# rickenator/steganosaurus

Measured on AMD Instinct MI355X. Metric: MPixels/s embed+extract round-trip (RGB 2D-FFT fwd+inv), higher is better.
Workload: dtype f32

## Files before the change

steganosaurus_amd/csrc/tfft_capi.hip:

```cpp
#include <hip/hip_runtime.h>
#include <math.h>
#include <stdio.h>
#include <stdlib.h>
#include <string.h>

#include <algorithm>
#include <complex>
#include <map>
#include <tuple>
#include <new>
#include <vector>

#include "tfft_kernels.h"

extern "C" void tfft_internal_radius_bounds(double lo, double hi, uint64_t* s_lo, uint64_t* s_hi, int* empty);
extern "C" float tfft_internal_mag2_threshold(double thr) { return tfft::mag2_threshold(thr); }

namespace {

using namespace tfft;

int next_pow2(int v) { int p = 1; while (p < v) p <<= 1; return p; }
int ilog2i(int n) { int l = 0; while ((1 << l) < n) l++; return l; }

struct Slot {
    int W = 0, H = 0, PW = 0, PH = 0, PWi = 0, center = 0;
    bool has_spec = false;
    const uint8_t* rgb_src = nullptr;
};

struct ColPlan { bool direct; int log_n1, log_n2; bool fused_fwd; };

}

struct tfft_ctx {
    int device = 0;
    int max_w = 0, max_h = 0, n_slots = 0;
    hipStream_t stream = nullptr;
    bool own_stream = false;
    hipEvent_t ev_t0 = nullptr, ev_t1 = nullptr;
    int last_hip = 0;
    size_t dev_bytes = 0;
    std::vector<Slot> slots;
    size_t img_stride_b = 0;
    size_t slot_stride = 0;
    size_t cand_stride = 0;
    uint8_t* img_pool = nullptr;
    float2* spec_pool = nullptr;
    float2* tmp_pool = nullptr;
    unsigned* cand_pool = nullptr;
    int stats_prio = 1;
    int stats_tile = 1;
    int stats_tile_step_forced = 0;
    int stats_tile_step = 8;
    float2* col0_pool = nullptr;
    int stats_skew = 0;
    SelectState* sel = nullptr;
    float* med = nullptr;
    unsigned* partial = nullptr;
    float* amb = nullptr;
    unsigned long long* usable = nullptr;
    int exact_stats = 1;
    ExactCand* ex_cand = nullptr; double2* ex_val = nullptr; unsigned long long* ex_below = nullptr; unsigned* ex_n = nullptr;
    std::map<int, double2*> ex_table;
    int ex_last[3] = {0, 0, 0};
    int* err = nullptr;
    uint8_t* trash = nullptr;
    int* last_row = nullptr;
    struct TileBuckets { float2* fl = nullptr; uint8_t* pb = nullptr; uint64_t fl_cap = 0;
                         unsigned* cnt = nullptr; unsigned* off = nullptr; TileBin* ent = nullptr; uint64_t cap = 0; int nb_cap = 0;
                         const void* built_for = nullptr; uint64_t built_n = 0; int built_ph = 0, built_pw = 0, built_g = 0; const void* built_index = nullptr; bool built_bad = false;
                         const void* row_for = nullptr; uint64_t row_n = 0; int row_ph = 0, row_pw = 0;
                         float2* jp = nullptr; uint64_t jp_cap = 0; uint64_t jp_for = 0;
                       } tb[2];
    const void* reg_bins = nullptr; uint64_t reg_n = 0;
    int embed_delta = 1;
    int tile_read = 1;
    hipStream_t stream2 = nullptr;
    hipEvent_t ev_fork = nullptr, ev_join = nullptr;
    hipStream_t stream_stats[2] = {nullptr, nullptr};
    hipEvent_t ev_stats_fork[2] = {nullptr, nullptr}, ev_stats_join[2] = {nullptr, nullptr};
    int stats_async = 1;
    int stats_m2 = 1;
    int n_streams = 1;
    int n_cus = 0, collect_resident = 0;
    uint32_t* bit_index = nullptr;
    uint64_t bit_index_n = 0;
    float* ph_jit = nullptr;
    uint64_t ph_n = 0;
    int ph_adaptive = 0;
    uint64_t ph_version = 0;
    std::map<int, float2*> tw;
    std::map<std::tuple<int, int, int, int>, float2*> dc;
    float dc_bias = 128.0f;
    uint8_t* sio_hdr = nullptr; uint8_t* sio_pay = nullptr; int* sio_status = nullptr; uint64_t sio_plen = 0;
    uint8_t* stream_bits = nullptr; unsigned* stream_plen = nullptr; size_t stream_cap = 0;
    void* stage_bins = nullptr; void* stage_bits = nullptr; void* stage_jit = nullptr; void* stage_out = nullptr;
    size_t stage_cap = 0;
    hipStream_t s_in = nullptr, s_out = nullptr;
    hipEvent_t ev_in[4] = {}, ev_comp[4] = {}, ev_out[4] = {};
    uint8_t* out_pool = nullptr;
    int cols_direct_max_log = 8;
    int cols_force_log_n1 = -1;
    int cols_tiles_per_block = 8;
    int cols_tiles_forced = 0;
    int cols_tiles_embed = 0;
    int cols_tiles_stat = 16;
    int cols_tiles_read = 16;
    int median_force_fallback = 0;
#ifndef TFFT_NO_GRAPHS
    struct GraphEntry { hipGraphExec_t exec = nullptr; int state = 0; };
    std::map<std::vector<uint64_t>, GraphEntry> graphs;
#endif
    int stats_fail_once = 0;
    bool stats_dirty = false;
    bool graphs_stale = false;
    int graph_max_images = 0;
    int stats_fused = 1;
    int stats_compact = 1;
    int fuse = 1;
    int fuse_wide = 1;
// ... 66 lines not shown
    if (w > c->max_w || h > c->max_h) return TFFT_E_TOO_LARGE;
    s.W = w; s.H = h; s.PW = next_pow2(w); s.PH = next_pow2(h);
    s.PWi = s.PW < 2 ? 2 : s.PW;
    s.center = center ? 1 : 0;
    if (s.PWi > TFFT_MAX_DIM || s.PH > TFFT_MAX_DIM) return TFFT_E_TOO_LARGE;
    return TFFT_OK;
}

enum Stage { ROWS_FWD = 0, COLS_FWD_A = 1, COLS_FWD_B = 2, EMBED = 3, COLS_INV_A = 4, COLS_INV_B = 5, ROWS_INV = 6,
             READ = 7, MEDIANS = 8, CAPACITY = 9,
             COLS_FWD_READ = 10,
             N_STAGES = 11 };

int get_dc_table(tfft_ctx* c, int valid, int N, int center, int kind, double scale, const float2** out);
void invalidate_graphs(tfft_ctx* c);

static void copy_embed_fields(ColParams& cp, const ColParams& e, bool inverse) {
    cp.rd_bins = e.rd_bins; cp.rd_off = e.rd_off; cp.trash = e.trash; cp.rd_walks = e.rd_walks;
    cp.em_n = e.em_n; cp.em_cos = e.em_cos; cp.em_sin = e.em_sin; cp.em_fl = e.em_fl; cp.em_pb = e.em_pb; cp.em_on = 1; cp.em_m2 = e.em_m2;
    if (inverse) { cp.em_jp = e.em_jp; cp.em_med = e.em_med; cp.em_alpha = e.em_alpha; cp.em_dsrc = e.em_dsrc; }
    cp.st_sel = e.st_sel; cp.st_cand = e.st_cand; cp.st_cand_stride = e.st_cand_stride; cp.st_partial = e.st_partial; cp.st_amb = e.st_amb;
    cp.st_col0 = e.st_col0; cp.st_slo = e.st_slo; cp.st_shi = e.st_shi; cp.st_cap = e.st_cap; cp.st_PW = e.st_PW;
}

static void copy_plain_extra(ColParams& cp, const ColParams& e) {
    if (e.tile_step > 1) cp.tiles_per_block = e.hist_sel ? 2 : 1;
    cp.tile_step = e.tile_step; cp.tile_off = e.tile_off; cp.out_M = e.out_M; cp.out_plane_stride = e.out_plane_stride; cp.out_img_stride = e.out_img_stride; cp.gate = e.gate;
    cp.hist_sel = e.hist_sel; cp.g_step = e.g_step; cp.g_off = e.g_off;
}

struct StageMode {
    const ColParams* fwd_emit = nullptr;
    const ColParams* fwd_read = nullptr;
    const int* fwd_last_row = nullptr;
    const ColParams* inv_embed = nullptr;
    const uint8_t* inv_cover = nullptr;
    const ColParams* fwd_plain_extra = nullptr;
    float2* fwd_out_override = nullptr;
    bool inv_via_spec = false;
};

int enqueue_fft_stage(tfft_ctx* c, int s0, int n, int stage, const uint8_t* rgb_in, uint8_t* rgb_out, hipStream_t st, const StageMode& md = StageMode()) {
    const Slot& s = c->slots[s0];
    const int M = s.PWi / 2;
    const float2 *tw_w, *tw_h;
    int rc = get_twiddles(c, s.PWi, &tw_w); if (rc) return rc;
    rc = get_twiddles(c, s.PH, &tw_h); if (rc) return rc;
    const ColPlan pl = plan_cols(c, s.PH, s.PWi, n);
    const int N1 = 1 << pl.log_n1, N2 = 1 << pl.log_n2;
    float2 *spec = c->spec(s0), *tmp = c->tmp(s0);
    ColParams cp{};
    cp.M = M; cp.PH = s.PH; cp.plane_stride = (size_t)s.PH * M; cp.img_stride = c->slot_stride;
    cp.tiles_per_block = c->cols_tiles_per_block;
    switch (stage) {
        case ROWS_FWD: {
            RowParams rp{s.W, s.H, s.PWi, s.PH, s.center, 0.f, c->slot_stride, c->dc_bias, nullptr};
            if (pl.fused_fwd && c->fuse_live && s.H < s.PH) HIPCHK(c, launch_rowcol_fwd_live(rgb_in, tmp, tw_w, tw_h, rp, n, st));
            else if (pl.fused_fwd) HIPCHK(c, launch_rowcol_fwd(rgb_in, tmp, tw_w, tw_h, rp, n, st));
            else HIPCHK(c, launch_rows_fwd(rgb_in, tmp, tw_w, rp, n, st));
            return TFFT_OK;
        }
        case COLS_FWD_A:
            if (pl.fused_fwd) return TFFT_OK;
            if (pl.direct) {
                cp.G = 1; cp.in_a = 1; cp.in_b = 0; cp.out_a = 1; cp.out_b = 0; cp.in_rows = s.H; cp.out_rows = s.PH; cp.tw_out = 0;
                cp.last_row_dev = md.fwd_last_row;
            if (c->dc_bias != 0.0f) {
                rc = get_dc_table(c, s.H, s.PH, s.center, 0, (double)c->dc_bias, &cp.dc_ah); if (rc) return rc;
                rc = get_dc_table(c, s.W, s.PWi, s.center, 1, 1.0, &cp.dc_aw); if (rc) return rc;
            }
                if (md.fwd_read) { const ColParams& r = *md.fwd_read; cp.rd_bins = r.rd_bins; cp.rd_off = r.rd_off; cp.rd_bits = r.rd_bits; cp.rd_n = r.rd_n; cp.em_jp = r.em_jp; cp.rd_walks = r.rd_walks; cp.trash = c->trash; cp.tiles_per_block = c->cols_tiles_read; }
                else if (md.fwd_emit) { copy_embed_fields(cp, *md.fwd_emit, false); if (!c->cols_tiles_forced && pl.log_n2 <= 8) cp.tiles_per_block = 2; if (cp.st_sel && c->cols_tiles_stat) cp.tiles_per_block = c->cols_tiles_stat; }
                else if (md.fwd_plain_extra) copy_plain_extra(cp, *md.fwd_plain_extra);
                HIPCHK(c, launch_cols(tmp, md.fwd_out_override ? md.fwd_out_override : spec, tw_h, cp, pl.log_n2, +1, 3 * n, st));
            } else {
                cp.G = N2; cp.in_a = N2; cp.in_b = 1; cp.out_a = N2; cp.out_b = 1; cp.in_rows = s.H; cp.out_rows = s.PH; cp.tw_out = 1;
                HIPCHK(c, launch_cols(tmp, tmp, tw_h, cp, pl.log_n1, +1, 3 * n, st));
            }
            return TFFT_OK;
        case COLS_FWD_B:
            if (pl.direct) return TFFT_OK;
            cp.G = N1; cp.in_a = 1; cp.in_b = N2; cp.out_a = N1; cp.out_b = 1; cp.in_rows = s.PH; cp.out_rows = s.PH; cp.tw_out = 0;
            cp.last_row_dev = md.fwd_last_row;
            if (c->dc_bias != 0.0f) {
                rc = get_dc_table(c, s.H, s.PH, s.center, 0, (double)c->dc_bias, &cp.dc_ah); if (rc) return rc;
                rc = get_dc_table(c, s.W, s.PWi, s.center, 1, 1.0, &cp.dc_aw); if (rc) return rc;
            }
            if (md.fwd_read) { const ColParams& r = *md.fwd_read; cp.rd_bins = r.rd_bins; cp.rd_off = r.rd_off; cp.rd_bits = r.rd_bits; cp.rd_n = r.rd_n; cp.em_jp = r.em_jp; cp.rd_walks = r.rd_walks; cp.trash = c->trash; cp.tiles_per_block = c->cols_tiles_read; }
            else if (md.fwd_emit) { copy_embed_fields(cp, *md.fwd_emit, false); if (!c->cols_tiles_forced && pl.log_n2 <= 8) cp.tiles_per_block = 2; if (cp.st_sel && c->cols_tiles_stat) cp.tiles_per_block = c->cols_tiles_stat; }
                else if (md.fwd_plain_extra) copy_plain_extra(cp, *md.fwd_plain_extra);
            HIPCHK(c, launch_cols(tmp, md.fwd_out_override ? md.fwd_out_override : spec, tw_h, cp, pl.log_n2, +1, 3 * n, st));
            return TFFT_OK;
        case COLS_INV_A:
            if (pl.direct) {
                cp.G = 1; cp.in_a = 1; cp.in_b = 0; cp.out_a = 1; cp.out_b = 0; cp.in_rows = s.PH; cp.out_rows = s.H; cp.tw_out = 0;
                if (md.inv_embed) { copy_embed_fields(cp, *md.inv_embed, true); cp.tiles_per_block = c->cols_tiles_embed ? c->cols_tiles_embed : (pl.log_n2 >= 9 ? 2 : 16); }
                else if (c->dc_bias != 0.0f) {
                    rc = get_dc_table(c, s.H, s.PH, s.center, 0, (double)c->dc_bias, &cp.dc_ah); if (rc) return rc;
                    rc = get_dc_table(c, s.W, s.PWi, s.center, 1, 1.0, &cp.dc_aw); if (rc) return rc;
                }
                HIPCHK(c, launch_cols(spec, md.inv_via_spec ? spec : tmp, tw_h, cp, pl.log_n2, -1, 3 * n, st));
            } else {
                cp.G = N1; cp.in_a = N1; cp.in_b = 1; cp.out_a = 1; cp.out_b = N2; cp.in_rows = s.PH; cp.out_rows = s.PH; cp.tw_out = 1;
                if (md.inv_embed) { copy_embed_fields(cp, *md.inv_embed, true); cp.tiles_per_block = c->cols_tiles_embed ? c->cols_tiles_embed : (pl.log_n2 >= 9 ? 2 : 16); }
                else if (c->dc_bias != 0.0f) {
                    rc = get_dc_table(c, s.H, s.PH, s.center, 0, (double)c->dc_bias, &cp.dc_ah); if (rc) return rc;
                    rc = get_dc_table(c, s.W, s.PWi, s.center, 1, 1.0, &cp.dc_aw); if (rc) return rc;
                }
                HIPCHK(c, launch_cols(spec, md.inv_via_spec ? spec : tmp, tw_h, cp, pl.log_n2, -1, 3 * n, st));
            }
            return TFFT_OK;
        case COLS_INV_B:
            if (pl.direct || pl.fused_fwd) return TFFT_OK;
            cp.G = N2; cp.in_a = N2; cp.in_b = 1; cp.out_a = N2; cp.out_b = 1; cp.in_rows = s.PH; cp.out_rows = s.H; cp.tw_out = 0;
            HIPCHK(c, launch_cols(md.inv_via_spec ? spec : tmp, md.inv_via_spec ? spec : tmp, tw_h, cp, pl.log_n1, -1, 3 * n, st));
            return TFFT_OK;
        case ROWS_INV: {
            RowParams rp{s.W, s.H, s.PWi, s.PH, s.center, (float)(1.0 / ((double)M * (double)s.PH)), c->slot_stride, c->dc_bias, nullptr};
            if (md.inv_cover) { rp.cover = md.inv_cover; rp.bias = 0.f; }
            if (md.inv_via_spec && !md.inv_embed) return TFFT_E_INVALID;
            if (pl.fused_fwd) HIPCHK(c, launch_colrow_inv(md.inv_via_spec ? spec : tmp, rgb_out, tw_w, rp, n, st));
            else HIPCHK(c, launch_rows_inv(md.inv_via_spec ? spec : tmp, rgb_out, tw_w, rp, n, st));
            return TFFT_OK;
        }
        default: return TFFT_E_INVALID;
    }
}

int enqueue_forward(tfft_ctx* c, int s0, int n, const uint8_t* rgb_dev, hipStream_t st, const StageMode& md = StageMode()) {
    for (int stage : {ROWS_FWD, COLS_FWD_A, COLS_FWD_B}) {
        int rc = enqueue_fft_stage(c, s0, n, stage, rgb_dev, nullptr, st, md);
        if (rc) return rc;
    }
    for (int i = 0; i < n; i++) { c->slots[s0 + i].has_spec = true; c->slots[s0 + i].rgb_src = nullptr; }
    return TFFT_OK;
}

int enqueue_inverse(tfft_ctx* c, int s0, int n, uint8_t* rgb_out_dev, hipStream_t st, const StageMode& md = StageMode()) {
    for (int stage : {COLS_INV_A, COLS_INV_B, ROWS_INV}) {
        int rc = enqueue_fft_stage(c, s0, n, stage, nullptr, rgb_out_dev, st, md);
        if (rc) return rc;
    }
    for (int i = 0; i < n; i++) c->slots[s0 + i].has_spec = false;
    return TFFT_OK;
}

static std::complex<double> dc_series(int k, int valid, int N, int center) {
    double th = 2.0 * M_PI * (double)k / (double)N + (center ? M_PI : 0.0);
    th = fmod(th, 2.0 * M_PI);
    const double sh = sin(0.5 * th);
    if (fabs(sh) < 1e-14) return std::complex<double>((double)valid, 0.0);
    const double mag = sin(0.5 * th * valid) / sh, ph = 0.5 * th * (valid - 1);
    return std::complex<double>(mag * cos(ph), mag * sin(ph));
}
int get_dc_table(tfft_ctx* c, int valid, int N, int center, int kind, double scale, const float2** out) {
    const auto key = std::make_tuple(valid, N, center ? 1 : 0, kind);
    auto it = c->dc.find(key);
    if (it != c->dc.end()) { *out = it->second; return TFFT_OK; }
    const int n = (kind == 0) ? N : (N / 2 > 0 ? N / 2 : 1);
    std::vector<float2> h((size_t)n);
    for (int k = 0; k < n; k++) {
        std::complex<double> a = dc_series(k, valid, N, center);
        if (kind == 1 && k == 0) a += std::complex<double>(0.0, 1.0) * dc_series(N / 2, valid, N, center);
        a *= scale;
        h[k] = make_float2((float)a.real(), (float)a.imag());
    }
    float2* d = nullptr;
    int rc = dev_alloc(c, (void**)&d, sizeof(float2) * (size_t)n);
    if (rc) return rc;
    HIPCHK(c, hipMemcpy(d, h.data(), sizeof(float2) * (size_t)n, hipMemcpyHostToDevice));
    c->dc[key] = d;
    *out = d;
// ... 135 lines not shown
}

bool slot_ok(const tfft_ctx* c, int slot) { return c && slot >= 0 && slot < c->n_slots; }

}

extern "C" {

int tfft_abi_version(void) { return TFFT_ABI_VERSION; }

const char* tfft_strerror(int status) {
    switch (status) {
        case TFFT_OK: return "ok";
        case TFFT_E_INVALID: return "invalid argument";
        case TFFT_E_NO_DEVICE: return "no usable gfx950 HIP device (this library has no CPU fallback)";
        case TFFT_E_TOO_LARGE: return "image larger than the context allows";
        case TFFT_E_NOMEM: return "out of memory";
        case TFFT_E_HIP: return "HIP runtime error";
        case TFFT_E_STATE: return "slot holds no forward spectrum";
        case TFFT_E_EXHAUSTED: return "annulus exhausted";
        case TFFT_E_BIN_RANGE: return "bin outside the grid or on an excluded axis";
        default: return "unknown status";
    }
}

int tfft_create(int device, int max_w, int max_h, int n_slots, tfft_ctx** out) {
    if (!out || max_w < 1 || max_h < 1 || n_slots < 1 || n_slots > 1024) return TFFT_E_INVALID;
    *out = nullptr;
    int pw = next_pow2(max_w), ph = next_pow2(max_h);
    if (pw < 2) pw = 2;
    if (pw > TFFT_MAX_DIM || ph > TFFT_MAX_DIM) return TFFT_E_TOO_LARGE;
    int ndev = 0;
    if (hipGetDeviceCount(&ndev) != hipSuccess || device < 0 || device >= ndev) return TFFT_E_NO_DEVICE;
    hipDeviceProp_t prop;
    if (hipGetDeviceProperties(&prop, device) != hipSuccess) return TFFT_E_NO_DEVICE;
    if (strncmp(prop.gcnArchName, "gfx950", 6) != 0 && !getenv("TFFT_ALLOW_OTHER_ARCH")) return TFFT_E_NO_DEVICE;
    if (hipSetDevice(device) != hipSuccess) return TFFT_E_NO_DEVICE;
    tfft_ctx* c = new (std::nothrow) tfft_ctx();
    if (!c) return TFFT_E_NOMEM;
    c->device = device; c->max_w = max_w; c->max_h = max_h; c->n_slots = n_slots;
    if (const char* e = getenv("TFFT_COLS_DIRECT_MAX_LOG")) c->cols_direct_max_log = atoi(e);
    if (const char* e = getenv("TFFT_COLS_LOG_N1")) c->cols_force_log_n1 = atoi(e);
    c->n_cus = prop.multiProcessorCount;
    c->collect_resident = collect_bracket_resident_blocks();
    if (const char* e = getenv("TFFT_FUSE")) c->fuse = atoi(e);
    if (const char* e = getenv("TFFT_FUSE_WIDE")) c->fuse_wide = atoi(e);
    if (const char* e = getenv("TFFT_FUSE_LIVE")) c->fuse_live = atoi(e);
    if (const char* e = getenv("TFFT_EMBED_DELTA")) c->embed_delta = atoi(e);
    if (const char* e = getenv("TFFT_STATS_ASYNC")) c->stats_async = atoi(e);
    if (const char* e = getenv("TFFT_STATS_M2")) c->stats_m2 = atoi(e);
    if (const char* e = getenv("TFFT_STATS_SKEW")) c->stats_skew = atoi(e);
    if (const char* e = getenv("TFFT_STREAMS")) c->n_streams = atoi(e);
    if (const char* e = getenv("TFFT_TILE_READ")) c->tile_read = atoi(e);
    if (const char* e = getenv("TFFT_DC_BIAS")) c->dc_bias = (float)atof(e);
    if (const char* e = getenv("TFFT_MEDIAN_FALLBACK")) c->median_force_fallback = atoi(e);
    if (const char* e = getenv("TFFT_STATS_FUSED")) c->stats_fused = atoi(e);
    if (const char* e = getenv("TFFT_STATS_COMPACT")) c->stats_compact = atoi(e);
    if (const char* e = getenv("TFFT_GRAPHS")) c->graph_max_images = atoi(e);
    if (const char* e = getenv("TFFT_EXACT_STATS")) c->exact_stats = atoi(e);
    if (const char* e = getenv("TFFT_BATCH_EXACT_TRACE")) c->bx_trace = atoi(e);
    if (const char* e = getenv("TFFT_STATS_TILE")) c->stats_tile = atoi(e);
    if (const char* e = getenv("TFFT_STATS_PRIO")) c->stats_prio = atoi(e);
    if (const char* e = getenv("TFFT_STATS_FAIL_ONCE")) c->stats_fail_once = atoi(e);
    if (const char* e = getenv("TFFT_STATS_TILE_STEP")) { c->stats_tile_step = atoi(e); if (c->stats_tile_step < 8) c->stats_tile_step = 8; c->stats_tile_step_forced = 1; }
    if (const char* e = getenv("TFFT_COLS_TILES")) { c->cols_tiles_per_block = atoi(e) > 0 ? atoi(e) : 1; c->cols_tiles_forced = 1; }
    if (const char* e = getenv("TFFT_COLS_TILES_EMBED")) c->cols_tiles_embed = atoi(e) > 0 ? atoi(e) : 0;
    if (const char* e = getenv("TFFT_COLS_TILES_STAT")) c->cols_tiles_stat = atoi(e) > 0 ? atoi(e) : 0;
    if (const char* e = getenv("TFFT_COLS_TILES_READ")) c->cols_tiles_read = atoi(e) > 0 ? atoi(e) : 1;
    if (c->cols_direct_max_log > 10) c->cols_direct_max_log = 10;
    if (hipStreamCreateWithFlags(&c->stream, hipStreamNonBlocking) != hipSuccess) { delete c; return TFFT_E_HIP; }
    c->own_stream = true;
    (void)hipEventCreate(&c->ev_t0); (void)hipEventCreate(&c->ev_t1);
    c->slots.resize(n_slots);
    const size_t M = (size_t)pw / 2;
    c->slot_stride = 3 * (size_t)ph * M;
    c->cand_stride = (size_t)ph * (M + 1) + (size_t)ph * M / 4 + 256;
    c->img_stride_b = (((size_t)max_w * max_h * 3 + 255) / 256) * 256;
    const size_t ns = (size_t)n_slots;
    int rc = dev_alloc(c, (void**)&c->img_pool, ns * c->img_stride_b + 256);
    if (!rc) rc = dev_alloc(c, (void**)&c->spec_pool, ns * c->slot_stride * sizeof(float2));
    if (!rc) rc = dev_alloc(c, (void**)&c->tmp_pool, ns * c->slot_stride * sizeof(float2));
    if (!rc) rc = dev_alloc(c, (void**)&c->cand_pool, ns * 3 * c->cand_stride * sizeof(unsigned));
    if (!rc) rc = dev_alloc(c, (void**)&c->col0_pool, ns * 3 * (size_t)ph * sizeof(float2));
    if (!rc) rc = dev_alloc(c, (void**)&c->sel, ns * 3 * sizeof(SelectState));
    if (!rc) rc = dev_alloc(c, (void**)&c->med, ns * 3 * sizeof(float));
    if (!rc) rc = dev_alloc(c, (void**)&c->partial, (ns * 3 * TFFT_STAT_MAX_BLOCKS + ns) * sizeof(unsigned));
    if (!rc) rc = dev_alloc(c, (void**)&c->amb, ns * 3 * TFFT_AMB_CAP * sizeof(float));
    if (!rc) rc = dev_alloc(c, (void**)&c->usable, ns * sizeof(unsigned long long));
    if (!rc) rc = dev_alloc(c, (void**)&c->err, sizeof(int));
    if (!rc) rc = dev_alloc(c, (void**)&c->trash, 8192);
    if (!rc) rc = dev_alloc(c, (void**)&c->last_row, 2 * sizeof(int));
    if (!rc && hipMemset(c->err, 0, sizeof(int)) != hipSuccess) rc = TFFT_E_HIP;
    if (!rc && hipMemset(c->sel, 0, ns * 3 * sizeof(SelectState)) != hipSuccess) rc = TFFT_E_HIP;
    if (!rc && hipDeviceSynchronize() != hipSuccess) rc = TFFT_E_HIP;
    if (rc != TFFT_OK) { tfft_destroy(c); return rc; }
    *out = c;
    return TFFT_OK;
}

int tfft_destroy(tfft_ctx* c) {
    if (!c) return TFFT_OK;
    (void)hipSetDevice(c->device);
    (void)hipDeviceSynchronize();
    invalidate_graphs(c);
    (void)hipFree(c->img_pool); (void)hipFree(c->spec_pool); (void)hipFree(c->tmp_pool); (void)hipFree(c->cand_pool);
    (void)hipFree(c->col0_pool);
    (void)hipFree(c->sel); (void)hipFree(c->med); (void)hipFree(c->partial); (void)hipFree(c->amb); (void)hipFree(c->usable); (void)hipFree(c->err); (void)hipFree(c->ex_cand); (void)hipFree(c->ex_val); (void)hipFree(c->ex_below); (void)hipFree(c->ex_n); for (auto& kv : c->ex_table) (void)hipFree(kv.second); (void)hipFree(c->trash); (void)hipFree(c->bit_index); (void)hipFree(c->last_row); (void)hipFree(c->ph_jit);
    (void)hipFree(c->fit_d); (void)hipFree(c->fit_mu); (void)hipFree(c->fit_part); (void)hipFree(c->fit_cnt); (void)hipFree(c->fit_iters); (void)hipFree(c->fit_wrong);
    (void)hipFree(c->bx_win); (void)hipFree(c->bx_cand); (void)hipFree(c->bx_below); (void)hipFree(c->bx_n); (void)hipFree(c->bx_idx); (void)hipFree(c->bx_grp);
    (void)hipFree(c->bx_part); (void)hipFree(c->bx_val); (void)hipFree(c->an_buf);
    for (auto& b : c->tb) { (void)hipFree(b.cnt); (void)hipFree(b.off); (void)hipFree(b.ent); (void)hipFree(b.fl); (void)hipFree(b.pb); (void)hipFree(b.jp); }
    for (auto& kv : c->tw) (void)hipFree(kv.second);
    for (auto& kv : c->dc) (void)hipFree(kv.second);
    (void)hipFree(c->stage_bins); (void)hipFree(c->stage_bits); (void)hipFree(c->stage_jit); (void)hipFree(c->stage_out);
    (void)hipFree(c->out_pool); (void)hipFree(c->stream_bits); (void)hipFree(c->stream_plen);
    (void)hipFree(c->sio_hdr); (void)hipFree(c->sio_pay); (void)hipFree(c->sio_status);
    for (int i = 0; i < 4; i++) { if (c->ev_in[i]) (void)hipEventDestroy(c->ev_in[i]); if (c->ev_comp[i]) (void)hipEventDestroy(c->ev_comp[i]); if (c->ev_out[i]) (void)hipEventDestroy(c->ev_out[i]); }
    if (c->s_in) (void)hipStreamDestroy(c->s_in);
    if (c->stream2) (void)hipStreamDestroy(c->stream2);
    for (int i = 0; i < 2; i++) {
        if (c->stream_stats[i]) (void)hipStreamDestroy(c->stream_stats[i]);
        if (c->ev_stats_fork[i]) (void)hipEventDestroy(c->ev_stats_fork[i]);
        if (c->ev_stats_join[i]) (void)hipEventDestroy(c->ev_stats_join[i]);
    }
    if (c->ev_fork) (void)hipEventDestroy(c->ev_fork);
    if (c->ev_join) (void)hipEventDestroy(c->ev_join);
    if (c->s_out) (void)hipStreamDestroy(c->s_out);
    if (c->ev_t0) (void)hipEventDestroy(c->ev_t0);
    if (c->ev_t1) (void)hipEventDestroy(c->ev_t1);
    if (c->own_stream && c->stream) (void)hipStreamDestroy(c->stream);
    delete c;
    return TFFT_OK;
}

int tfft_set_stream(tfft_ctx* c, void* hip_stream) {
    if (!c) return TFFT_E_INVALID;
    invalidate_graphs(c);
    HIPCHK(c, hipStreamSynchronize(c->stream));
    if (c->own_stream && c->stream) (void)hipStreamDestroy(c->stream);
    c->stream = (hipStream_t)hip_stream;
    c->own_stream = false;
    return TFFT_OK;
}

int tfft_sync(tfft_ctx* c) {
    if (!c) return TFFT_E_INVALID;
    return check_err_flag(c);
}

int tfft_last_hip_error(const tfft_ctx* c) { return c ? c->last_hip : 0; }

int tfft_plan_info(const tfft_ctx* c, int w, int h, int n_images, int info[4]) {
    if (!c || !info || w < 1 || h < 1 || n_images < 1) return TFFT_E_INVALID;
    int pw = next_pow2(w), ph = next_pow2(h);
    if (pw < 2) pw = 2;
    if (pw > TFFT_MAX_DIM || ph > TFFT_MAX_DIM) return TFFT_E_TOO_LARGE;
    const ColPlan p = plan_cols(c, ph, pw, n_images);
    info[0] = p.direct ? 1 : 0; info[1] = p.log_n1; info[2] = p.log_n2; info[3] = p.fused_fwd ? 1 : 0;
    return TFFT_OK;
}
// ... 597 lines not shown
    if (!slot_ok(c, slot) || !out) return TFFT_E_INVALID;
    Slot& s = c->slots[slot];
    if (!s.has_spec) return TFFT_E_STATE;
    const size_t n = (size_t)3 * s.PH * s.PW;
    float2* d = nullptr;
    if (hipMalloc((void**)&d, n * sizeof(float2)) != hipSuccess) return TFFT_E_NOMEM;
    hipError_t e = launch_export_full(c->spec(slot), s.PH, s.PWi, s.PW, d, c->stream);
    if (e == hipSuccess) e = hipMemcpyAsync(out, d, n * sizeof(float2), hipMemcpyDeviceToHost, c->stream);
    if (e == hipSuccess) e = hipStreamSynchronize(c->stream);
    (void)hipFree(d);
    if (e != hipSuccess) { c->last_hip = (int)e; return TFFT_E_HIP; }
    return TFFT_OK;
}

static int batch_geometry(tfft_ctx* c, int g, int w, int h, int center) {
    for (int i = 0; i < g; i++) { int rc = set_geometry(c, c->slots[i], w, h, center); if (rc) return rc; }
    return TFFT_OK;
}

static int ensure_buckets(tfft_ctx* c, int which, uint64_t n, int nb, bool with_values = false) {
    auto& b = c->tb[which];
    if (n > b.cap || !b.ent) {
        (void)hipStreamSynchronize(c->stream);
        if (c->stream2) (void)hipStreamSynchronize(c->stream2);
        invalidate_graphs(c);
        b.built_for = nullptr;
        (void)hipFree(b.ent); b.ent = nullptr; b.cap = 0;
        const uint64_t cap = n + n / 4 + 1024;
        if (dev_alloc(c, (void**)&b.ent, cap * sizeof(TileBin))) return TFFT_E_NOMEM;
        b.cap = cap;
    }
    if (nb + 1 > b.nb_cap || !b.cnt) {
        (void)hipStreamSynchronize(c->stream);
        if (c->stream2) (void)hipStreamSynchronize(c->stream2);
        invalidate_graphs(c);
        b.built_for = nullptr;
        (void)hipFree(b.cnt); (void)hipFree(b.off); b.cnt = b.off = nullptr; b.nb_cap = 0;
        if (dev_alloc(c, (void**)&b.cnt, (size_t)(nb + 1) * sizeof(unsigned)) || dev_alloc(c, (void**)&b.off, (size_t)(nb + 1 + (nb + 1023) / 1024) * sizeof(unsigned)))
            return TFFT_E_NOMEM;
        b.nb_cap = nb + 1;
    }
    if (with_values && (n * (uint64_t)c->n_slots > b.fl_cap || !b.fl)) {
        (void)hipStreamSynchronize(c->stream);
        if (c->stream2) (void)hipStreamSynchronize(c->stream2);
        invalidate_graphs(c);
        (void)hipFree(b.fl); (void)hipFree(b.pb); b.fl = nullptr; b.pb = nullptr; b.fl_cap = 0;
        const uint64_t cap = (n + n / 4 + 1024) * (uint64_t)c->n_slots;
        if (dev_alloc(c, (void**)&b.fl, cap * sizeof(float2)) || dev_alloc(c, (void**)&b.pb, cap)) return TFFT_E_NOMEM;
        b.fl_cap = cap;
    }
    return TFFT_OK;
}

static int build_buckets(tfft_ctx* c, int which, const tfft_bin* bins, uint64_t n_bits, const Slot& s, int G, hipStream_t st) {
    auto& tb = c->tb[which];
    const bool registered = bins == c->reg_bins && n_bits == c->reg_n;
    if (!(registered && tb.built_for == bins && tb.built_n == n_bits && tb.built_ph == s.PH && tb.built_pw == s.PWi && tb.built_g == G &&
          tb.built_index == c->bit_index)) {
        if (tb.built_for) c->graphs_stale = true;
        HIPCHK(c, launch_bucket_bins(bins, c->bit_index, n_bits, s.PH, s.PWi, G, tb.cnt, tb.off, tb.ent, c->err, c->tile_read == 2, st));
        tb.built_for = registered ? bins : nullptr; tb.built_n = n_bits; tb.built_ph = s.PH; tb.built_pw = s.PWi; tb.built_g = G; tb.built_index = c->bit_index;
        tb.built_bad = false;
        tb.jp_for = 0;
        if (registered && st == c->stream) {
            const int rc = check_err_flag(c);
            if (rc == TFFT_E_BIN_RANGE) tb.built_bad = true;
            else if (rc) return rc;
        }
    }
    if (tb.built_bad) HIPCHK(c, hipMemsetAsync(c->err, 0x01, sizeof(int), st));
    return TFFT_OK;
}

static int gather_jitter(tfft_ctx* c, int which, uint64_t n_bits, int nb, hipStream_t st) {
    auto& tb = c->tb[which];
    if (!c->ph_jit) return TFFT_OK;
    if (n_bits > tb.jp_cap || !tb.jp) {
        (void)hipStreamSynchronize(c->stream);
        if (c->stream2) (void)hipStreamSynchronize(c->stream2);
        invalidate_graphs(c);
        (void)hipFree(tb.jp); tb.jp = nullptr; tb.jp_cap = 0; tb.jp_for = 0;
        const uint64_t cap = n_bits + n_bits / 4 + 1024;
        if (dev_alloc(c, (void**)&tb.jp, cap * sizeof(float2))) return TFFT_E_NOMEM;
        tb.jp_cap = cap;
    }
    if (tb.jp_for != c->ph_version) {
        if (tb.jp_for) c->graphs_stale = true;
        HIPCHK(c, launch_gather_jitter(tb.ent, tb.off + nb, c->ph_jit, n_bits, tb.jp, st));
        tb.jp_for = c->ph_version;
    }
    return TFFT_OK;
}

static hipError_t create_stats_stream(tfft_ctx* c, hipStream_t* out) {
    int lo = 0, hi = 0;
    if (c->stats_prio && hipDeviceGetStreamPriorityRange(&lo, &hi) == hipSuccess && lo != hi)
        return hipStreamCreateWithPriority(out, hipStreamNonBlocking, lo);
    return hipStreamCreateWithFlags(out, hipStreamNonBlocking);
}

static bool tilestats_applies(const tfft_ctx* c, const Slot& s, const ColPlan& pl, const CapParams& p, int n) {
    if (!(c->stats_tile && c->stats_fused && c->stats_compact && !c->median_force_fallback)) return false;
    if (c->stats_tile < 2 && (unsigned long long)n * s.PH * s.PWi < (1ull << 24)) return false;
    const unsigned long long mirror_d = (unsigned long long)(p.PW - s.PWi / 2) * (unsigned long long)(p.PW - s.PWi / 2);
    return p.bw > 0 && p.s_lo <= p.s_hi && p.s_hi < 0xFFFFFFFFull && mirror_d > p.s_hi && !pl.direct && pl.log_n2 >= 4 && pl.log_n2 <= 9 &&
           (unsigned long long)s.PH * s.PWi <= (1ull << 24) && (s.PWi / 2) % 16 == 0;
}

static int enqueue_tilestats_select(tfft_ctx* c, int s0, int g, hipStream_t st) {
    const Slot& s = c->slots[s0];
    HIPCHK(c, launch_stat_select(s.PH, g, c->sel + 3 * s0, c->cand_pool + (size_t)3 * s0 * c->cand_stride, c->cand_stride, c->med + 3 * s0,
                                 c->col0_pool + (size_t)s0 * 3 * s.PH, st));
    return TFFT_OK;
// ... 25 lines not shown
    if (!c->stats_tile_step_forced && G >= 8 && step >= 2 && ntiles / step >= 2) { g_step = 4; step /= 2; }
    const int off = ntiles > step / 2 ? step / 2 : 0;
    const int Ms = 16 * ((ntiles - off + step - 1) / step);
    int rc;
    for (int stage : {ROWS_FWD, COLS_FWD_A}) {
        if (stage == final_fwd || !(phases & 1)) break;
        rc = enqueue_fft_stage(c, s0, g, stage, rgb_in, nullptr, st);
        if (rc) return rc;
    }
    float2* col0 = c->col0_pool + (size_t)s0 * 3 * s.PH;
    SelectState* sel = c->sel + 3 * s0;
    unsigned* partial = c->partial + (size_t)s0 * (3 * TFFT_STAT_MAX_BLOCKS + 1);
    float* amb = c->amb + (size_t)3 * s0 * TFFT_AMB_CAP;
    unsigned* cand = c->cand_pool + (size_t)3 * s0 * c->cand_stride;
    ColParams ex{};
    ex.tile_step = step; ex.tile_off = off; ex.out_M = Ms; ex.out_plane_stride = (size_t)s.PH * Ms; ex.out_img_stride = (size_t)3 * s.PH * Ms;
    ex.hist_sel = sel; ex.g_step = g_step; ex.g_off = g_step / 2;
    if (phases & 2) {
        StageMode ms;
        ms.fwd_plain_extra = &ex;
        rc = enqueue_fft_stage(c, s0, g, final_fwd, rgb_in, nullptr, st, ms);
        if (rc) return rc;
        HIPCHK(c, launch_stat_guess(nullptr, s.PH, s.PWi, Ms, ex.out_img_stride, g, sel, &cap, partial, 0, st));
        if (c->stats_skew) HIPCHK(c, launch_skew_bracket(sel, g, c->stats_skew, st));
    }
    if (phases & 4) {
    em.st_sel = sel; em.st_cand = cand; em.st_cand_stride = c->cand_stride; em.st_partial = partial; em.st_amb = amb; em.st_col0 = col0;
    em.st_slo = cap.s_lo > 0xFFFFFFFFull ? 0xFFFFFFFFu : (unsigned)cap.s_lo; em.st_shi = cap.s_hi > 0xFFFFFFFFull ? 0xFFFFFFFFu : (unsigned)cap.s_hi;
    em.st_cap = 1; em.st_PW = cap.PW;
    { StageMode me; me.fwd_emit = &em;
      rc = enqueue_fft_stage(c, s0, g, final_fwd, rgb_in, nullptr, st, me); }
    em.st_sel = nullptr;
    if (rc) return rc;
    }
    if (phases & 8) {
        rc = enqueue_tilestats_select(c, s0, g, st);
        if (rc) return rc;
    }
    if (phases & 16) return enqueue_tilestats_tail(c, s0, g, rgb_in, st, cap, usable);
    return TFFT_OK;
}

struct FrameSrc { const uint8_t* hdr; const uint8_t* pay; uint64_t plen; };
struct WalkSrc { const float* jit; int adaptive; };
static int build_buckets_walks(tfft_ctx* c, int which, const tfft_bin* bins, uint64_t n_bits, int g, const Slot& s, int G, const float* jit,
                               hipStream_t st) {
    const int ntiles = (s.PWi / 2 + 15) / 16, nbt = 3 * ntiles * G * g + 1;
    if ((uint64_t)g * n_bits > 0xFFFFFFFFull || (uint64_t)3 * ntiles * G * g + 1 > 1024ull * 1024ull) return TFFT_E_TOO_LARGE;
    int rc = ensure_buckets(c, which, (uint64_t)g * n_bits, nbt);
    if (rc) return rc;
    auto& tb = c->tb[which];
    if (tb.built_for) c->graphs_stale = true;
    tb.built_for = nullptr; tb.jp_for = 0; tb.row_for = nullptr;
    HIPCHK(c, launch_bucket_walks(bins, n_bits, g, s.PH, s.PWi, G, tb.cnt, tb.off, tb.ent, c->err, st));
    if (!jit) return TFFT_OK;
    const uint64_t need = (uint64_t)g * n_bits;
    if (need > tb.jp_cap || !tb.jp) {
        (void)hipStreamSynchronize(c->stream);
        if (c->stream2) (void)hipStreamSynchronize(c->stream2);
        invalidate_graphs(c);
        (void)hipFree(tb.jp); tb.jp = nullptr; tb.jp_cap = 0;
        const uint64_t cap = need + need / 4 + 1024;
        if (dev_alloc(c, (void**)&tb.jp, cap * sizeof(float2))) return TFFT_E_NOMEM;
        tb.jp_cap = cap;
    }
    HIPCHK(c, launch_gather_jitter_walks(tb.ent, jit, n_bits, g, tb.jp, st));
    return TFFT_OK;
}
static int embed_chunk_impl(tfft_ctx* c, int s0, int g, const uint8_t* rgb_in, const tfft_bin* bins, const uint8_t* bits,
                            uint64_t n_bits, double alpha, double rmin, double rmax, double magmin,
                            unsigned long long* usable, uint8_t* rgb_out, hipStream_t st, uint64_t limit, const FrameSrc* frame, const WalkSrc* walks);
static int embed_chunk(tfft_ctx* c, int s0, int g, const uint8_t* rgb_in, const tfft_bin* bins, const uint8_t* bits,
                       uint64_t n_bits, double alpha, double rmin, double rmax, double magmin,
                       unsigned long long* usable, uint8_t* rgb_out, hipStream_t st, uint64_t limit = ~0ull, const FrameSrc* frame = nullptr,
                       const WalkSrc* walks = nullptr) {
    if (!usable && (walks ? walks->adaptive : c->ph_adaptive) && n_bits > 0) usable = c->usable + s0;
    int rc = usable ? stats_clean_if_dirty(c, st) : TFFT_OK;
    if (!rc) rc = embed_chunk_impl(c, s0, g, rgb_in, bins, bits, n_bits, alpha, rmin, rmax, magmin, usable, rgb_out, st, limit, frame, walks);
    if (!rc && usable && c->stats_fail_once) {
        c->stats_fail_once = 0;
        HIPCHK(c, hipMemsetAsync(c->sel, 0x01, (size_t)c->n_slots * 3 * sizeof(SelectState), st));
        rc = TFFT_E_HIP;
    }
    if (rc && usable) c->stats_dirty = true;
    return rc;
}
static int embed_chunk_impl(tfft_ctx* c, int s0, int g, const uint8_t* rgb_in, const tfft_bin* bins, const uint8_t* bits,
                            uint64_t n_bits, double alpha, double rmin, double rmax, double magmin,
                            unsigned long long* usable, uint8_t* rgb_out, hipStream_t st, uint64_t limit, const FrameSrc* frame, const WalkSrc* walks) {
    const Slot& s = c->slots[s0];
    if (!index_ok(c, n_bits) || !phase_ok(c, n_bits)) return TFFT_E_STATE;
    if (walks && (c->bit_index || c->ph_jit)) return TFFT_E_STATE;
    const bool adaptive = walks ? walks->adaptive != 0 : c->ph_adaptive != 0;
    const float* jit = walks ? walks->jit : c->ph_jit;
    EmbedParams ep = embed_params(c, s, n_bits, alpha, adaptive, nullptr, jit != nullptr);
    if (walks) ep.bins_stride = n_bits;
    if (adaptive) ep.med_dev = c->med + 3 * s0;
    if (limit < n_bits) ep.limit = limit;
    if (frame) { ep.frame_hdr = frame->hdr; ep.frame_pay = frame->pay; ep.frame_plen = frame->plen; }
    const bool delta = c->embed_delta && alpha > 0.0 && alpha < M_PI && n_bits > 0;
    const int which = (c->stream2 && st == c->stream2) ? 1 : 0;
    ColParams em{};
    int rc;
    if (delta) {
        const ColPlan pl = plan_cols(c, s.PH, s.PWi, g);
        const int G = pl.direct ? 1 : (1 << pl.log_n1), ntiles = (s.PWi / 2 + 15) / 16, nb = 3 * ntiles * G;
        rc = ensure_buckets(c, which, n_bits, nb, true);
        if (rc) return rc;
        rc = walks ? build_buckets_walks(c, which, bins, n_bits, g, s, G, jit, st) : build_buckets(c, which, bins, n_bits, s, G, st);
        if (rc) return rc;
        auto& tb = c->tb[which];
        em.rd_bins = tb.ent; em.rd_off = tb.off; em.trash = c->trash; em.em_fl = tb.fl + (size_t)s0 * n_bits; em.em_pb = tb.pb + (size_t)s0 * n_bits;
        em.em_n = walks ? 0 : n_bits; em.em_cos = ep.cos_a; em.em_sin = ep.sin_a; em.rd_walks = walks ? 1 : 0;
        if (!walks) rc = gather_jitter(c, which, n_bits, nb, st);
        if (rc) return rc;
        em.em_jp = jit ? tb.jp : nullptr;
        em.em_med = adaptive ? c->med + 3 * s0 : nullptr; em.em_alpha = (float)alpha;
        if (usable) {
            CapParams p0 = cap_params(c, s, rmin, rmax);
            if (stats_m2_applies(c, s, p0)) { em.em_m2 = 1; em.st_col0 = c->col0_pool + (size_t)s0 * 3 * s.PH; }
        } else if (c->stats_m2) {
            em.em_m2 = 2; em.st_col0 = c->col0_pool + (size_t)s0 * 3 * s.PH;
        }
        if (walks) HIPCHK(c, launch_gather_bits_walks(tb.ent, bits, ep.frame_hdr, ep.frame_pay, ep.frame_plen, n_bits, ep.limit, g, tb.pb + (size_t)s0 * n_bits, st));
        else HIPCHK(c, launch_gather_bits(tb.ent, tb.off + nb, bits, ep.frame_hdr, ep.frame_pay, ep.frame_plen, n_bits, ep.limit, g, tb.pb + (size_t)s0 * n_bits, st));
    }
    if (delta && usable) {
        CapParams p = cap_params(c, s, rmin, rmax);
        p.magmin = magmin;
        if (tilestats_applies(c, s, plan_cols(c, s.PH, s.PWi, g), p, g)) {
            em.em_m2 = 0;
            rc = enqueue_forward_tilestats(c, s0, g, rgb_in, st, em, p, usable, 7);
            if (rc) return rc;
            hipStream_t sst = st;
            if (c->stats_async && !adaptive) {
                if (!c->stream_stats[which]) {
                    HIPCHK(c, create_stats_stream(c, &c->stream_stats[which]));
                    HIPCHK(c, hipEventCreateWithFlags(&c->ev_stats_fork[which], hipEventDisableTiming));
                    HIPCHK(c, hipEventCreateWithFlags(&c->ev_stats_join[which], hipEventDisableTiming));
                }
                sst = c->stream_stats[which];
                HIPCHK(c, hipEventRecord(c->ev_stats_fork[which], st));
                HIPCHK(c, hipStreamWaitEvent(sst, c->ev_stats_fork[which], 0));
            }
            rc = enqueue_tilestats_select(c, s0, g, sst);
            if (rc) return rc;
            if (adaptive) {
                rc = enqueue_tilestats_tail(c, s0, g, rgb_in, st, p, usable);
                if (rc) return rc;
            }
            StageMode mi;
            mi.inv_embed = &em; mi.inv_cover = rgb_in; mi.inv_via_spec = true;
            rc = enqueue_inverse(c, s0, g, rgb_out, st, mi);
            if (rc) return rc;
            if (sst != st) {
                HIPCHK(c, hipEventRecord(c->ev_stats_join[which], sst));
                HIPCHK(c, hipStreamWaitEvent(st, c->ev_stats_join[which], 0));
            }
            return adaptive ? TFFT_OK : enqueue_tilestats_tail(c, s0, g, rgb_in, st, p, usable);
        }
    }
    StageMode md;
    if (delta) md.fwd_emit = &em;
    rc = enqueue_forward(c, s0, g, rgb_in, st, md);
    if (rc) return rc;
    hipStream_t sst = st;
// ... 9 lines not shown
        HIPCHK(c, hipStreamWaitEvent(sst, c->ev_stats_fork[which], 0));
    }
    if (usable) {
        CapParams p = cap_params(c, s, rmin, rmax);
        p.magmin = magmin;
        if (c->stats_fused && p.bw > 0) {
            rc = enqueue_medians(c, s0, g, sst, &p, usable, em.em_m2 != 0);
            if (rc) return rc;
        } else {
            rc = enqueue_medians(c, s0, g, sst);
            if (rc) return rc;
            HIPCHK(c, launch_capacity(c->spec(s0), p, g, c->med + 3 * s0, c->partial + (size_t)s0 * (3 * TFFT_STAT_MAX_BLOCKS + 1), usable, sst));
        }
    }
    if (delta) {
        StageMode mi;
        mi.inv_embed = &em; mi.inv_cover = rgb_in;
        rc = enqueue_inverse(c, s0, g, rgb_out, st, mi);
        if (async) {
            HIPCHK(c, hipEventRecord(c->ev_stats_join[which], sst));
            HIPCHK(c, hipStreamWaitEvent(st, c->ev_stats_join[which], 0));
        }
        return rc;
    }
    HIPCHK(c, launch_embed(c->spec(s0), bins, bits, jit, ep, g, c->err, st));
    return enqueue_inverse(c, s0, g, rgb_out, st);
}
static int extract_chunk(tfft_ctx* c, int s0, int g, const uint8_t* rgb_in, const tfft_bin* bins, uint64_t n_bits,
                         double alpha, uint8_t* bits_out, hipStream_t st, const WalkSrc* walks = nullptr) {
    const Slot& s = c->slots[s0];
    if (!index_ok(c, n_bits) || !phase_ok(c, n_bits)) return TFFT_E_STATE;
    if (walks && (c->bit_index || c->ph_jit)) return TFFT_E_STATE;
    const bool adaptive = walks ? walks->adaptive != 0 : c->ph_adaptive != 0;
    const float* jit = walks ? walks->jit : c->ph_jit;
    if (adaptive && !(fabs(alpha) < M_PI / 2)) return TFFT_E_INVALID;
    const int which = (c->stream2 && st == c->stream2) ? 1 : 0;
    EmbedParams ep = embed_params(c, s, n_bits, alpha, 0, nullptr, jit != nullptr);
    if (walks) ep.bins_stride = n_bits;
    int rc;
    const bool reg_large = !walks && bins == c->reg_bins && n_bits == c->reg_n && (unsigned long long)s.PH * s.PWi >= (1ull << 23);
    if (c->tile_read && n_bits > 0 && alpha > 0.0 && alpha < M_PI && (g >= 8 || c->tile_read >= 2 || reg_large)) {
        const ColPlan pl = plan_cols(c, s.PH, s.PWi, g);
        const int G = pl.direct ? 1 : (1 << pl.log_n1), ntiles = (s.PWi / 2 + 15) / 16, nb = 3 * ntiles * G;
        rc = walks ? TFFT_OK : ensure_buckets(c, which, n_bits, nb);
        if (rc) return rc;
        auto& tb = c->tb[which];
        HIPCHK(c, hipMemsetAsync(bits_out, 0, (size_t)g * n_bits, st));
        rc = walks ? build_buckets_walks(c, which, bins, n_bits, g, s, G, jit, st) : build_buckets(c, which, bins, n_bits, s, G, st);
        if (rc) return rc;
        if (!walks) rc = gather_jitter(c, which, n_bits, nb, st);
        if (rc) return rc;
        ColParams rd{};
        rd.rd_bins = tb.ent; rd.rd_off = tb.off; rd.rd_bits = bits_out; rd.rd_n = n_bits; rd.trash = c->trash;
        rd.em_jp = jit ? tb.jp : nullptr; rd.rd_walks = walks ? 1 : 0;
        StageMode md;
        md.fwd_read = &rd;
        rc = enqueue_forward(c, s0, g, rgb_in, st, md);
        if (rc) return rc;
    } else {
        int* last_row = c->last_row + which;
        auto& tbr = c->tb[which];
        const bool registered = !walks && bins == c->reg_bins && n_bits == c->reg_n;
        if (!(registered && tbr.row_for == bins && tbr.row_n == n_bits && tbr.row_ph == s.PH && tbr.row_pw == s.PWi)) {
            HIPCHK(c, launch_bins_last_row(bins, walks ? (uint64_t)g * n_bits : n_bits, s.PH, s.PWi, last_row, st));
            tbr.row_for = registered ? bins : nullptr; tbr.row_n = n_bits; tbr.row_ph = s.PH; tbr.row_pw = s.PWi;
        }
        StageMode md;
        md.fwd_last_row = last_row;
        rc = enqueue_forward(c, s0, g, rgb_in, st, md);
        if (rc) return rc;
        HIPCHK(c, launch_read(c->spec(s0), bins, jit, ep, g, bits_out, c->err, st));
    }
    for (int i = 0; i < g; i++) c->slots[s0 + i].has_spec = false;
    return TFFT_OK;
}

static int split_fork(tfft_ctx* c, int g, int* h1) {
    *h1 = 0;
    if (c->n_streams < 2 || g < 8) return TFFT_OK;
    if (!c->stream2) {
        HIPCHK(c, hipStreamCreateWithFlags(&c->stream2, hipStreamNonBlocking));
        HIPCHK(c, hipEventCreateWithFlags(&c->ev_fork, hipEventDisableTiming));
        HIPCHK(c, hipEventCreateWithFlags(&c->ev_join, hipEventDisableTiming));
    }
    HIPCHK(c, hipEventRecord(c->ev_fork, c->stream));
    HIPCHK(c, hipStreamWaitEvent(c->stream2, c->ev_fork, 0));
    *h1 = g / 2;
    return TFFT_OK;
}
static int split_join(tfft_ctx* c) {
    HIPCHK(c, hipEventRecord(c->ev_join, c->stream2));
    HIPCHK(c, hipStreamWaitEvent(c->stream, c->ev_join, 0));
    return TFFT_OK;
}

static int embed_batch_dev_impl(tfft_ctx* c, int n_images, const void* rgb_dev, int w, int h, int center, const void* bins_dev,
                                const void* bits_dev, uint64_t n_bits, double alpha, double rmin, double rmax, double magmin,
                                void* usable_out_dev, void* rgb_out_dev, int32_t* bx = nullptr) {
    const size_t img_bytes = (size_t)w * h * 3;
    for (int i0 = 0; i0 < n_images; i0 += c->n_slots) {
        const int g = (n_images - i0 < c->n_slots) ? n_images - i0 : c->n_slots;
        int rc = batch_geometry(c, g, w, h, center);
        if (rc) return rc;
        const uint8_t* cov = (const uint8_t*)rgb_dev + (size_t)i0 * img_bytes;
        if (bx && c->bx_mode) { cov = bx_keep_covers(c, g, cov, (const uint8_t*)rgb_out_dev + (size_t)i0 * img_bytes, img_bytes, c->stream, &rc); if (rc) return rc; }
        int h1 = 0;
        rc = split_fork(c, g, &h1);
// ... 413 lines not shown
        if (dev_alloc(c, (void**)&c->fit_part, (size_t)c->n_slots * kFitMaxBlocks * 2 * sizeof(unsigned)) ||
            dev_alloc(c, (void**)&c->fit_cnt, (size_t)c->n_slots * 2 * sizeof(unsigned)) ||
            dev_alloc(c, (void**)&c->fit_iters, (size_t)c->n_slots * sizeof(int32_t)) ||
            dev_alloc(c, (void**)&c->fit_wrong, (size_t)c->n_slots * sizeof(uint32_t))) return TFFT_E_NOMEM;
    }
    if (c->fit_d && need <= c->fit_cap) return TFFT_OK;
    (void)hipStreamSynchronize(c->stream);
    invalidate_graphs(c);
    (void)hipFree(c->fit_d); (void)hipFree(c->fit_mu); c->fit_d = nullptr; c->fit_mu = nullptr; c->fit_cap = 0;
    const uint64_t cap = need + need / 4 + 1024;
    if (dev_alloc(c, (void**)&c->fit_d, cap * sizeof(float2)) || dev_alloc(c, (void**)&c->fit_mu, cap * sizeof(float))) return TFFT_E_NOMEM;
    c->fit_cap = cap;
    return TFFT_OK;
}

static int fit_forward(tfft_ctx* c, int g, const uint8_t* rgb, hipStream_t st) {
    auto& tb = c->tb[0];
    ColParams em{};
    em.rd_bins = tb.ent; em.rd_off = tb.off; em.trash = c->trash; em.em_fl = tb.fl; em.em_pb = tb.pb; em.em_n = 0; em.rd_walks = 1;
    if (c->stats_m2) { em.em_m2 = 2; em.st_col0 = c->col0_pool; }
    StageMode md; md.fwd_emit = &em;
    return enqueue_forward(c, 0, g, rgb, st, md);
}

static int fit_chunk(tfft_ctx* c, int g, const uint8_t* cover, const tfft_bin* bins, const float* jit, uint64_t n_bins, int adaptive,
                     const FrameSrc& fr, uint64_t n_bits, double alpha, double rmin, double rmax, double magmin, unsigned long long* usable,
                     int max_iters, double margin, uint8_t* rgb_out, int32_t* iters, uint32_t* wrong_dev) {
    hipStream_t st = c->stream;
    const Slot& s = c->slots[0];
    const WalkSrc ws{jit, adaptive ? 1 : 0};
    int rc = embed_chunk(c, 0, g, cover, bins, nullptr, n_bins, alpha, rmin, rmax, magmin, usable, rgb_out, st, n_bits, &fr, &ws);
    if (rc) return rc;
    rc = check_err_flag(c);
    if (rc) return rc;
    auto& tb = c->tb[0];
    if (!c->embed_delta) {
        const ColPlan pl = plan_cols(c, s.PH, s.PWi, g);
        const int G = pl.direct ? 1 : (1 << pl.log_n1), ntiles = (s.PWi / 2 + 15) / 16;
        rc = ensure_buckets(c, 0, n_bins, 3 * ntiles * G, true);
        if (!rc) rc = build_buckets_walks(c, 0, bins, n_bins, g, s, G, jit, st);
        if (rc) return rc;
        HIPCHK(c, launch_gather_bits_walks(tb.ent, nullptr, fr.hdr, fr.pay, fr.plen, n_bins, n_bits, g, tb.pb, st));
        rc = fit_forward(c, g, cover, st);
        if (rc) return rc;
    }
    const float2* jp = jit ? tb.jp : nullptr;
    const double sigma = sqrt((double)s.W * (double)s.H / 24.0);
    HIPCHK(c, launch_fit_init(tb.ent, tb.fl, tb.pb, jp, bins, adaptive ? c->med : nullptr, n_bins, g, alpha, margin, TFFT_FIT_KAPPA * sigma,
                              c->fit_d, c->fit_mu, st));
    const double gain = ((double)s.PW * (double)s.PH) / ((double)s.W * (double)s.H);
    const unsigned nblk = (unsigned)std::min<uint64_t>(kFitMaxBlocks, (n_bins + 1023) / 1024);
    ColParams ed{};
    ed.rd_bins = tb.ent; ed.rd_off = tb.off; ed.trash = c->trash; ed.em_fl = c->fit_d; ed.em_pb = tb.pb; ed.em_n = 0; ed.rd_walks = 1; ed.em_dsrc = 1;
    std::vector<unsigned> cnt((size_t)2 * g);
    for (int i = 0; i < g; i++) iters[i] = -1;
    for (int t = 0;; t++) {
        rc = fit_forward(c, g, rgb_out, st);
        if (rc) return rc;
        HIPCHK(c, launch_fit_count(tb.ent, tb.fl, tb.pb, jp, c->fit_mu, n_bins, g, nblk, c->fit_part, c->fit_cnt, wrong_dev, st));
        HIPCHK(c, hipMemcpyAsync(cnt.data(), c->fit_cnt, cnt.size() * sizeof(unsigned), hipMemcpyDeviceToHost, st));
        HIPCHK(c, hipStreamSynchronize(st));
        bool all = true;
        for (int i = 0; i < g; i++) {
            if (iters[i] < 0 && cnt[2 * i] == 0 && cnt[2 * i + 1] == 0) iters[i] = t;
            all = all && iters[i] >= 0;
        }
        if (all || t >= max_iters) break;
        HIPCHK(c, launch_fit_correct(tb.ent, tb.fl, tb.pb, jp, c->fit_mu, c->fit_cnt, n_bins, g, gain, c->fit_d, st));
        StageMode mi; mi.inv_embed = &ed; mi.inv_cover = cover;
        rc = enqueue_inverse(c, 0, g, rgb_out, st, mi);
        if (rc) return rc;
    }
    return TFFT_OK;
}

static int fit_args_ok(const tfft_ctx* c, int n_images, uint64_t n_bins, uint64_t payload_len, double alpha, int adaptive, int max_iters,
                       double margin) {
    int rc = walks_args_ok(c, n_images, n_bins, alpha, adaptive, false);
    if (rc) return rc;
    if (!(alpha > 0.0 && alpha < M_PI / 2) || max_iters < 0 || !(margin > 0.0)) return TFFT_E_INVALID;
    if (n_bins < 912 || payload_len > (n_bins - 912) / 56) return TFFT_E_INVALID;
    return TFFT_OK;
}

int tfft_embed_stream_batch_fit_dev(tfft_ctx* c, int n_images, const void* rgb_dev, int w, int h, int center, const void* bins_dev,
                                    const void* jitter_dev, uint64_t n_bins, int adaptive, const void* header_dev, const void* payload_dev,
                                    uint64_t payload_len, double alpha, double rmin, double rmax, double magmin, int max_iters, double margin,
                                    void* usable_out_dev, void* iters_out_dev, void* wrong_out_dev, void* rgb_out_dev) {
    if (!c || !rgb_dev || !rgb_out_dev || !bins_dev || !header_dev || (payload_len && !payload_dev)) return TFFT_E_INVALID;
    int rc = fit_args_ok(c, n_images, n_bins, payload_len, alpha, adaptive, max_iters, margin);
    if (rc) return rc;
    rc = ensure_fit(c, n_bins);
    if (rc) return rc;
    const uint64_t n_bits = 38ull * 24 + payload_len * 56;
    const size_t img_bytes = (size_t)w * h * 3;
    std::vector<int32_t> iters((size_t)c->n_slots);
    int32_t* bx = bx_begin(c, n_images, usable_out_dev);
    for (int i0 = 0; i0 < n_images; i0 += c->n_slots) {
        const int g = (n_images - i0 < c->n_slots) ? n_images - i0 : c->n_slots;
        rc = batch_geometry(c, g, w, h, center);
        if (rc) return rc;
        HIPCHK(c, hipMemcpyAsync(c->img(0), (const uint8_t*)rgb_dev + (size_t)i0 * img_bytes, (size_t)g * img_bytes, hipMemcpyDeviceToDevice, c->stream));
        const FrameSrc fr{(const uint8_t*)header_dev + (size_t)i0 * 38, (const uint8_t*)payload_dev + (size_t)i0 * payload_len, payload_len};
        rc = fit_chunk(c, g, c->img(0), (const tfft_bin*)bins_dev + (size_t)i0 * n_bins, jitter_dev ? (const float*)jitter_dev + (size_t)i0 * n_bins : nullptr,
                       n_bins, adaptive, fr, n_bits, alpha, rmin, rmax, magmin, usable_out_dev ? (unsigned long long*)usable_out_dev + i0 : nullptr,
                       max_iters, margin, (uint8_t*)rgb_out_dev + (size_t)i0 * img_bytes, iters.data(), wrong_out_dev ? (uint32_t*)wrong_out_dev + i0 : nullptr);
// ... 229 lines not shown
    return TFFT_OK;
}
int tfft_frame_majority_dev(tfft_ctx* c, int n_images, const void* bits_dev, uint64_t payload_len, void* header_out_dev,
                            void* payload_out_dev) {
    if (!c || n_images < 0 || !bits_dev || !header_out_dev || (payload_len && !payload_out_dev)) return TFFT_E_INVALID;
    if (n_images == 0) return TFFT_OK;
    HIPCHK(c, launch_frame_majority((const uint8_t*)bits_dev, payload_len, n_images, (uint8_t*)header_out_dev, (uint8_t*)payload_out_dev, c->stream));
    return TFFT_OK;
}

int tfft_profile_stage(tfft_ctx* c, int n_images, int stage, int reps, const void* rgb_dev, void* rgb_out_dev,
                       const void* bins_dev, const void* bits_dev, void* bits_out_dev, uint64_t n_bits, double alpha,
                       float* ms_per_rep, int* n_launches) {
    if (!c || n_images < 1 || n_images > c->n_slots || reps < 1 || !ms_per_rep || stage < 0 || stage >= N_STAGES) return TFFT_E_INVALID;
    const Slot& s = c->slots[0];
    if (s.PH == 0) return TFFT_E_STATE;
    for (int i = 1; i < n_images; i++) c->slots[i] = s;
    const ColPlan pl = plan_cols(c, s.PH, s.PWi, n_images);
    int launches = 1;
    const int final_fwd = pl.direct ? COLS_FWD_A : COLS_FWD_B;
    if ((stage == COLS_FWD_B || stage == COLS_INV_B) && pl.direct) launches = 0;
    if ((stage == COLS_FWD_A || stage == COLS_INV_B) && pl.fused_fwd) launches = 0;
    if (stage == ROWS_FWD && pl.fused_fwd && c->fuse_live && s.H < s.PH && (s.H % (s.PH >> 3)) != 0) launches = 2;
    {
        const bool compact = c->stats_compact && (unsigned long long)s.PH * s.PWi <= (1ull << 24);
        const bool finish1 = compact && (unsigned long long)s.PH * s.PWi <= (1ull << 22) && n_images <= 4;
        if (stage == MEDIANS) launches = compact ? (c->median_force_fallback ? 2 : (finish1 ? 5 : 7)) + (c->stats_fused ? 1 : 0)
                                                 : (c->median_force_fallback ? 7 : 13) + (c->stats_fused ? 3 : 0);
    }
    if (stage == CAPACITY) launches = c->stats_fused ? 0 : 2;
    bool delta = false;
    if (c->embed_delta && bins_dev && n_bits > 0 && (stage == EMBED || stage == COLS_INV_A || stage == ROWS_INV || stage == final_fwd || stage == MEDIANS)) {
        const EmbedParams ep0 = embed_params(c, s, n_bits, alpha, 0, nullptr, false);
        delta = !ep0.generic;
    }
    CapParams tcap = cap_params(c, s, 0.05, 0.45);
    tcap.magmin = 0.01;
    const bool tile = delta && bits_dev && tilestats_applies(c, s, pl, tcap, n_images) && (stage == final_fwd || stage == MEDIANS);
    const bool m2 = delta && bits_dev && !tile && stats_m2_applies(c, s, tcap);
    if (tile && stage == MEDIANS) launches = 10;

    if (n_launches) *n_launches = launches;
    *ms_per_rep = 0.f;
    if (launches == 0) return TFFT_OK;
    { const float2* t; int rc = get_twiddles(c, s.PWi, &t); if (rc) return rc; rc = get_twiddles(c, s.PH, &t); if (rc) return rc; }
    ColParams rd{};
    if (stage == COLS_FWD_READ) {
        if (!bins_dev || !index_ok(c, n_bits)) return TFFT_E_INVALID;
        if (c->tile_read && n_bits > 0 && (n_images >= 8 || c->tile_read >= 2)) {
            if (!bits_out_dev) return TFFT_E_INVALID;
            const int G = pl.direct ? 1 : (1 << pl.log_n1), ntiles = (s.PWi / 2 + 15) / 16;
            int rc = ensure_buckets(c, 0, n_bits, 3 * ntiles * G);
            if (rc) return rc;
            HIPCHK(c, launch_bucket_bins((const tfft_bin*)bins_dev, c->bit_index, n_bits, s.PH, s.PWi, G, c->tb[0].cnt, c->tb[0].off, c->tb[0].ent, c->err, c->tile_read == 2, c->stream));
            rd.rd_bins = c->tb[0].ent; rd.rd_off = c->tb[0].off; rd.rd_bits = (uint8_t*)bits_out_dev; rd.rd_n = n_bits; rd.trash = c->trash;
        } else {
            HIPCHK(c, launch_bins_last_row((const tfft_bin*)bins_dev, n_bits, s.PH, s.PWi, c->last_row, c->stream));
        }
    }
    ColParams em{};
    if ((stage == COLS_INV_A || stage == final_fwd || stage == EMBED || (stage == MEDIANS && tile)) && delta && bits_dev) {
        if (!index_ok(c, n_bits)) return TFFT_E_STATE;
        const int G = pl.direct ? 1 : (1 << pl.log_n1), ntiles = (s.PWi / 2 + 15) / 16;
        int rc = ensure_buckets(c, 0, n_bits, 3 * ntiles * G, true);
        if (rc) return rc;
        rc = build_buckets(c, 0, (const tfft_bin*)bins_dev, n_bits, s, G, c->stream);
        if (rc) return rc;
        const EmbedParams ep0 = embed_params(c, s, n_bits, alpha, 0, nullptr, false);
        em.rd_bins = c->tb[0].ent; em.rd_off = c->tb[0].off; em.trash = c->trash; em.em_fl = c->tb[0].fl; em.em_pb = c->tb[0].pb; em.em_n = n_bits;
        em.em_cos = ep0.cos_a; em.em_sin = ep0.sin_a;
        if (m2) { em.em_m2 = 1; em.st_col0 = c->col0_pool; }
    }
    if (tile) {
        float ms_all = 0.f, ms_stat = 0.f;
        int rc = enqueue_forward_tilestats(c, 0, n_images, (const uint8_t*)rgb_dev, c->stream, em, tcap, c->usable, 2);
        if (rc) return rc;
        HIPCHK(c, hipEventRecord(c->ev_t0, c->stream));
        for (int r = 0; r < reps; r++) { rc = enqueue_forward_tilestats(c, 0, n_images, (const uint8_t*)rgb_dev, c->stream, em, tcap, c->usable, 4); if (rc) return rc; }
        HIPCHK(c, hipEventRecord(c->ev_t1, c->stream));
        HIPCHK(c, hipEventSynchronize(c->ev_t1));
        HIPCHK(c, hipEventElapsedTime(&ms_stat, c->ev_t0, c->ev_t1));
        if (stage == MEDIANS) {
            HIPCHK(c, hipEventRecord(c->ev_t0, c->stream));
            for (int r = 0; r < reps; r++) { rc = enqueue_forward_tilestats(c, 0, n_images, (const uint8_t*)rgb_dev, c->stream, em, tcap, c->usable, 2 | 4 | 8 | 16); if (rc) return rc; }
            HIPCHK(c, hipEventRecord(c->ev_t1, c->stream));
            HIPCHK(c, hipEventSynchronize(c->ev_t1));
            HIPCHK(c, hipEventElapsedTime(&ms_all, c->ev_t0, c->ev_t1));
        }
        *ms_per_rep = (stage == MEDIANS ? (ms_all > ms_stat ? ms_all - ms_stat : 0.f) : ms_stat) / (float)reps;
        return TFFT_OK;
    }
    HIPCHK(c, hipEventRecord(c->ev_t0, c->stream));
    for (int r = 0; r < reps; r++) {
        int rc = TFFT_OK;
        switch (stage) {
            case COLS_FWD_A:
            case COLS_FWD_B:
                { StageMode md; if (em.rd_bins && stage == final_fwd) md.fwd_emit = &em;
                  rc = enqueue_fft_stage(c, 0, n_images, stage, (const uint8_t*)rgb_dev, nullptr, c->stream, md); }
                break;
            case COLS_INV_A:
                { StageMode md; if (em.rd_bins) md.inv_embed = &em;
                  rc = enqueue_fft_stage(c, 0, n_images, stage, nullptr, nullptr, c->stream, md); }
                break;
            case ROWS_INV:
                { StageMode md; if (delta && rgb_dev) md.inv_cover = (const uint8_t*)rgb_dev;
                  rc = enqueue_fft_stage(c, 0, n_images, stage, nullptr, (uint8_t*)rgb_out_dev, c->stream, md); }
                break;
            case COLS_FWD_READ:
                { StageMode md; if (rd.rd_bins) md.fwd_read = &rd; else md.fwd_last_row = c->last_row;
                  rc = enqueue_fft_stage(c, 0, n_images, final_fwd, nullptr, nullptr, c->stream, md); }
                break;
            case EMBED: {
                if (!index_ok(c, n_bits)) return TFFT_E_STATE;
                if (em.rd_bins) {
                    const int G = pl.direct ? 1 : (1 << pl.log_n1), nb = 3 * ((s.PWi / 2 + 15) / 16) * G;
                    HIPCHK(c, launch_gather_bits(c->tb[0].ent, c->tb[0].off + nb, (const uint8_t*)bits_dev, nullptr, nullptr, 0, n_bits, n_bits, n_images, c->tb[0].pb, c->stream));
                    break;
                }
                EmbedParams ep = embed_params(c, s, n_bits, alpha, 0, nullptr, false);
                HIPCHK(c, launch_embed(c->spec(0), (const tfft_bin*)bins_dev, (const uint8_t*)bits_dev, nullptr, ep, n_images, c->err, c->stream));
                break;
            }
            case READ: {
                if (!index_ok(c, n_bits)) return TFFT_E_STATE;
                EmbedParams ep = embed_params(c, s, n_bits, alpha, 0, nullptr, false);
                HIPCHK(c, launch_read(c->spec(0), (const tfft_bin*)bins_dev, nullptr, ep, n_images, (uint8_t*)bits_out_dev, c->err, c->stream));
                break;
            }
            case MEDIANS:
                if (c->stats_fused) {
                    CapParams p = cap_params(c, s, 0.05, 0.45);
                    p.magmin = 0.01;
                    rc = enqueue_medians(c, 0, n_images, c->stream, &p, c->usable, m2);
                } else rc = enqueue_medians(c, 0, n_images, c->stream);
                break;
            case CAPACITY: {
                CapParams p = cap_params(c, s, 0.05, 0.45);
                p.magmin = 0.01;
                HIPCHK(c, launch_capacity(c->spec(0), p, n_images, c->med, c->partial, c->usable, c->stream));
                break;
            }
            default: rc = enqueue_fft_stage(c, 0, n_images, stage, (const uint8_t*)rgb_dev, (uint8_t*)rgb_out_dev, c->stream);
        }
        if (rc) return rc;
    }
    HIPCHK(c, hipEventRecord(c->ev_t1, c->stream));
    HIPCHK(c, hipEventSynchronize(c->ev_t1));
    float ms = 0.f;
    HIPCHK(c, hipEventElapsedTime(&ms, c->ev_t0, c->ev_t1));
    *ms_per_rep = ms / (float)reps;
    return TFFT_OK;
}

static int audit_run(tfft_ctx* c, double* host, const uint8_t* rgb, int w, int h, int center, int n_planes, int ph, int pw, int inverse) {
    const size_t bytes = (size_t)n_planes * ph * pw * sizeof(double2);
    double2 *a = nullptr, *scratch = nullptr, *wtab = nullptr;
    uint8_t* img = nullptr;
    int rc = TFFT_OK;
// ... 48 lines not shown
```

steganosaurus_amd/csrc/tfft_kernels.h:

```cpp
#pragma once
#include <hip/hip_runtime.h>
#include <float.h>
#include <math.h>
#include <stdint.h>

#include "../../include/turtlefft_hip.h"

namespace tfft {

struct RowParams {
    int W, H;
    int PW, PH;
    int center;
    float scale;
    size_t img_stride;
    float bias;
    const uint8_t* cover;
};

struct TileBin { uint16_t k; uint8_t c; uint8_t conj; uint32_t bit; };

struct ColParams {
    int M;
    int PH;
    int G;
    int in_a, in_b;
    int out_a, out_b;
    int in_rows;
    int out_rows;
    const struct TileBin* rd_bins;
    const unsigned* rd_off;
    uint8_t* rd_bits;
    uint64_t rd_n;
    uint8_t* trash;
    float2* em_fl;
    int em_m2;
    const uint8_t* em_pb;
    uint64_t em_n;
    float em_cos, em_sin;
    const float2* em_jp;
    const float* em_med;
    float em_alpha;
    struct SelectState* st_sel;
    unsigned* st_cand; size_t st_cand_stride;
    unsigned st_resv;
    unsigned st_cand_fixed;
    unsigned* st_partial;
    float* st_amb;
    float2* st_col0;
    unsigned st_slo, st_shi;
    int st_cap, st_PW;
    int tile_step, tile_off; int out_M; size_t out_plane_stride, out_img_stride;
    const struct SelectState* gate;
    struct SelectState* hist_sel; unsigned hist_lds_off;
    int g_step, g_off;
    int em_on;
    const float2* dc_ah;
    const float2* dc_aw;
    const int* last_row_dev;
    int tw_out;
    int tiles_per_block;
    size_t plane_stride;
    size_t img_stride;
    int rd_walks;
    int em_dsrc;
};

struct EmbedParams {
    uint64_t n;
    int PH, PW;
    int generic;
    int adaptive;
    float cos_a, sin_a;
    double alpha;
    double med[3];
    size_t img_stride;
    const uint32_t* bit_index;
    uint64_t limit;
    const uint8_t* frame_hdr; const uint8_t* frame_pay; uint64_t frame_plen;
    const float* med_dev;
    uint64_t bins_stride;
};

struct CapParams {
    int PH, PW;
    int PWi;
    int bw, bh;
    unsigned long long s_lo, s_hi;
    double magmin;
    double thr[3];
    size_t img_stride;
};

__host__ __device__ inline float mag2_threshold(double thr) {
    if (!(thr > 0.0)) return -INFINITY;
    float tf = (float)thr;
    if ((double)tf < thr) tf = nextafterf(tf, INFINITY);
    if (!(tf < INFINITY)) return INFINITY;
    float c = tf * tf;
    if (!(c < INFINITY)) c = FLT_MAX;
    for (int i = 0; i < 8 && !(sqrtf(c) < tf); i++) c = nextafterf(c, -INFINITY);
    for (int i = 0; i < 16 && sqrtf(c) < tf; i++) c = nextafterf(c, INFINITY);
    return c;
}

struct ExactCand { uint16_t y, x, w, plane; float m2; };
struct ExactCollect {
    int PH, PW;
    int PW_full;
    int cap;
    unsigned long long s_lo, s_hi;
    float lo2[3], hi2[3];
    int cap_cand;
};
hipError_t launch_exact_collect(const float2* spec, const ExactCollect& P, ExactCand* cand, unsigned long long* below, unsigned* n_cand, hipStream_t s);
hipError_t launch_exact_table(double2* table, int PW, hipStream_t s);
hipError_t launch_exact_eval(const uint8_t* rgb, int W, int H, int PW, int PH, int center, const ExactCand* cand, unsigned n, int n_split,
                             const double2* table, double2* out, hipStream_t s);
struct ExactCandB { uint16_t y, x, w, plane; float m2; uint32_t img; };
struct ExactWin { int img; float lo2[3], hi2[3]; int rsv; };
struct ExactVal { double re, im; float m2; uint32_t w; };
struct ExactGroup { unsigned first, count; };
#define TFFT_EXACT_K 8
hipError_t launch_exact_collect_batch(const float2* spec, size_t img_stride, const ExactCollect& P, const ExactWin* win, int n_win, ExactCandB* cand,
                                      unsigned long long* below, unsigned* n_cand, hipStream_t s);
hipError_t launch_exact_eval_batch(const uint8_t* rgb, size_t img_bytes, int W, int H, int PW, int PH, int center, const ExactCandB* cand,
                                   const unsigned* idx, const ExactGroup* groups, unsigned n_groups, int n_split, const double2* table, double2* out, hipStream_t s);
hipError_t launch_exact_sum_batch(const double2* part, int n_split, const ExactCandB* cand, const unsigned* idx, unsigned n, ExactVal* out, hipStream_t s);

#define TFFT_STAT_MAX_BLOCKS 512

struct SelectState {
    unsigned hist[4096];
    unsigned long long rank;
    unsigned long long below;
    unsigned prefix;
    unsigned n_cand;
    unsigned lo, hi;
    unsigned done;
    unsigned fast;
    float t2_lo, t2_hi;
    unsigned n_amb;
    unsigned cand_fixed;
};
#define TFFT_AMB_CAP 8192
#define TFFT_CAND_HOLE 0x7FFFFFFFu

hipError_t launch_rows_fwd(const uint8_t* rgb, float2* out, const float2* tw_pw, const RowParams& P, int n_images,
                           hipStream_t s);
hipError_t launch_rowcol_fwd(const uint8_t* rgb, float2* out, const float2* tw_pw, const float2* tw_ph, const RowParams& P,
                             int n_images, hipStream_t s);
hipError_t launch_colrow_inv(const float2* in, uint8_t* rgb, const float2* tw_pw, const RowParams& P, int n_images, hipStream_t s);
hipError_t launch_rowcol_fwd_live(const uint8_t* rgb, float2* out, const float2* tw_pw, const float2* tw_ph, const RowParams& P, int n_images, hipStream_t s);
hipError_t launch_rows_inv(const float2* in, uint8_t* rgb, const float2* tw_pw, const RowParams& P, int n_images,
                           hipStream_t s);
hipError_t launch_cols(const float2* in, float2* out, const float2* tw_ph, const ColParams& P, int logl, int sign,
                       int n_planes, hipStream_t s);
hipError_t audit_fft2d_f64(double2* a, double2* scratch, double2* wtab, int n_planes, int PH, int PW, int inverse, hipStream_t s);
hipError_t audit_load_rgb8_f64(const uint8_t* rgb_dev, int W, int H, int PW, int PH, int center, double2* out, hipStream_t s);
hipError_t launch_bucket_bins(const tfft_bin* bins, const uint32_t* bit_index, uint64_t n, int PH, int PW, int G,
                              unsigned* cnt, unsigned* off, TileBin* out, int* err, int force_global, hipStream_t s);
hipError_t launch_bucket_walks(const tfft_bin* bins, uint64_t n, int n_images, int PH, int PW, int G, unsigned* cnt, unsigned* off, TileBin* out,
                               int* err, hipStream_t s);
hipError_t launch_gather_bits_walks(const TileBin* ent, const uint8_t* bits, const uint8_t* hdr, const uint8_t* pay, uint64_t plen, uint64_t n,
                                    uint64_t limit, int n_images, uint8_t* out, hipStream_t s);
hipError_t launch_gather_jitter_walks(const TileBin* ent, const float* jitter, uint64_t n, int n_images, float2* out, hipStream_t s);
hipError_t launch_fit_init(const TileBin* ent, const float2* fl, const uint8_t* pb, const float2* jp, const tfft_bin* bins, const float* med,
                           uint64_t n, int n_images, double alpha, double tau, double mu_floor, float2* d, float* mu, hipStream_t s);
hipError_t launch_fit_count(const TileBin* ent, const float2* fl, const uint8_t* pb, const float2* jp, const float* mu, uint64_t n, int n_images,
                            unsigned nblk, unsigned* partial, unsigned* counts, uint32_t* wrong_out, hipStream_t s);
hipError_t launch_fit_correct(const TileBin* ent, const float2* fl, const uint8_t* pb, const float2* jp, const float* mu, const unsigned* counts,
                              uint64_t n, int n_images, double gain, float2* d, hipStream_t s);
hipError_t launch_stat_guess(const float2* mini, int PH, int PW, int Ms, size_t mini_img_stride, int n_images, SelectState* st, const struct CapParams* cap,
                             unsigned* partial, int col0_packed, hipStream_t s);
hipError_t launch_skew_bracket(SelectState* st, int n_images, int skew, hipStream_t s);
hipError_t launch_stat_select(int PH, int n_images, SelectState* st, unsigned* cand, size_t cand_stride, float* med_out, const float2* col0, hipStream_t s);
hipError_t launch_stat_settle(const float2* spec, int PH, int PW, size_t img_stride, int n_images, SelectState* st, float* med_out, const struct CapParams* cap,
                              unsigned* partial, float* amb, unsigned long long* usable, hipStream_t s);
hipError_t launch_gather_bits(const TileBin* ent, const unsigned* n_ent, const uint8_t* bits, const uint8_t* hdr, const uint8_t* pay, uint64_t plen,
                              uint64_t n, uint64_t limit, int n_images, uint8_t* out, hipStream_t s);
hipError_t launch_gather_jitter(const TileBin* ent, const unsigned* n_ent, const float* jitter, uint64_t n, float2* out, hipStream_t s);
hipError_t launch_bins_last_row(const tfft_bin* bins, uint64_t n, int PH, int PW, int* last_row, hipStream_t s);
hipError_t launch_embed(float2* spec, const tfft_bin* bins, const uint8_t* bits, const float* jitter,
                        const EmbedParams& P, int n_images, int* err, hipStream_t s);
hipError_t launch_read(const float2* spec, const tfft_bin* bins, const float* jitter, const EmbedParams& P,
                       int n_images, uint8_t* bits_out, int* err, hipStream_t s);
hipError_t launch_medians(const float2* spec, int PH, int PW, size_t img_stride, int n_images, SelectState* st,
                          unsigned* cand, size_t cand_stride, float* med_out, int force_fallback, int fill_cus, int fill_resident, hipStream_t s,
                          const CapParams* cap = nullptr, unsigned* partial = nullptr, float* amb = nullptr, unsigned long long* usable = nullptr,
                          int compact = 1, const float2* col0_m2 = nullptr, int skew = 0);
int collect_bracket_resident_blocks();
hipError_t launch_capacity(const float2* spec, const CapParams& P, int n_images, const float* med_dev,
                           unsigned* partial, unsigned long long* usable, hipStream_t s, const unsigned* only_flagged = nullptr);
hipError_t launch_frame_expand(const uint8_t* header, const uint8_t* payload, uint64_t plen, int n_images, uint8_t* bits,
                               uint64_t stride, hipStream_t s);
hipError_t launch_frame_majority(const uint8_t* bits, uint64_t plen, int n_images, uint8_t* header, uint8_t* payload,
                                 hipStream_t s);
hipError_t launch_stream_decode(const uint8_t* bits, uint64_t n_bins, uint64_t max_plen, int n_images, uint8_t* header, uint8_t* payload,
                                int* status, unsigned* plen, hipStream_t s);
hipError_t launch_export_full(const float2* spec, int PH, int PW, int PWout, float2* out, hipStream_t s);
hipError_t launch_lowfreq_f64(const uint8_t* rgb, int W, int H, int PW, int PH, int center, int region, double2* rowsum, double* out,
                              hipStream_t s);
hipError_t launch_lowfreq_f64_batch(const uint8_t* rgb, int W, int H, int PW, int PH, int center, int region, int n_images, double2* rowsum,
                                    size_t rowsum_stride, double* out, hipStream_t s);

struct PhaseHistParams {
    CapParams cap;
    float t2[3];
    int log_bins;
};
#define TFFT_PH_PARTIAL_WORDS 65536
int phase_hist_blocks(const CapParams& cp, int log_bins, int n_images);
hipError_t launch_phase_hist(const float2* spec, const PhaseHistParams& P, int n_images, unsigned* partial, uint32_t* hist_out, hipStream_t s);
#define TFFT_QA_TX 64
#define TFFT_QA_TY 32
#define TFFT_QA_LDS_OFF 18656
// ... 11 lines not shown
```

steganosaurus_amd/csrc/tfft_kernels.hip:

```cpp
#include <hip/hip_runtime.h>
#include <float.h>
#include <math.h>
#include <stdint.h>

#include <type_traits>

#include "tfft_fft.h"
#include "tfft_kernels.h"

#ifndef TFFT_WAVES_PER_EU
#define TFFT_WAVES_PER_EU(n) __attribute__((amdgpu_waves_per_eu(n)))
#endif
#ifndef TFFT_COLS_WAVES
#define TFFT_COLS_WAVES(logl) ((logl) >= 8 ? 4 : 1)
#endif
#ifndef TFFT_COLS_PF_MAXLOG
#define TFFT_COLS_PF_MAXLOG 7
#endif
#ifndef TFFT_COLS_PFEMIT
#define TFFT_COLS_PFEMIT 0
#endif
#ifndef TFFT_ROWS_LAZY_LOG
#define TFFT_ROWS_LAZY_LOG 11
#endif
// ... 98 lines not shown
            ldsf[2 * lay.idx(n >> 1, b) + (n & 1)] = v;
        };
        for (int o = tid; o < head && o < nbytes; o += nthr) put(o, src[o]);
        const int nwords = nbytes > head ? (nbytes - head) / 4 : 0;
        const uint32_t* srcw = reinterpret_cast<const uint32_t*>(src + head);
        for (int w = tid; w < nwords; w += nthr) {
            const uint32_t v = srcw[w];
            const int o = head + 4 * w;
            put(o, v & 0xFF); put(o + 1, (v >> 8) & 0xFF); put(o + 2, (v >> 16) & 0xFF); put(o + 3, v >> 24);
        }
        for (int o = head + 4 * nwords + tid; o < nbytes; o += nthr) put(o, src[o]);
        for (int n = P.W + tid; n < 2 * M; n += nthr) {
#pragma unroll
            for (int b = 0; b < PPB; b++) ldsf[2 * lay.idx(n >> 1, b) + (n & 1)] = 0.0f;
        }
    }
    constexpr bool LAZY = LOGM >= TFFT_ROWS_LAZY_LOG;
    float2 W[LAZY ? 1 : tw_regs<M, E>()];
    if (!LAZY) fft_prefetch_twiddles<M, E, +1>(W, t, tw, 2);
    constexpr int NSPLIT = (M / 2) / T + 1;
    float2 wk[NSPLIT];
#pragma unroll
    for (int j = 0; j < NSPLIT; j++) wk[j] = tw[imin(t + j * T, M / 2)];
    lds_barrier();

    float2 u[E];
#pragma unroll
    for (int m = 0; m < E; m++) u[m] = lds[lay.idx(t + m * T, pb)];
    Sync::sync();
    if (LAZY) fft_block_lazy<M, E, +1, Sync>(u, lds, lay, t, pb, tw, 2);
    else fft_block<M, E, +1, Sync>(u, lds, lay, t, pb, W);
#pragma unroll
    for (int m = 0; m < E; m++) lds[lay.idx(t + m * T, pb)] = u[m];
    Sync::sync();

    float2* dst = out + (size_t)img * P.img_stride + ((size_t)(plane0 + pb) * P.PH + y) * M;
#pragma unroll
    for (int j = 0; j < NSPLIT; j++) {
        const int k = t + j * T;
        if (k > M / 2) break;
        const int k2 = (M - k) & (M - 1);
        const float2 zk = lds[lay.idx(k, pb)], zm = lds[lay.idx(k2, pb)];
        float2 xk, xmk;
        rsplit_fwd(zk, zm, wk[j], xk, xmk);
        if (k == 0) {
            dst[0] = make_float2(xk.x, xmk.x);
        } else {
            dst[k] = xk;
            if (k2 != k) dst[k2] = xmk;
        }
    }
}

template <int LOGN1, int LOGM>
__global__ void __launch_bounds__(1 << (LOGM - 4 + LOGN1)) k_rowcol_fwd(const uint8_t* __restrict__ rgb, float2* __restrict__ out,
                             const float2* __restrict__ tw, const float2* __restrict__ tw_h, RowParams P) {
    constexpr int M = 1 << LOGM, E = 16, T = M / E, N1 = 1 << LOGN1;
    using Sync = typename std::conditional<T == 64, WaveSync, BlockSync>::type;
    const int t = threadIdx.x, n1 = threadIdx.y;
    const int N2 = P.PH >> LOGN1;
    int n2, plane;
    xcd_plane_order(N2, n2, plane);
    const int img = blockIdx.y;
    const int y = n1 * N2 + n2;
    float2* lds = reinterpret_cast<float2*>(tfft_smem);
    float* ldsf = reinterpret_cast<float*>(tfft_smem);
    LayRows lay{LayRows::padded(M)};
    const bool live = y < P.H;

    float2* ltw = lds + (size_t)N1 * lay.pitch;
    float2* lwc = ltw + M;

    constexpr int NT = M / (T * N1);
    float2 tv[NT];
#pragma unroll
    for (int i = 0; i < NT; i++) tv[i] = tw[2 * (n1 * T + t + i * T * N1)];
    float2 cv = make_float2(0.f, 0.f);
    if (n1 == 0 && t < N1) cv = tw_h[(n2 * t) & (P.PH - 1)];
    const int px = n1 * T + t;
    const float2 wsx = tw[px], wsh = tw[M / 2];
    const uint8_t* src = rgb + ((size_t)img * P.H + (live ? y : 0)) * (size_t)(P.W * 3);
    const bool fastp = live && ((P.W & 3) == 0) && (((uintptr_t)rgb & 3) == 0);
    constexpr int GMAX = (2 * M / 4) / T;
    const int ng = P.W >> 2;
    uint32_t ra[GMAX], rb[GMAX], rc[GMAX];
    if (fastp) {
        const uint32_t* srcw = reinterpret_cast<const uint32_t*>(src);
#pragma unroll
        for (int i = 0; i < GMAX; i++) {
            const int g = imin(t + i * T, ng - 1);
            ra[i] = srcw[3 * g]; rb[i] = srcw[3 * g + 1]; rc[i] = srcw[3 * g + 2];
        }
    }
#pragma unroll
    for (int i = 0; i < NT; i++) ltw[n1 * T + t + i * T * N1] = tv[i];
    if (n1 == 0 && t < N1) lwc[t] = cv;
    if (fastp) {
        const float s0 = (P.center && (y & 1)) ? -1.0f : 1.0f, s1 = P.center ? -s0 : s0;
#pragma unroll
        for (int i = 0; i < GMAX; i++) {
            const int g = t + i * T;
            if (g < ng) {
                float v0, v1, v2, v3;
                plane_samples4(ra[i], rb[i], rc[i], plane, P.bias, v0, v1, v2, v3);
                lds[lay.idx(2 * g, n1)] = make_float2(s0 * v0, s1 * v1);
                lds[lay.idx(2 * g + 1, n1)] = make_float2(s0 * v2, s1 * v3);
            }
        }
        for (int m = (P.W >> 1) + t; m < M; m += T) lds[lay.idx(m, n1)] = make_float2(0.f, 0.f);
    } else if (live) {
        for (int n = t; n < 2 * M; n += T) {
            float v = 0.0f;
            if (n < P.W) { v = (float)src[3 * n + plane] - P.bias; if (P.center && ((n + y) & 1)) v = -v; }
            ldsf[2 * lay.idx(n >> 1, n1) + (n & 1)] = v;
        }
    }
    lds_barrier();
    if constexpr (T == 64) {
        if (live) {
            float2 u[E];
#pragma unroll
            for (int m = 0; m < E; m++) u[m] = lds[lay.idx(t + m * T, n1)];
            WaveSync::sync();
            fft_block_lazy<M, E, +1, WaveSync>(u, lds, lay, t, n1, ltw, 1);
#pragma unroll
            for (int m = 0; m < E; m++) lds[lay.idx(t + m * T, n1)] = u[m];
        } else {
#pragma unroll
            for (int m = 0; m < E; m++) lds[lay.idx(t + m * T, n1)] = make_float2(0.f, 0.f);
        }
    } else {
        float2 u[E];
        if (live) {
#pragma unroll
            for (int m = 0; m < E; m++) u[m] = lds[lay.idx(t + m * T, n1)];
        }
        Sync::sync();
        fft_block_lazy<M, E, +1, Sync>(u, lds, lay, t, n1, ltw, 1, live);
#pragma unroll
        for (int m = 0; m < E; m++) lds[lay.idx(t + m * T, n1)] = live ? u[m] : make_float2(0.f, 0.f);
    }
    lds_barrier();

    static_assert(T * N1 == M / 2, "one column pair per thread");
    float2 wc[N1];
#pragma unroll
    for (int k1 = 0; k1 < N1; k1++) wc[k1] = lwc[k1];
    float2* dst = out + (size_t)img * P.img_stride + (size_t)plane * P.PH * M + (size_t)n2 * M;
    const int xa = px, xb = (px == 0) ? M / 2 : M - px;
    float2 va[N1], vb[N1];
#pragma unroll
    for (int r = 0; r < N1; r++) {
        const float2 zk = lds[lay.idx(xa, r)], zm = lds[lay.idx((M - xa) & (M - 1), r)];
        rsplit_fwd(zk, zm, wsx, va[r], vb[r]);
        if (px == 0) {
            va[r] = make_float2(va[r].x, vb[r].x);
            const float2 zh = lds[lay.idx(M / 2, r)];
            const float2 ah = make_float2(zh.x, 0.0f), dh = make_float2(0.0f, 2.0f * zh.y);
            const float2 odh = make_float2(0.5f * dh.y, -0.5f * dh.x);
            vb[r] = cadd(ah, cmul(wsh, odh));
        }
    }
    DftReg<N1, +1, 0, N1>::run(va);
    DftReg<N1, +1, 0, N1>::run(vb);
#pragma unroll
    for (int k1 = 0; k1 < N1; k1++) {
        dst[(size_t)k1 * N2 * M + xa] = cmul(va[bitrev(k1, LOGN1)], wc[k1]);
        dst[(size_t)k1 * N2 * M + xb] = cmul(vb[bitrev(k1, LOGN1)], wc[k1]);
    }
}

template <int LOGM, int NL>
__global__ void __launch_bounds__((1 << (LOGM - 4)) * NL) k_rowcol_fwd_live(const uint8_t* __restrict__ rgb, float2* __restrict__ out,
                             const float2* __restrict__ tw, const float2* __restrict__ tw_h, RowParams P, int n2_lo, int n2_cnt) {
    constexpr int M = 1 << LOGM, E = 16, T = M / E, N1 = 8, NTHR = T * NL;
    constexpr bool LTW = (LOGM <= 10);
    constexpr int NPAIR = ((M / 2) + NTHR - 1) / NTHR;
    using Sync = typename std::conditional<T == 64, WaveSync, BlockSync>::type;
    const int t = threadIdx.x, n1 = threadIdx.y, tid = n1 * T + t;
    const int N2 = P.PH >> 3;
    int n2, plane;
    xcd_plane_order(n2_cnt, n2, plane);
    n2 += n2_lo;
    const int img = blockIdx.y;
    const int y = n1 * N2 + n2;
    float2* lds = reinterpret_cast<float2*>(tfft_smem);
    float* ldsf = reinterpret_cast<float*>(tfft_smem);
    LayRows lay{LayRows::padded(M)};
    const bool live = y < P.H;
    float2* ltw = lds + (size_t)NL * lay.pitch;
    float2* lwc = ltw + (LTW ? M : 0);

    constexpr int NT = LTW ? (M + NTHR - 1) / NTHR : 1;
    float2 tv[NT];
    if (LTW) {
#pragma unroll
        for (int i = 0; i < NT; i++) tv[i] = tw[2 * imin(tid + i * NTHR, M - 1)];
    }
    float2 cv = make_float2(0.f, 0.f);
    if (tid < N1) cv = tw_h[(n2 * tid) & (P.PH - 1)];
    float2 wsx[NPAIR];
#pragma unroll
    for (int i = 0; i < NPAIR; i++) wsx[i] = tw[imin(tid + i * NTHR, M / 2)];
    const float2 wsh = tw[M / 2];
    const uint8_t* src = rgb + ((size_t)img * P.H + (live ? y : 0)) * (size_t)(P.W * 3);
    const bool fastp = live && ((P.W & 3) == 0) && (((uintptr_t)rgb & 3) == 0);
    constexpr int GMAX = (2 * M / 4) / T;
    const int ng = P.W >> 2;
    uint32_t ra[GMAX], rb[GMAX], rc[GMAX];
    if (fastp) {
        const uint32_t* srcw = reinterpret_cast<const uint32_t*>(src);
#pragma unroll
        for (int i = 0; i < GMAX; i++) {
            const int g = imin(t + i * T, ng - 1);
            ra[i] = srcw[3 * g]; rb[i] = srcw[3 * g + 1]; rc[i] = srcw[3 * g + 2];
        }
    }
    if (LTW) {
#pragma unroll
        for (int i = 0; i < NT; i++) if (tid + i * NTHR < M) ltw[tid + i * NTHR] = tv[i];
    }
    if (tid < N1) lwc[tid] = cv;
    if (fastp) {
        const float s0 = (P.center && (y & 1)) ? -1.0f : 1.0f, s1 = P.center ? -s0 : s0;
#pragma unroll
        for (int i = 0; i < GMAX; i++) {
            const int g = t + i * T;
            if (g < ng) {
// ... 2 lines not shown
                lds[lay.idx(2 * g, n1)] = make_float2(s0 * v0, s1 * v1);
                lds[lay.idx(2 * g + 1, n1)] = make_float2(s0 * v2, s1 * v3);
            }
        }
        for (int m = (P.W >> 1) + t; m < M; m += T) lds[lay.idx(m, n1)] = make_float2(0.f, 0.f);
    } else if (live) {
        for (int n = t; n < 2 * M; n += T) {
            float v = 0.0f;
            if (n < P.W) { v = (float)src[3 * n + plane] - P.bias; if (P.center && ((n + y) & 1)) v = -v; }
            ldsf[2 * lay.idx(n >> 1, n1) + (n & 1)] = v;
        }
    }
    lds_barrier();
    {
        float2 u[E];
        if (live) {
#pragma unroll
            for (int m = 0; m < E; m++) u[m] = lds[lay.idx(t + m * T, n1)];
        }
        Sync::sync();
        if (LTW) fft_block_lazy<M, E, +1, Sync>(u, lds, lay, t, n1, ltw, 1, live);
        else fft_block_lazy<M, E, +1, Sync>(u, lds, lay, t, n1, tw, 2, live);
#pragma unroll
        for (int m = 0; m < E; m++) lds[lay.idx(t + m * T, n1)] = live ? u[m] : make_float2(0.f, 0.f);
    }
    lds_barrier();

    float2 wc[N1];
#pragma unroll
    for (int k1 = 0; k1 < N1; k1++) wc[k1] = lwc[k1];
    float2* dst = out + (size_t)img * P.img_stride + (size_t)plane * P.PH * M + (size_t)n2 * M;
#pragma unroll
    for (int i = 0; i < NPAIR; i++) {
        const int px = tid + i * NTHR;
        if (px >= M / 2) break;
        const int xa = px, xb = (px == 0) ? M / 2 : M - px;
        float2 va[N1], vb[N1];
#pragma unroll
        for (int r = 0; r < N1; r++) {
            if (r < NL) {
                const float2 zk = lds[lay.idx(xa, r)], zm = lds[lay.idx((M - xa) & (M - 1), r)];
                rsplit_fwd(zk, zm, wsx[i], va[r], vb[r]);
                if (px == 0) {
                    va[r] = make_float2(va[r].x, vb[r].x);
                    const float2 zh = lds[lay.idx(M / 2, r)];
                    const float2 ah = make_float2(zh.x, 0.0f), dh = make_float2(0.0f, 2.0f * zh.y);
                    const float2 odh = make_float2(0.5f * dh.y, -0.5f * dh.x);
                    vb[r] = cadd(ah, cmul(wsh, odh));
                }
            } else {
                va[r] = make_float2(0.f, 0.f); vb[r] = make_float2(0.f, 0.f);
            }
        }
        DftReg<N1, +1, 0, N1>::run(va);
        DftReg<N1, +1, 0, N1>::run(vb);
#pragma unroll
        for (int k1 = 0; k1 < N1; k1++) {
            dst[(size_t)k1 * N2 * M + xa] = cmul(va[bitrev(k1, 3)], wc[k1]);
            dst[(size_t)k1 * N2 * M + xb] = cmul(vb[bitrev(k1, 3)], wc[k1]);
        }
    }
}

__device__ __forceinline__ uint32_t cover_word(const uint8_t* p) {
    return *reinterpret_cast<const uint32_t*>(reinterpret_cast<uintptr_t>(p) & ~(uintptr_t)3);
}
__device__ __forceinline__ unsigned cover_pick(uint32_t w, const uint8_t* p) {
    return (w >> (8u * (unsigned)(reinterpret_cast<uintptr_t>(p) & 3))) & 255u;
}
__device__ __forceinline__ unsigned quantise_u8(float v) {
    v = fminf(fmaxf(v, 0.0f), 255.0f);
    const float r = truncf(v);
    return (unsigned)r + ((v - r >= 0.5f) ? 1u : 0u);
}

template <int LOGN1, int LOGM>
__global__ void __launch_bounds__(1 << (LOGM - 4 + LOGN1)) k_colrow_inv(const float2* __restrict__ in, uint8_t* __restrict__ rgb,
                             const float2* __restrict__ tw, RowParams P) {
    constexpr int M = 1 << LOGM, E = 16, T = M / E, N1 = 1 << LOGN1;
    using Sync = typename std::conditional<T == 64, WaveSync, BlockSync>::type;
    const int t = threadIdx.x, n1 = threadIdx.y;
    const int N2 = P.PH >> LOGN1;
    int n2, plane;
    xcd_plane_order(N2, n2, plane);
    const int img = blockIdx.y;
    const int y = n1 * N2 + n2;
    float2* lds = reinterpret_cast<float2*>(tfft_smem);
    float* ldsf = reinterpret_cast<float*>(tfft_smem);
    LayRows lay{LayRows::padded(M)};

    float2* ltw = lds + (size_t)N1 * lay.pitch;
    constexpr int NT = M / (T * N1);
    float2 tv[NT];
#pragma unroll
    for (int i = 0; i < NT; i++) tv[i] = tw[2 * (n1 * T + t + i * T * N1)];

    static_assert(T * N1 == M / 2, "one column pair per thread");
    const int px = n1 * T + t;
    const int xa = px, xb = (px == 0) ? M / 2 : M - px;
    const float2 wsx = tw[px], wsh = tw[M / 2];
    const float2* src = in + (size_t)img * P.img_stride + (size_t)plane * P.PH * M + (size_t)n2 * M;
    const size_t pix0 = ((size_t)img * P.H + y) * (size_t)P.W * 3 + plane;
    const uint8_t* cov = P.cover ? P.cover + pix0 : nullptr;
    const bool cov4 = cov && (P.W & 3) == 0 && (reinterpret_cast<uintptr_t>(P.cover) & 3) == 0;
    uint32_t cw[2 * E];
    auto load_cover = [&]() {
        if (cov4) {
            const uint32_t* row = reinterpret_cast<const uint32_t*>(cov - plane);
            const int last = (P.W >> 2) - 1;
#pragma unroll
            for (int i = 0; i < E / 2; i++) {
                const int q = imin(t + i * T, last);
                cw[3 * i] = row[3 * q]; cw[3 * i + 1] = row[3 * q + 1]; cw[3 * i + 2] = row[3 * q + 2];
            }
        } else {
            const int last = (P.W >> 1) - 1;
#pragma unroll
            for (int i = 0; i < E; i++) {
                const uint8_t* a = cov + 6 * imin(t + i * T, last);
                cw[2 * i] = cover_word(a);
                cw[2 * i + 1] = cover_word(a + 3);
            }
        }
    };
    float2 va[N1], vb[N1];
#pragma unroll
    for (int k1 = 0; k1 < N1; k1++) { va[k1] = src[(size_t)k1 * N2 * M + xa]; vb[k1] = src[(size_t)k1 * N2 * M + xb]; }
    if (T == 64 && y < P.H && cov && (P.W & 1) == 0) load_cover();
    DftReg<N1, -1, 0, N1>::run(va);
    DftReg<N1, -1, 0, N1>::run(vb);
#pragma unroll
    for (int r = 0; r < N1; r++) {
        if (r * N2 + n2 >= P.H) continue;
        const float2 xk = va[bitrev(r, LOGN1)], xm = vb[bitrev(r, LOGN1)];
        if (px == 0) {
            lds[lay.idx(0, r)] = make_float2(0.5f * (xk.x + xk.y), 0.5f * (xk.x - xk.y));
            const float2 od = cmul(make_float2(0.0f, xm.y), cconj(wsh));
            lds[lay.idx(M / 2, r)] = make_float2(xm.x - od.y, 0.0f + od.x);
        } else {
            float2 za, zb;
            rsplit_inv(xk, xm, wsx, za, zb);
            lds[lay.idx(xa, r)] = za;
            lds[lay.idx(xb, r)] = zb;
        }
    }
#pragma unroll
    for (int i = 0; i < NT; i++) ltw[n1 * T + t + i * T * N1] = tv[i];
    lds_barrier();
    const bool live = y < P.H;
    if constexpr (T == 64) {
        if (!live) return;
        WaveSync::sync();
        float2 u[E];
#pragma unroll
        for (int m = 0; m < E; m++) u[m] = lds[lay.idx(t + m * T, n1)];
        WaveSync::sync();
        fft_block_lazy<M, E, -1, WaveSync>(u, lds, lay, t, n1, ltw, 1);
#pragma unroll
        for (int m = 0; m < E; m++) lds[lay.idx(t + m * T, n1)] = cscale(u[m], P.scale);
        WaveSync::sync();
    } else {
        float2 u[E];
        if (live) {
#pragma unroll
            for (int m = 0; m < E; m++) u[m] = lds[lay.idx(t + m * T, n1)];
        }
        Sync::sync();
        fft_block_lazy<M, E, -1, Sync>(u, lds, lay, t, n1, ltw, 1, live);
        if (live) {
#pragma unroll
            for (int m = 0; m < E; m++) lds[lay.idx(t + m * T, n1)] = cscale(u[m], P.scale);
        }
        Sync::sync();
        if (!live) return;
    }

    uint8_t* dst = rgb + pix0;
    if ((P.W & 1) == 0) {
        const float s0 = (P.center && (y & 1)) ? -1.0f : 1.0f, s1 = P.center ? -s0 : s0;
        if (cov && T != 64) load_cover();
        if (cov4) {
            const unsigned sh = 8u * (unsigned)plane;
#pragma unroll
            for (int i = 0; i < E / 2; i++) {
                const int q = t + i * T;
                if (q < (P.W >> 2)) {
                    const uint32_t w0 = cw[3 * i], w1 = cw[3 * i + 1], w2 = cw[3 * i + 2];
                    const uint32_t x0 = w0, x1 = (w0 >> 24) | (w1 << 8), x2 = (w1 >> 16) | (w2 << 16), x3 = w2 >> 8;
                    const float2 va = lds[lay.idx(2 * q, n1)], vb = lds[lay.idx(2 * q + 1, n1)];
                    uint8_t* d = dst + 12 * q;
                    d[0] = (uint8_t)quantise_u8(s0 * va.x + (float)((x0 >> sh) & 255u));
                    d[3] = (uint8_t)quantise_u8(s1 * va.y + (float)((x1 >> sh) & 255u));
                    d[6] = (uint8_t)quantise_u8(s0 * vb.x + (float)((x2 >> sh) & 255u));
                    d[9] = (uint8_t)quantise_u8(s1 * vb.y + (float)((x3 >> sh) & 255u));
                }
            }
        } else if (cov) {
#pragma unroll
            for (int i = 0; i < E; i++) {
                const int m = t + i * T;
                if (m < (P.W >> 1)) {
                    const float2 v = lds[lay.idx(m, n1)];
                    {
                    dst[6 * m] = (uint8_t)quantise_u8(s0 * v.x + (float)cover_pick(cw[2 * i], cov + 6 * m));
                    dst[6 * m + 3] = (uint8_t)quantise_u8(s1 * v.y + (float)cover_pick(cw[2 * i + 1], cov + 6 * m + 3));
                    }
                }
            }
        } else {
            for (int m = t; m < (P.W >> 1); m += T) {
                const float2 v = lds[lay.idx(m, n1)];
                dst[6 * m] = (uint8_t)quantise_u8(s0 * v.x + P.bias);
                dst[6 * m + 3] = (uint8_t)quantise_u8(s1 * v.y + P.bias);
            }
        }
    } else {
        for (int n = t; n < P.W; n += T) {
            float v = ldsf[2 * lay.idx(n >> 1, n1) + (n & 1)];
            if (P.center && ((n + y) & 1)) v = -v;
            dst[3 * n] = (uint8_t)quantise_u8(v + (cov ? (float)cov[3 * n] : P.bias));
        }
    }
}

template <int LOGM, int PPB>
__global__ void __launch_bounds__((1 << LOGM) / rows_elems(LOGM) * PPB) TFFT_WAVES_PER_EU(LOGM >= TFFT_ROWS_LAZY_LOG ? 4 : 1)
k_rows_inv(const float2* __restrict__ in, uint8_t* __restrict__ rgb, const float2* __restrict__ tw,
                           RowParams P) {
    constexpr int M = 1 << LOGM, E = rows_elems(LOGM), T = M / E;
    const int t = threadIdx.x, pb = threadIdx.y;
    int y = blockIdx.x, plane0 = blockIdx.y * PPB;
    if (PPB == 1) xcd_plane_order(P.H, y, plane0);
    const int img = blockIdx.z;
    const int tid = pb * T + t, nthr = T * PPB;
    float2* lds = reinterpret_cast<float2*>(tfft_smem);
    float* ldsf = reinterpret_cast<float*>(tfft_smem);
    LayRows lay{LayRows::padded(M)};
    using Sync = typename std::conditional<T == 64, WaveSync, BlockSync>::type;

    const float2* src = in + (size_t)img * P.img_stride + ((size_t)(plane0 + pb) * P.PH + y) * M;
    constexpr int NSPLIT = (M / 2) / T + 1;
    float2 xk[NSPLIT], xm[NSPLIT], wk[NSPLIT];
#pragma unroll
    for (int j = 0; j < NSPLIT; j++) {
        const int k = imin(t + j * T, M / 2);
        xk[j] = src[k]; xm[j] = src[(M - k) & (M - 1)]; wk[j] = tw[k];
    }
    constexpr bool LAZY = LOGM >= TFFT_ROWS_LAZY_LOG;
    float2 W[LAZY ? 1 : tw_regs<M, E>()];
    if (!LAZY) fft_prefetch_twiddles<M, E, -1>(W, t, tw, 2);
#pragma unroll
    for (int j = 0; j < NSPLIT; j++) {
        const int k = t + j * T;
        if (k <= M / 2) {
            const int k2 = (M - k) & (M - 1);
            float2 zk, zk2;
            rsplit_inv(xk[j], xm[j], wk[j], zk, zk2);
            if (k == 0) zk = make_float2(0.5f * (xk[j].x + xk[j].y), 0.5f * (xk[j].x - xk[j].y));
            lds[lay.idx(k, pb)] = zk;
            if (k2 != k) lds[lay.idx(k2, pb)] = zk2;
        }
    }
    Sync::sync();
    float2 u[E];
#pragma unroll
    for (int m = 0; m < E; m++) u[m] = lds[lay.idx(t + m * T, pb)];
    Sync::sync();
    if (LAZY) fft_block_lazy<M, E, -1, Sync>(u, lds, lay, t, pb, tw, 2);
    else fft_block<M, E, -1, Sync>(u, lds, lay, t, pb, W);
#pragma unroll
    for (int m = 0; m < E; m++) lds[lay.idx(t + m * T, pb)] = cscale(u[m], P.scale);
    lds_barrier();

    const int nbytes = P.W * 3;
    const size_t row0 = ((size_t)img * P.H + y) * (size_t)nbytes;
    uint8_t* dst = rgb + row0;
    const uint8_t* cov = P.cover ? P.cover + row0 : nullptr;
    const bool fast = (PPB == 3) && ((P.W & 3) == 0) && (((uintptr_t)rgb & 3) == 0) && (((uintptr_t)P.cover & 3) == 0);
    if (fast) {
        const float s0 = (P.center && (y & 1)) ? -1.0f : 1.0f, s1 = P.center ? -s0 : s0;
        uint32_t* dstw = reinterpret_cast<uint32_t*>(dst);
        const uint32_t* covw = reinterpret_cast<const uint32_t*>(cov);
        constexpr int NG = imax(1, (M / 2 + T * PPB - 1) / (T * PPB));
        uint32_t cw[3 * NG];
        if (covw) {
#pragma unroll
            for (int i = 0; i < NG; i++) {
                const int g = imin(tid + i * nthr, (P.W >> 2) - 1);
                cw[3 * i] = covw[3 * g]; cw[3 * i + 1] = covw[3 * g + 1]; cw[3 * i + 2] = covw[3 * g + 2];
            }
        }
#pragma unroll
        for (int gi = 0; gi < NG; gi++) {
            const int g = tid + gi * nthr;
            if (g >= (P.W >> 2)) break;
            const int i0 = lay.idx(2 * g, 0), i1 = lay.idx(2 * g + 1, 0);
            const float2 r01 = lds[i0], r23 = lds[i1], g01 = lds[i0 + lay.pitch], g23 = lds[i1 + lay.pitch],
                         b01 = lds[i0 + 2 * lay.pitch], b23 = lds[i1 + 2 * lay.pitch];
            float zR0, zG0, zB0, zR1, zG1, zB1, zR2, zG2, zB2, zR3, zG3, zB3;
            if (covw) {
                const uint32_t c0 = cw[3 * gi], c1 = cw[3 * gi + 1], c2 = cw[3 * gi + 2];
                zR0 = (float)(c0 & 255u); zG0 = (float)((c0 >> 8) & 255u); zB0 = (float)((c0 >> 16) & 255u); zR1 = (float)(c0 >> 24);
                zG1 = (float)(c1 & 255u); zB1 = (float)((c1 >> 8) & 255u); zR2 = (float)((c1 >> 16) & 255u); zG2 = (float)(c1 >> 24);
                zB2 = (float)(c2 & 255u); zR3 = (float)((c2 >> 8) & 255u); zG3 = (float)((c2 >> 16) & 255u); zB3 = (float)(c2 >> 24);
            } else {
                zR0 = zG0 = zB0 = zR1 = zG1 = zB1 = zR2 = zG2 = zB2 = zR3 = zG3 = zB3 = P.bias;
            }
            const unsigned R0 = quantise_u8(s0 * r01.x + zR0), R1 = quantise_u8(s1 * r01.y + zR1), R2 = quantise_u8(s0 * r23.x + zR2), R3 = quantise_u8(s1 * r23.y + zR3);
// ... 32 lines not shown
                    cv[2 * i] = cover_word(a);
                    cv[2 * i + 1] = cover_word(a + 3);
                }
            }
#pragma unroll
            for (int i = 0; i < NP; i++) {
                const int m = tid + i * nthr;
                if (m >= (P.W >> 1)) break;
                const float2 v = lds[lay.idx(m, 0)];
                d1[6 * m] = (uint8_t)quantise_u8(s0 * v.x + (cov ? (float)cover_pick(cv[2 * i], cov + plane0 + 6 * m) : P.bias));
                d1[6 * m + 3] = (uint8_t)quantise_u8(s1 * v.y + (cov ? (float)cover_pick(cv[2 * i + 1], cov + plane0 + 6 * m + 3) : P.bias));
            }
        } else {
            for (int n = tid; n < P.W; n += nthr) dst[3 * n + plane0] = (uint8_t)get(3 * n + plane0);
        }
    }
}

__device__ __forceinline__ unsigned opaque_u32(unsigned v) {
#if defined(__HIPCC__)
    asm volatile("" : "+v"(v));
#endif
    return v;
}
constexpr int cols_threads(int logl) { return imax(256, 16 * ((1 << logl) / elems_for(1 << logl))); }
__device__ __forceinline__ int read_bit_value(float2 v, const EmbedParams& P, int p, const float* __restrict__ jitter, uint64_t j);

enum { COLS_PLAIN = 0, COLS_ROWLIMIT = 1, COLS_READ = 2, COLS_EMBED = 3, COLS_EMIT = 4, COLS_STAT = 5, COLS_EMBED_D = 6 };
constexpr bool embed_mode(int mode) { return mode == COLS_EMBED || mode == COLS_EMBED_D; }
__device__ __forceinline__ unsigned wave_rank_of(unsigned long long m) {
    return __builtin_amdgcn_mbcnt_hi((unsigned)(m >> 32), __builtin_amdgcn_mbcnt_lo((unsigned)m, 0u));
}
__device__ __forceinline__ unsigned frame_bit(const uint8_t* __restrict__ header, const uint8_t* __restrict__ payload, uint64_t i);
template <int LOGL, int SIGN, int MODE = COLS_PLAIN, bool DC = false, bool TW = false, bool FULL = false, bool PH = false, bool PI = false>
__global__ void __launch_bounds__(cols_threads(LOGL)) TFFT_WAVES_PER_EU((MODE == COLS_EMIT && TFFT_COLS_PFEMIT) ? 1 : (FULL ? TFFT_COLS_WAVES(LOGL) : imin(2, TFFT_COLS_WAVES(LOGL)))) k_fft_cols(const float2* in, float2* out, const float2* __restrict__ tw,
                           ColParams P) {
    constexpr int L = 1 << LOGL, E = elems_for(L), T = L / E, C = 16;
    const int c = threadIdx.x, t = threadIdx.y, gl = threadIdx.z;
    const int g = (MODE == COLS_PLAIN && SIGN > 0 && FULL && P.g_step > 1) ? (int)(blockIdx.y * blockDim.z + gl) * P.g_step + P.g_off
                                                                            : (int)(blockIdx.y * blockDim.z + gl);
    const int img = blockIdx.z / 3, plane = blockIdx.z - 3 * img;
    const size_t plane_off = (size_t)img * P.img_stride + (size_t)plane * P.plane_stride;
    float2* lds = reinterpret_cast<float2*>(tfft_smem) + (size_t)gl * L * C;
    LayColumns lay{C};

    if (MODE == COLS_PLAIN && SIGN > 0 && P.gate) {
        const SelectState* gs = P.gate + 3 * img;
        if (gs[0].fast && gs[1].fast && gs[2].fast && gs[0].n_amb <= TFFT_AMB_CAP && gs[1].n_amb <= TFFT_AMB_CAP && gs[2].n_amb <= TFFT_AMB_CAP) return;
    }
    const int ts = (MODE == COLS_PLAIN && SIGN > 0 && P.tile_step > 1) ? P.tile_step : 1;
    const int toff = ts > 1 ? P.tile_off : 0;
    const int tile0 = blockIdx.x * P.tiles_per_block;
    const int ntiles = ((P.M + C - 1) / C - toff + ts - 1) / ts;
    const int tile1 = (tile0 + P.tiles_per_block < ntiles) ? tile0 + P.tiles_per_block : ntiles;
    const int rows_in_max = P.in_a * (L - 1) + P.in_b * (P.G - 1);
    const bool in_full = (rows_in_max < P.in_rows) && (P.M % C == 0) && (P.G % (int)blockDim.z == 0);
    const unsigned voff_in = (unsigned)((P.in_a * t + P.in_b * g) * P.M + c) * 8u;
    const size_t stride_in = (size_t)P.in_a * T * P.M * sizeof(float2);
    const char* in_bytes = reinterpret_cast<const char*>(in + plane_off);
    const int oM = ts > 1 ? P.out_M : P.M;
    const unsigned voff_out = (unsigned)((P.out_a * t + P.out_b * g) * oM + c) * 8u;
    const size_t stride_out = (size_t)P.out_a * T * oM * sizeof(float2);
    char* out_bytes = reinterpret_cast<char*>(out + (ts > 1 ? (size_t)img * P.out_img_stride + (size_t)plane * P.out_plane_stride : plane_off));
    char* m2_bytes = reinterpret_cast<char*>(reinterpret_cast<float*>(out + (size_t)img * P.img_stride) + (size_t)plane * P.plane_stride);
    auto load_tile = [&](int tile, float2 (&v)[E]) {
        if (in_full) {
            const char* tb = in_bytes + (size_t)(imin(tile, ntiles - 1) * ts + toff) * (C * sizeof(float2));
            const unsigned vo = opaque_u32(voff_in);
#pragma unroll
            for (int m = 0; m < E; m++) v[m] = *reinterpret_cast<const float2*>(tb + m * stride_in + vo);
        } else {
            const int col = imin((tile * ts + toff) * C + c, P.M - 1);
            const float2* src = in + plane_off;
            const int gc = imin(g, P.G - 1), to = (int)opaque_u32((unsigned)t);
#pragma unroll
            for (int m = 0; m < E; m++) {
                const int row = imin(P.in_a * (to + m * T) + P.in_b * gc, P.in_rows - 1);
                v[m] = src[(unsigned)(row * P.M + col)];
            }
        }
    };
    auto tile_mask = [&](int tile, float2 (&v)[E]) {
        if (in_full) return;
        const bool active = ((tile * ts + toff) * C + c < P.M) && (g < P.G);
#pragma unroll
        for (int m = 0; m < E; m++) {
            const int row = P.in_a * (t + m * T) + P.in_b * g;
            if (!(active && row < P.in_rows)) v[m] = make_float2(0.f, 0.f);
        }
    };
    constexpr bool PF = (LOGL <= TFFT_COLS_PF_MAXLOG || (MODE == COLS_EMIT && TFFT_COLS_PFEMIT)) && !embed_mode(MODE);
    float2 u[E], un[E];
    float2 awc = make_float2(0.f, 0.f), awn = make_float2(0.f, 0.f);
    auto load_aw = [&](int tile) -> float2 { const int col = (tile * ts + toff) * C + c; return (DC && col < P.M) ? P.dc_aw[col] : make_float2(0.f, 0.f); };
    if (PF) { load_tile(tile0, u); awc = load_aw(tile0); }
    const int out_rows = (MODE == COLS_ROWLIMIT) ? imin(P.out_rows, *P.last_row_dev + 1) : P.out_rows;
    float2* lds_ah = reinterpret_cast<float2*>(tfft_smem) + (size_t)blockDim.z * L * C + (size_t)gl * L;
    float2* lds_wo = reinterpret_cast<float2*>(tfft_smem) + (size_t)blockDim.z * L * (C + (DC ? 1 : 0)) + (size_t)gl * L;
    if (DC) {
        for (int k = t * C + c; k < L; k += T * C) {
            const int row = (SIGN > 0) ? P.out_a * k + P.out_b * g : P.in_a * k + P.in_b * g;
            lds_ah[k] = (g < P.G && row < P.PH) ? P.dc_ah[row] : make_float2(0.f, 0.f);
        }
    }
    if (TW) {
        for (int k = t * C + c; k < L; k += T * C) lds_wo[k] = twload<SIGN>(tw, (k * g) & (P.PH - 1));
    }
// ... 540 lines not shown
                       const float* __restrict__ jitter, EmbedParams P, uint8_t* __restrict__ bits_out,
                       int* __restrict__ err) {
    const uint64_t i = (uint64_t)blockIdx.x * blockDim.x + threadIdx.x;
    if (i >= P.n) return;
    const int img = blockIdx.y;
    spec += (size_t)img * P.img_stride;
    bits_out += (size_t)img * P.n;
    bins += (size_t)img * P.bins_stride;
    if (jitter) jitter += (size_t)img * P.bins_stride;
    const tfft_bin bn = bins[i];
    const uint64_t j = P.bit_index ? (uint64_t)P.bit_index[i] : i;
    const int x = bn.x, y = bn.y, p = bn.plane;
    if (p > 2 || x >= P.PW || y >= P.PH || x == 0 || y == 0 || 2 * x == P.PW || 2 * y == P.PH) {
        atomicOr(err, 1);
        bits_out[j] = 0;
        return;
    }
    const BinRef r = locate(p, y, x, P.PH, P.PW);
    float2 v = spec[r.idx];
    if (r.conj) v = cconj(v);
    bits_out[j] = (uint8_t)read_bit_value(v, P, p, jitter, j);
}

__device__ __forceinline__ bool tile_bin_of(const tfft_bin bn, int PH, int PW, int G, unsigned& bucket, TileBin& tb) {
    const int x = bn.x, y = bn.y, p = bn.plane;
    if (p > 2 || x >= PW || y >= PH || x == 0 || y == 0 || 2 * x == PW || 2 * y == PH) return false;
    const int M = PW >> 1, ntiles = (M + 15) >> 4;
    const bool conj = x > M;
    const int xs = conj ? PW - x : x, ys = conj ? ((PH - y) & (PH - 1)) : y;
    const int g = ys % G;
    bucket = (unsigned)((p * G + g) * ntiles + (xs >> 4));
    tb.k = (uint16_t)(ys / G); tb.c = (uint8_t)(xs & 15); tb.conj = conj ? 1 : 0; tb.bit = 0;
    return true;
}
constexpr unsigned BUCKET_LCAP = 8192;
__device__ __forceinline__ bool bucket_span(const tfft_bin* __restrict__ bins, uint64_t lo, uint64_t hi, int PH, int PW, int G,
                                            unsigned* mm, unsigned& bmin, unsigned& width, int* err) {
    if (threadIdx.x == 0) { mm[0] = 0xFFFFFFFFu; mm[1] = 0u; }
    __syncthreads();
    unsigned tmin = 0xFFFFFFFFu, tmax = 0u;
    for (uint64_t i = lo + threadIdx.x; i < hi; i += blockDim.x) {
        unsigned b; TileBin tb;
        if (tile_bin_of(bins[i], PH, PW, G, b, tb)) { tmin = b < tmin ? b : tmin; tmax = b > tmax ? b : tmax; }
        else if (err) atomicOr(err, 1);
    }
    if (tmin <= tmax) { atomicMin(&mm[0], tmin); atomicMax(&mm[1], tmax); }
    __syncthreads();
    bmin = mm[0];
    const unsigned bmax = mm[1];
    width = (bmin <= bmax) ? bmax - bmin + 1 : 0;
    return width > 0 && width <= BUCKET_LCAP;
}
__global__ void k_bucket_count(const tfft_bin* __restrict__ bins, uint64_t n, int PH, int PW, int G, unsigned* __restrict__ cnt,
                               int* __restrict__ err, int force_global) {
    unsigned* lc = reinterpret_cast<unsigned*>(tfft_smem);
    unsigned* mm = lc + BUCKET_LCAP;
    const uint64_t per = (n + gridDim.x - 1) / gridDim.x, lo = (uint64_t)blockIdx.x * per, hi = (lo + per < n) ? lo + per : n;
    unsigned bmin, width;
    const bool local = bucket_span(bins, lo, hi, PH, PW, G, mm, bmin, width, err) && !force_global;
    if (local) {
        for (unsigned i = threadIdx.x; i < width; i += blockDim.x) lc[i] = 0;
        __syncthreads();
    }
    for (uint64_t i = lo + threadIdx.x; i < hi; i += blockDim.x) {
        unsigned b; TileBin tb;
        if (tile_bin_of(bins[i], PH, PW, G, b, tb)) atomicAdd(local ? &lc[b - bmin] : &cnt[b], 1u);
    }
    if (local) {
        __syncthreads();
        for (unsigned i = threadIdx.x; i < width; i += blockDim.x) if (lc[i]) atomicAdd(&cnt[bmin + i], lc[i]);
    }
}
__global__ void k_bucket_scan_a(unsigned* __restrict__ cnt, unsigned* __restrict__ off, unsigned* __restrict__ totals, int nb) {
    unsigned* sh = reinterpret_cast<unsigned*>(tfft_smem);
    const int t = threadIdx.x, i = blockIdx.x * 1024 + t;
    const unsigned v = (i < nb) ? cnt[i] : 0u;
    if (i < nb) cnt[i] = 0;
    sh[t] = v;
    __syncthreads();
    for (int d = 1; d < 1024; d <<= 1) {
        const unsigned a = (t >= d) ? sh[t - d] : 0u;
        __syncthreads();
        sh[t] += a;
        __syncthreads();
    }
    if (i < nb) off[i] = sh[t] - v;
    if (t == 1023) totals[blockIdx.x] = sh[t];
}
__global__ void k_bucket_scan_b(unsigned* __restrict__ totals, int nblk, unsigned* __restrict__ off, int nb) {
    unsigned* sh = reinterpret_cast<unsigned*>(tfft_smem);
    const int t = threadIdx.x;
    const unsigned v = (t < nblk) ? totals[t] : 0u;
    sh[t] = v;
    __syncthreads();
    for (int d = 1; d < 1024; d <<= 1) {
        const unsigned a = (t >= d) ? sh[t - d] : 0u;
        __syncthreads();
        sh[t] += a;
        __syncthreads();
    }
    if (t < nblk) totals[t] = sh[t] - v;
    if (t == 1023) off[nb] = sh[t];
}
__global__ void k_bucket_scan_c(unsigned* __restrict__ off, const unsigned* __restrict__ totals, int nb) {
    const int i = blockIdx.x * 1024 + threadIdx.x;
    if (i < nb) off[i] += totals[blockIdx.x];
}
__global__ void k_bucket_fill(const tfft_bin* __restrict__ bins, const uint32_t* __restrict__ bit_index, uint64_t n, int PH, int PW,
                              int G, unsigned* __restrict__ cursor, const unsigned* __restrict__ off, TileBin* __restrict__ out,
                              int force_global) {
    unsigned* lc = reinterpret_cast<unsigned*>(tfft_smem);
    unsigned* mm = lc + BUCKET_LCAP;
    const uint64_t per = (n + gridDim.x - 1) / gridDim.x, lo = (uint64_t)blockIdx.x * per, hi = (lo + per < n) ? lo + per : n;
    unsigned bmin, width;
    const bool local = bucket_span(bins, lo, hi, PH, PW, G, mm, bmin, width, nullptr) && !force_global;
    if (local) {
        for (unsigned i = threadIdx.x; i < width; i += blockDim.x) lc[i] = 0;
        __syncthreads();
        for (uint64_t i = lo + threadIdx.x; i < hi; i += blockDim.x) {
            unsigned b; TileBin tb;
            if (tile_bin_of(bins[i], PH, PW, G, b, tb)) atomicAdd(&lc[b - bmin], 1u);
        }
        __syncthreads();
        for (unsigned i = threadIdx.x; i < width; i += blockDim.x) {
            const unsigned k = lc[i];
            if (k) lc[i] = off[bmin + i] + atomicAdd(&cursor[bmin + i], k);
        }
        __syncthreads();
    }
    for (uint64_t i = lo + threadIdx.x; i < hi; i += blockDim.x) {
        unsigned b; TileBin tb;
        if (!tile_bin_of(bins[i], PH, PW, G, b, tb)) continue;
        tb.bit = bit_index ? bit_index[i] : (uint32_t)i;
        const unsigned pos = local ? atomicAdd(&lc[b - bmin], 1u) : off[b] + atomicAdd(&cursor[b], 1u);
        out[pos] = tb;
    }
}

__global__ void k_bucket_count_walks(const tfft_bin* __restrict__ bins, uint64_t n, int chunks, int PH, int PW, int G, unsigned nb,
                                     unsigned* __restrict__ cnt, int* __restrict__ err) {
    unsigned* lc = reinterpret_cast<unsigned*>(tfft_smem);
    const int img = blockIdx.x / chunks, ch = blockIdx.x - img * chunks, nimg = gridDim.x / chunks;
    const uint64_t per = (n + chunks - 1) / chunks, lo = (uint64_t)ch * per, hi = (lo + per < n) ? lo + per : n;
    const bool local = nb + 1 <= BUCKET_LCAP;
    const tfft_bin* b0 = bins + (size_t)img * n;
    unsigned* gc = cnt + (size_t)img * nb;
    unsigned* gbad = cnt + (size_t)nimg * nb;
    if (local) {
        for (unsigned i = threadIdx.x; i <= nb; i += blockDim.x) lc[i] = 0;
        __syncthreads();
    }
    for (uint64_t i = lo + threadIdx.x; i < hi; i += blockDim.x) {
        unsigned b; TileBin tb;
        if (!tile_bin_of(b0[i], PH, PW, G, b, tb)) { atomicOr(err, 1); b = nb; }
        atomicAdd(local ? &lc[b] : (b < nb ? &gc[b] : gbad), 1u);
    }
    if (local) {
        __syncthreads();
        for (unsigned i = threadIdx.x; i <= nb; i += blockDim.x) if (lc[i]) atomicAdd(i < nb ? &gc[i] : gbad, lc[i]);
    }
}
__global__ void k_bucket_fill_walks(const tfft_bin* __restrict__ bins, uint64_t n, int chunks, int PH, int PW, int G, unsigned nb,
                                    unsigned* __restrict__ cursor, const unsigned* __restrict__ off, TileBin* __restrict__ out) {
    unsigned* lc = reinterpret_cast<unsigned*>(tfft_smem);
    const int img = blockIdx.x / chunks, ch = blockIdx.x - img * chunks, nimg = gridDim.x / chunks;
    const uint64_t per = (n + chunks - 1) / chunks, lo = (uint64_t)ch * per, hi = (lo + per < n) ? lo + per : n;
    const bool local = nb + 1 <= BUCKET_LCAP;
    const tfft_bin* b0 = bins + (size_t)img * n;
    auto gidx = [&](unsigned b) -> size_t { return b < nb ? (size_t)img * nb + b : (size_t)nimg * nb; };
    if (local) {
        for (unsigned i = threadIdx.x; i <= nb; i += blockDim.x) lc[i] = 0;
        __syncthreads();
        for (uint64_t i = lo + threadIdx.x; i < hi; i += blockDim.x) {
            unsigned b; TileBin tb;
            if (!tile_bin_of(b0[i], PH, PW, G, b, tb)) b = nb;
            atomicAdd(&lc[b], 1u);
        }
        __syncthreads();
        for (unsigned i = threadIdx.x; i <= nb; i += blockDim.x) {
            const unsigned k = lc[i];
            if (k) lc[i] = off[gidx(i)] + atomicAdd(&cursor[gidx(i)], k);
        }
        __syncthreads();
    }
    for (uint64_t i = lo + threadIdx.x; i < hi; i += blockDim.x) {
        unsigned b; TileBin tb;
        if (!tile_bin_of(b0[i], PH, PW, G, b, tb)) { b = nb; tb.k = 0; tb.c = 0; tb.conj = 0; }
        tb.bit = (uint32_t)i;
        const unsigned pos = local ? atomicAdd(&lc[b], 1u) : off[gidx(b)] + atomicAdd(&cursor[gidx(b)], 1u);
        out[pos] = tb;
    }
}
__global__ void k_gather_bits_walks(const TileBin* __restrict__ ent, const uint8_t* __restrict__ bits, const uint8_t* __restrict__ hdr,
                                    const uint8_t* __restrict__ pay, uint64_t plen, uint64_t n, uint64_t limit, uint64_t total,
// ... 847 lines not shown
    const uint8_t* p = bits + img * n_bins + 912 + k * 56;
    unsigned v = 0;
    for (int q = 0; q < 8; q++, p += 7)
        v = (v << 1) | ((p[0] + p[1] + p[2] + p[3] + p[4] + p[5] + p[6]) >= 4 ? 1u : 0u);
    payload[img * max_plen + k] = (uint8_t)v;
}

hipError_t launch_frame_expand(const uint8_t* header, const uint8_t* payload, uint64_t plen, int n_images, uint8_t* bits,
                               uint64_t stride, hipStream_t s) {
    const uint64_t n = 38ull * 24 + plen * 56;
    if (stride < n) return hipErrorInvalidValue;
    hipLaunchKernelGGL(k_frame_expand, dim3((unsigned)((n / 4 + 255) / 256), n_images), dim3(256), 0, s, header, payload, plen, bits, stride);
    return hipGetLastError();
}
hipError_t launch_frame_majority(const uint8_t* bits, uint64_t plen, int n_images, uint8_t* header, uint8_t* payload,
                                 hipStream_t s) {
    hipLaunchKernelGGL(k_frame_majority, dim3((unsigned)((38 + plen + 255) / 256), n_images), dim3(256), 0, s, bits, plen, header, payload);
    return hipGetLastError();
}
hipError_t launch_stream_decode(const uint8_t* bits, uint64_t n_bins, uint64_t max_plen, int n_images, uint8_t* header, uint8_t* payload,
                                int* status, unsigned* plen, hipStream_t s) {
    if (n_images == 0) return hipSuccess;
    hipLaunchKernelGGL(k_stream_header, dim3(n_images), dim3(64), 64, s, bits, n_bins, max_plen, header, status, plen);
    if (max_plen)
        hipLaunchKernelGGL(k_stream_payload, dim3((unsigned)((max_plen + 255) / 256), n_images), dim3(256), 0, s, bits, n_bins, max_plen, plen, payload);
    return hipGetLastError();
}

#define TFFT_DISPATCH_LOG(n, F)                                                                   \
    switch (n) {                                                                                  \
        case 0: F(0); break; case 1: F(1); break; case 2: F(2); break; case 3: F(3); break;       \
        case 4: F(4); break; case 5: F(5); break; case 6: F(6); break; case 7: F(7); break;       \
        case 8: F(8); break; case 9: F(9); break; case 10: F(10); break; case 11: F(11); break;   \
        case 12: F(12); break; case 13: F(13); break;                                             \
        default: return hipErrorInvalidValue;                                                     \
    }

constexpr int rows_ppb(int logm) { return logm <= 10 ? 3 : 1; }

template <int LOGM, int PPB, bool FWD>
static hipError_t launch_rows_t(const void* in, void* out, const float2* tw, const RowParams& P, int n_images,
                                hipStream_t s) {
    constexpr int M = 1 << LOGM, E = rows_elems(LOGM), T = M / E;
    const size_t lds = (size_t)PPB * LayRows::padded(M) * sizeof(float2);
    dim3 grid(PPB == 1 ? P.H * 3 : P.H, PPB == 1 ? 1 : 3 / PPB, n_images), block(T, PPB, 1);
    if (FWD) {
        auto k = k_rows_fwd<LOGM, PPB>;
        if (lds > 48 * 1024) {
            hipError_t e = hipFuncSetAttribute((const void*)k, hipFuncAttributeMaxDynamicSharedMemorySize, (int)lds);
            if (e != hipSuccess) return e;
        }
        hipLaunchKernelGGL(k, grid, block, lds, s, (const uint8_t*)in, (float2*)out, tw, P);
    } else {
        auto k = k_rows_inv<LOGM, PPB>;
        if (lds > 48 * 1024) {
            hipError_t e = hipFuncSetAttribute((const void*)k, hipFuncAttributeMaxDynamicSharedMemorySize, (int)lds);
            if (e != hipSuccess) return e;
        }
        hipLaunchKernelGGL(k, grid, block, lds, s, (const float2*)in, (uint8_t*)out, tw, P);
    }
    return hipGetLastError();
}

hipError_t launch_rows_fwd(const uint8_t* rgb, float2* out, const float2* tw_pw, const RowParams& P, int n_images,
                           hipStream_t s) {
    const int logm = ilog2(P.PW >> 1);
#define F(n) return launch_rows_t<n, rows_ppb(n), true>(rgb, out, tw_pw, P, n_images, s)
    TFFT_DISPATCH_LOG(logm, F)
#undef F
    return hipSuccess;
}
template <int LOGM>
static hipError_t launch_rowcol_fwd_t(const uint8_t* rgb, float2* out, const float2* tw_pw, const float2* tw_ph, const RowParams& P,
                                      int n_images, hipStream_t s) {
    constexpr int LOGN1 = 3, M = 1 << LOGM;
    const size_t lds = ((size_t)(1 << LOGN1) * LayRows::padded(M) + M + (1 << LOGN1)) * sizeof(float2);
    auto k = k_rowcol_fwd<LOGN1, LOGM>;
    hipError_t e = hipFuncSetAttribute((const void*)k, hipFuncAttributeMaxDynamicSharedMemorySize, (int)lds);
    if (e != hipSuccess) return e;
    hipLaunchKernelGGL(k, dim3((P.PH >> LOGN1) * 3, n_images), dim3(M / 16, 1 << LOGN1), lds, s, rgb, out, tw_pw, tw_ph, P);
    return hipGetLastError();
}
hipError_t launch_rowcol_fwd(const uint8_t* rgb, float2* out, const float2* tw_pw, const float2* tw_ph, const RowParams& P,
                             int n_images, hipStream_t s) {
    if (P.PW == 2048) return launch_rowcol_fwd_t<10>(rgb, out, tw_pw, tw_ph, P, n_images, s);
    if (P.PW == 4096) return launch_rowcol_fwd_t<11>(rgb, out, tw_pw, tw_ph, P, n_images, s);
    return hipErrorInvalidValue;
}
template <int LOGM>
static hipError_t launch_colrow_inv_t(const float2* in, uint8_t* rgb, const float2* tw_pw, const RowParams& P, int n_images, hipStream_t s) {
    constexpr int LOGN1 = 3, M = 1 << LOGM;
    const size_t lds = ((size_t)(1 << LOGN1) * LayRows::padded(M) + M) * sizeof(float2);
    auto k = k_colrow_inv<LOGN1, LOGM>;
    hipError_t e = hipFuncSetAttribute((const void*)k, hipFuncAttributeMaxDynamicSharedMemorySize, (int)lds);
    if (e != hipSuccess) return e;
    hipLaunchKernelGGL(k, dim3((P.PH >> LOGN1) * 3, n_images), dim3(M / 16, 1 << LOGN1), lds, s, in, rgb, tw_pw, P);
    return hipGetLastError();
}
hipError_t launch_colrow_inv(const float2* in, uint8_t* rgb, const float2* tw_pw, const RowParams& P, int n_images, hipStream_t s) {
    if (P.PW == 2048) return launch_colrow_inv_t<10>(in, rgb, tw_pw, P, n_images, s);
    if (P.PW == 4096) return launch_colrow_inv_t<11>(in, rgb, tw_pw, P, n_images, s);
    return hipErrorInvalidValue;
}
template <int LOGM, int NL>
static hipError_t launch_fwd_live_t(const uint8_t* in, float2* out, const float2* tw_pw, const float2* tw_ph, const RowParams& P, int n_images,
                                    int n2_lo, int n2_cnt, hipStream_t s) {
    constexpr int M = 1 << LOGM;
    const size_t lds = ((size_t)NL * LayRows::padded(M) + (LOGM <= 10 ? M : 0) + 8) * sizeof(float2);
    auto k = k_rowcol_fwd_live<LOGM, NL>;
    hipError_t e = hipFuncSetAttribute((const void*)k, hipFuncAttributeMaxDynamicSharedMemorySize, (int)lds);
    if (e != hipSuccess) return e;
    hipLaunchKernelGGL(k, dim3(n2_cnt * 3, n_images), dim3(M / 16, NL), lds, s, in, out, tw_pw, tw_ph, P, n2_lo, n2_cnt);
    return hipGetLastError();
}
template <int LOGM>
static hipError_t launch_fwd_live_nl(int nl, const uint8_t* in, float2* out, const float2* tw_pw, const float2* tw_ph, const RowParams& P, int n_images,
                                     int n2_lo, int n2_cnt, hipStream_t s) {
    switch (nl) {
        case 4: return launch_fwd_live_t<LOGM, 4>(in, out, tw_pw, tw_ph, P, n_images, n2_lo, n2_cnt, s);
        case 5: return launch_fwd_live_t<LOGM, 5>(in, out, tw_pw, tw_ph, P, n_images, n2_lo, n2_cnt, s);
        case 6: return launch_fwd_live_t<LOGM, 6>(in, out, tw_pw, tw_ph, P, n_images, n2_lo, n2_cnt, s);
        case 7: return launch_fwd_live_t<LOGM, 7>(in, out, tw_pw, tw_ph, P, n_images, n2_lo, n2_cnt, s);
        default: return launch_fwd_live_t<LOGM, 8>(in, out, tw_pw, tw_ph, P, n_images, n2_lo, n2_cnt, s);
    }
}
hipError_t launch_rowcol_fwd_live(const uint8_t* rgb, float2* out, const float2* tw_pw, const float2* tw_ph, const RowParams& P, int n_images, hipStream_t s) {
    const int N2 = P.PH >> 3, hi = P.H / N2, rem = P.H % N2;
    hipError_t e = hipSuccess;
    for (int part = 0; part < 2 && e == hipSuccess; part++) {
        const int lo = part ? rem : 0, cnt = part ? N2 - rem : rem;
        int nl = part ? hi : hi + 1;
        if (cnt == 0) continue;
        if (nl < 4) nl = 4;
        if (nl > 8) nl = 8;
        if (P.PW == 2048) e = launch_fwd_live_nl<10>(nl, rgb, out, tw_pw, tw_ph, P, n_images, lo, cnt, s);
        else if (P.PW == 4096) e = launch_fwd_live_nl<11>(nl, rgb, out, tw_pw, tw_ph, P, n_images, lo, cnt, s);
        else e = hipErrorInvalidValue;
    }
    return e;
}
hipError_t launch_rows_inv(const float2* in, uint8_t* rgb, const float2* tw_pw, const RowParams& P, int n_images,
                           hipStream_t s) {
    const int logm = ilog2(P.PW >> 1);
#define F(n) return launch_rows_t<n, rows_ppb(n), false>(in, rgb, tw_pw, P, n_images, s)
    TFFT_DISPATCH_LOG(logm, F)
#undef F
    return hipSuccess;
}

template <int LOGL, int SIGN, int MODE = COLS_PLAIN, bool DC = false, bool TW = false, bool FULL = false, bool PH = false, bool PI = false>
static hipError_t launch_cols_t(const float2* in, float2* out, const float2* tw, const ColParams& P, int n_planes,
                                hipStream_t s) {
    constexpr int L = 1 << LOGL, E = elems_for(L), T = L / E, C = 16;
    const bool gsample = (MODE == COLS_PLAIN && SIGN > 0 && P.hist_sel && P.g_step > 1);
    const int Geff = gsample ? (P.G - P.g_off + P.g_step - 1) / P.g_step : P.G;
    int gpb = 256 / (T * C);
    if (gpb < 1) gpb = 1;
    if (gpb > Geff) gpb = Geff;
    if constexpr (!FULL && (LOGL >= 6 || MODE == COLS_STAT || (MODE == COLS_PLAIN && SIGN > 0 && !TW)) && MODE != COLS_ROWLIMIT) {
        const int rows_out_max = P.out_a * (L - 1) + P.out_b * (P.G - 1);
        if ((LOGL >= 6 || MODE == COLS_STAT || P.hist_sel) && rows_out_max < P.out_rows && P.M % C == 0 && Geff % gpb == 0)
            return launch_cols_t<LOGL, SIGN, MODE, DC, TW, true, PH, PI>(in, out, tw, P, n_planes, s);
// ... 48 lines not shown
         : (P.em_on && P.st_sel) ? GW(n, COLS_STAT, false) : P.em_on ? GW(n, COLS_EMIT, false)                            \
         : P.em_jp ? GW(n, COLS_READ, true) : GW(n, COLS_READ, false)
    TFFT_DISPATCH_LOG(logl, F)
#undef F
#undef GW
#undef L_
    return hipSuccess;
}
hipError_t launch_cols(const float2* in, float2* out, const float2* tw_ph, const ColParams& P, int logl, int sign,
                       int n_planes, hipStream_t s) {
    if (logl > 9) return hipErrorInvalidValue;
    if ((P.last_row_dev || (P.rd_bins && !P.em_on)) && sign < 0) return hipErrorInvalidValue;
    if (P.em_on && (!P.rd_bins || (sign < 0 && P.dc_ah) || (sign > 0 && P.last_row_dev))) return hipErrorInvalidValue;
    if (P.tw_out && sign > 0 && (P.dc_ah || P.rd_bins || P.last_row_dev)) return hipErrorInvalidValue;
    if (P.em_on && !P.em_fl) return hipErrorInvalidValue;
    if (P.rd_bins && !P.trash) return hipErrorInvalidValue;
    if (P.st_sel && (!P.em_on || sign < 0 || logl > 9 || logl < 4 || !P.st_cand || !P.st_col0 || (P.st_cap && (!P.st_partial || !P.st_amb)))) return hipErrorInvalidValue;
    if ((P.tile_step > 1 || P.gate) && (sign < 0 || P.rd_bins || P.last_row_dev || P.tw_out)) return hipErrorInvalidValue;
    if (P.em_m2 && sign > 0 && (!P.em_on || !P.st_col0)) return hipErrorInvalidValue;
    if ((P.em_jp || P.em_med) && !((sign < 0 && P.em_on) || (sign > 0 && P.rd_bins && !P.em_on))) return hipErrorInvalidValue;
    if (P.em_med && sign > 0) return hipErrorInvalidValue;
    if (P.em_dsrc && !(sign < 0 && P.em_on && P.rd_walks && !P.em_jp && !P.em_med)) return hipErrorInvalidValue;
    const bool phase = P.em_jp || P.em_med;
    if (P.rd_walks) return launch_cols_walks(in, out, tw_ph, P, logl, sign, n_planes, s);
#define G(n, MODE)                                                                      \
    (P.dc_ah ? launch_cols_t<(n <= 9 ? n : 9), +1, MODE, true>(in, out, tw_ph, P, n_planes, s) \
             : launch_cols_t<(n <= 9 ? n : 9), +1, MODE, false>(in, out, tw_ph, P, n_planes, s))
#define GI(n, DCF)                                                                      \
    (P.tw_out ? launch_cols_t<(n <= 9 ? n : 9), -1, COLS_PLAIN, DCF, true>(in, out, tw_ph, P, n_planes, s) \
              : launch_cols_t<(n <= 9 ? n : 9), -1, COLS_PLAIN, DCF, false>(in, out, tw_ph, P, n_planes, s))
#define GE(n)                                                                      \
    (phase ? (P.tw_out ? launch_cols_t<(n <= 9 ? n : 9), -1, COLS_EMBED, false, true, false, true>(in, out, tw_ph, P, n_planes, s) \
                       : launch_cols_t<(n <= 9 ? n : 9), -1, COLS_EMBED, false, false, false, true>(in, out, tw_ph, P, n_planes, s)) \
           : P.tw_out ? launch_cols_t<(n <= 9 ? n : 9), -1, COLS_EMBED, false, true>(in, out, tw_ph, P, n_planes, s) \
                      : launch_cols_t<(n <= 9 ? n : 9), -1, COLS_EMBED, false, false>(in, out, tw_ph, P, n_planes, s))
#define GR(n)                                                                      \
    (!P.em_jp ? G(n, COLS_READ)                                                    \
              : P.dc_ah ? launch_cols_t<(n <= 9 ? n : 9), +1, COLS_READ, true, false, false, true>(in, out, tw_ph, P, n_planes, s) \
                        : launch_cols_t<(n <= 9 ? n : 9), +1, COLS_READ, false, false, false, true>(in, out, tw_ph, P, n_planes, s))
#define F(n)                                                                            \
    return sign < 0 ? (P.em_on ? GE(n) : P.dc_ah ? GI(n, true) : GI(n, false)) \
         : P.tw_out ? launch_cols_t<(n <= 9 ? n : 9), +1, COLS_PLAIN, false, true>(in, out, tw_ph, P, n_planes, s) \
         : (P.em_on && P.st_sel) ? G(n, COLS_STAT) : P.em_on ? G(n, COLS_EMIT) : P.rd_bins ? GR(n) : P.last_row_dev ? G(n, COLS_ROWLIMIT) : G(n, COLS_PLAIN)
    TFFT_DISPATCH_LOG(logl, F)
#undef F
#undef G
#undef GI
#undef GE
#undef GR
    return hipSuccess;
}

hipError_t launch_bucket_bins(const tfft_bin* bins, const uint32_t* bit_index, uint64_t n, int PH, int PW, int G,
                              unsigned* cnt, unsigned* off, TileBin* out, int* err, int force_global, hipStream_t s) {
    const int M = PW >> 1, ntiles = (M + 15) >> 4, nb = 3 * ntiles * G;
    hipError_t e = hipMemsetAsync(cnt, 0, (size_t)nb * sizeof(unsigned), s);
    if (e != hipSuccess) return e;
    unsigned blocks = (unsigned)((n + 2047) / 2048);
    if (blocks < 1) blocks = 1;
    if (blocks > 4096) blocks = 4096;
    const size_t lds = (BUCKET_LCAP + 2) * sizeof(unsigned);
    hipLaunchKernelGGL(k_bucket_count, dim3(blocks), dim3(256), lds, s, bins, n, PH, PW, G, cnt, err, force_global);
    const int nblk = (nb + 1023) / 1024;
    if (nblk > 1024) return hipErrorInvalidValue;
    unsigned* totals = off + nb + 1;
    hipLaunchKernelGGL(k_bucket_scan_a, dim3(nblk), dim3(1024), 1024 * sizeof(unsigned), s, cnt, off, totals, nb);
    hipLaunchKernelGGL(k_bucket_scan_b, dim3(1), dim3(1024), 1024 * sizeof(unsigned), s, totals, nblk, off, nb);
    hipLaunchKernelGGL(k_bucket_scan_c, dim3(nblk), dim3(1024), 0, s, off, totals, nb);
    hipLaunchKernelGGL(k_bucket_fill, dim3(blocks), dim3(256), lds, s, bins, bit_index, n, PH, PW, G, cnt, off, out, force_global);
    return hipGetLastError();
}
hipError_t launch_bucket_walks(const tfft_bin* bins, uint64_t n, int n_images, int PH, int PW, int G, unsigned* cnt, unsigned* off, TileBin* out,
                               int* err, hipStream_t s) {
    if (n == 0 || n_images <= 0) return hipErrorInvalidValue;
    const int M = PW >> 1, ntiles = (M + 15) >> 4;
    const unsigned nb = 3u * (unsigned)ntiles * (unsigned)G, nbi = nb + 1;
    const uint64_t nbt = (uint64_t)nb * (uint64_t)n_images + 1;
    if (nbt > 1024ull * 1024ull || (uint64_t)n * (uint64_t)n_images > 0xFFFFFFFFull) return hipErrorInvalidValue;
    hipError_t e = hipMemsetAsync(cnt, 0, (size_t)nbt * sizeof(unsigned), s);
    if (e != hipSuccess) return e;
    int chunks = (int)((n + 8191) / 8192);
    if (chunks < 1) chunks = 1;
    if ((uint64_t)chunks * (uint64_t)n_images > 65535ull) chunks = 65535 / n_images > 0 ? 65535 / n_images : 1;
    const size_t lds = nbi <= BUCKET_LCAP ? (size_t)nbi * sizeof(unsigned) : 16;
    hipLaunchKernelGGL(k_bucket_count_walks, dim3((unsigned)(chunks * n_images)), dim3(256), lds, s, bins, n, chunks, PH, PW, G, nb, cnt, err);
    const int nblk = (int)((nbt + 1023) / 1024);
    unsigned* totals = off + nbt + 1;
    hipLaunchKernelGGL(k_bucket_scan_a, dim3(nblk), dim3(1024), 1024 * sizeof(unsigned), s, cnt, off, totals, (int)nbt);
    hipLaunchKernelGGL(k_bucket_scan_b, dim3(1), dim3(1024), 1024 * sizeof(unsigned), s, totals, nblk, off, (int)nbt);
    hipLaunchKernelGGL(k_bucket_scan_c, dim3(nblk), dim3(1024), 0, s, off, totals, (int)nbt);
    hipLaunchKernelGGL(k_bucket_fill_walks, dim3((unsigned)(chunks * n_images)), dim3(256), lds, s, bins, n, chunks, PH, PW, G, nb, cnt, off, out);
    return hipGetLastError();
}
hipError_t launch_gather_bits_walks(const TileBin* ent, const uint8_t* bits, const uint8_t* hdr, const uint8_t* pay, uint64_t plen, uint64_t n,
                                    uint64_t limit, int n_images, uint8_t* out, hipStream_t s) {
    if (n == 0 || n_images <= 0) return hipSuccess;
    const uint64_t total = n * (uint64_t)n_images;
    hipLaunchKernelGGL(k_gather_bits_walks, dim3((unsigned)((total + 255) / 256)), dim3(256), 0, s, ent, bits, hdr, pay, plen, n, limit, total, out);
    return hipGetLastError();
}
hipError_t launch_gather_jitter_walks(const TileBin* ent, const float* jitter, uint64_t n, int n_images, float2* out, hipStream_t s) {
    if (n == 0 || n_images <= 0) return hipSuccess;
    const uint64_t total = n * (uint64_t)n_images;
    hipLaunchKernelGGL(k_gather_jitter_walks, dim3((unsigned)((total + 255) / 256)), dim3(256), 0, s, ent, jitter, n, total, out);
    return hipGetLastError();
}
hipError_t launch_fit_init(const TileBin* ent, const float2* fl, const uint8_t* pb, const float2* jp, const tfft_bin* bins, const float* med,
                           uint64_t n, int n_images, double alpha, double tau, double mu_floor, float2* d, float* mu, hipStream_t s) {
    if (n == 0 || n_images <= 0) return hipSuccess;
    const uint64_t total = n * (uint64_t)n_images;
    hipLaunchKernelGGL(k_fit_init, dim3((unsigned)((total + 255) / 256)), dim3(256), 0, s, ent, fl, pb, jp, bins, med, n, total, (float)alpha,
                       (float)cos(alpha), (float)sin(alpha), (float)tau, (float)mu_floor, d, mu);
    return hipGetLastError();
}
hipError_t launch_fit_count(const TileBin* ent, const float2* fl, const uint8_t* pb, const float2* jp, const float* mu, uint64_t n, int n_images,
                            unsigned nblk, unsigned* partial, unsigned* counts, uint32_t* wrong_out, hipStream_t s) {
    if (n == 0 || n_images <= 0 || nblk == 0) return hipSuccess;
    hipLaunchKernelGGL(k_fit_count, dim3(nblk, (unsigned)n_images), dim3(256), 2 * sizeof(unsigned), s, ent, fl, pb, jp, mu, n, partial);
    hipError_t e = hipGetLastError();
    if (e != hipSuccess) return e;
    hipLaunchKernelGGL(k_fit_sum, dim3((unsigned)n_images), dim3(64), 0, s, partial, nblk, counts, wrong_out);
    return hipGetLastError();
}
hipError_t launch_fit_correct(const TileBin* ent, const float2* fl, const uint8_t* pb, const float2* jp, const float* mu, const unsigned* counts,
                              uint64_t n, int n_images, double gain, float2* d, hipStream_t s) {
    if (n == 0 || n_images <= 0) return hipSuccess;
    const uint64_t total = n * (uint64_t)n_images;
    hipLaunchKernelGGL(k_fit_correct, dim3((unsigned)((total + 255) / 256)), dim3(256), 0, s, ent, fl, pb, jp, mu, counts, n, total, (float)gain, d);
    return hipGetLastError();
}
hipError_t launch_gather_bits(const TileBin* ent, const unsigned* n_ent, const uint8_t* bits, const uint8_t* hdr, const uint8_t* pay, uint64_t plen,
                              uint64_t n, uint64_t limit, int n_images, uint8_t* out, hipStream_t s) {
    if (n == 0 || n_images == 0) return hipSuccess;
    hipLaunchKernelGGL(k_gather_bits, dim3((unsigned)((n + 255) / 256), n_images), dim3(256), 0, s, ent, n_ent, bits, hdr, pay, plen, n, limit, out);
    return hipGetLastError();
}
hipError_t launch_gather_jitter(const TileBin* ent, const unsigned* n_ent, const float* jitter, uint64_t n, float2* out, hipStream_t s) {
    if (n == 0) return hipSuccess;
    hipLaunchKernelGGL(k_gather_jitter, dim3((unsigned)((n + 255) / 256)), dim3(256), 0, s, ent, n_ent, jitter, n, out);
    return hipGetLastError();
}
// ... 436 lines not shown
```

Measured before the change: 24690.

## Prune column FFT work beyond highest occupied embed column tile

While bucketing embed bins, the scan kernel records on device the highest column tile that holds any bin (x_lim). Column and fused row/column FFT kernels in the forward-read and inverse-embed paths receive this limit and get template variants that can skip columns past it. ROWS_INV now also carries the embed parameters. The aim is to avoid transforming spectrum columns that hold no payload. It adds an atomicMax in the scan, a device-side limit that must be reset every build, and extra kernel instantiations.

Measured after the change: 24860 (median of 6 runs). No clear change (+0.7%).

```diff
diff --git a/steganosaurus_amd/csrc/tfft_capi.hip b/steganosaurus_amd/csrc/tfft_capi.hip
--- a/steganosaurus_amd/csrc/tfft_capi.hip
+++ b/steganosaurus_amd/csrc/tfft_capi.hip
@@ -67,6 +67,8 @@
     int* err = nullptr;
     uint8_t* trash = nullptr;
     int* last_row = nullptr;
+    int* col_lim = nullptr;
+    int prune_cols = 1;
     struct TileBuckets { float2* fl = nullptr; uint8_t* pb = nullptr; uint64_t fl_cap = 0;
                          unsigned* cnt = nullptr; unsigned* off = nullptr; TileBin* ent = nullptr; uint64_t cap = 0; int nb_cap = 0;
                          const void* built_for = nullptr; uint64_t built_n = 0; int built_ph = 0, built_pw = 0, built_g = 0; const void* built_index = nullptr; bool built_bad = false;
@@ -239,9 +241,12 @@
     ColParams cp{};
     cp.M = M; cp.PH = s.PH; cp.plane_stride = (size_t)s.PH * M; cp.img_stride = c->slot_stride;
     cp.tiles_per_block = c->cols_tiles_per_block;
+    const int* lim_fwd = md.fwd_read ? md.fwd_read->x_lim : nullptr;
+    const int* lim_inv = md.inv_embed ? md.inv_embed->x_lim : nullptr;
     switch (stage) {
         case ROWS_FWD: {
             RowParams rp{s.W, s.H, s.PWi, s.PH, s.center, 0.f, c->slot_stride, c->dc_bias, nullptr};
+            if (pl.fused_fwd) rp.x_lim = lim_fwd;
             if (pl.fused_fwd && c->fuse_live && s.H < s.PH) HIPCHK(c, launch_rowcol_fwd_live(rgb_in, tmp, tw_w, tw_h, rp, n, st));
             else if (pl.fused_fwd) HIPCHK(c, launch_rowcol_fwd(rgb_in, tmp, tw_w, tw_h, rp, n, st));
             else HIPCHK(c, launch_rows_fwd(rgb_in, tmp, tw_w, rp, n, st));
@@ -256,12 +261,13 @@
                 rc = get_dc_table(c, s.H, s.PH, s.center, 0, (double)c->dc_bias, &cp.dc_ah); if (rc) return rc;
                 rc = get_dc_table(c, s.W, s.PWi, s.center, 1, 1.0, &cp.dc_aw); if (rc) return rc;
             }
-                if (md.fwd_read) { const ColParams& r = *md.fwd_read; cp.rd_bins = r.rd_bins; cp.rd_off = r.rd_off; cp.rd_bits = r.rd_bits; cp.rd_n = r.rd_n; cp.em_jp = r.em_jp; cp.rd_walks = r.rd_walks; cp.trash = c->trash; cp.tiles_per_block = c->cols_tiles_read; }
+                if (md.fwd_read) { const ColParams& r = *md.fwd_read; cp.rd_bins = r.rd_bins; cp.rd_off = r.rd_off; cp.rd_bits = r.rd_bits; cp.rd_n = r.rd_n; cp.em_jp = r.em_jp; cp.rd_walks = r.rd_walks; cp.trash = c->trash; cp.tiles_per_block = c->cols_tiles_read; cp.x_lim = lim_fwd; }
                 else if (md.fwd_emit) { copy_embed_fields(cp, *md.fwd_emit, false); if (!c->cols_tiles_forced && pl.log_n2 <= 8) cp.tiles_per_block = 2; if (cp.st_sel && c->cols_tiles_stat) cp.tiles_per_block = c->cols_tiles_stat; }
                 else if (md.fwd_plain_extra) copy_plain_extra(cp, *md.fwd_plain_extra);
                 HIPCHK(c, launch_cols(tmp, md.fwd_out_override ? md.fwd_out_override : spec, tw_h, cp, pl.log_n2, +1, 3 * n, st));
             } else {
                 cp.G = N2; cp.in_a = N2; cp.in_b = 1; cp.out_a = N2; cp.out_b = 1; cp.in_rows = s.H; cp.out_rows = s.PH; cp.tw_out = 1;
+                cp.x_lim = lim_fwd;
                 HIPCHK(c, launch_cols(tmp, tmp, tw_h, cp, pl.log_n1, +1, 3 * n, st));
             }
             return TFFT_OK;
@@ -273,7 +279,7 @@
                 rc = get_dc_table(c, s.H, s.PH, s.center, 0, (double)c->dc_bias, &cp.dc_ah); if (rc) return rc;
                 rc = get_dc_table(c, s.W, s.PWi, s.center, 1, 1.0, &cp.dc_aw); if (rc) return rc;
             }
-            if (md.fwd_read) { const ColParams& r = *md.fwd_read; cp.rd_bins = r.rd_bins; cp.rd_off = r.rd_off; cp.rd_bits = r.rd_bits; cp.rd_n = r.rd_n; cp.em_jp = r.em_jp; cp.rd_walks = r.rd_walks; cp.trash = c->trash; cp.tiles_per_block = c->cols_tiles_read; }
+            if (md.fwd_read) { const ColParams& r = *md.fwd_read; cp.rd_bins = r.rd_bins; cp.rd_off = r.rd_off; cp.rd_bits = r.rd_bits; cp.rd_n = r.rd_n; cp.em_jp = r.em_jp; cp.rd_walks = r.rd_walks; cp.trash = c->trash; cp.tiles_per_block = c->cols_tiles_read; cp.x_lim = lim_fwd; }
             else if (md.fwd_emit) { copy_embed_fields(cp, *md.fwd_emit, false); if (!c->cols_tiles_forced && pl.log_n2 <= 8) cp.tiles_per_block = 2; if (cp.st_sel && c->cols_tiles_stat) cp.tiles_per_block = c->cols_tiles_stat; }
                 else if (md.fwd_plain_extra) copy_plain_extra(cp, *md.fwd_plain_extra);
             HIPCHK(c, launch_cols(tmp, md.fwd_out_override ? md.fwd_out_override : spec, tw_h, cp, pl.log_n2, +1, 3 * n, st));
@@ -281,7 +287,7 @@
         case COLS_INV_A:
             if (pl.direct) {
                 cp.G = 1; cp.in_a = 1; cp.in_b = 0; cp.out_a = 1; cp.out_b = 0; cp.in_rows = s.PH; cp.out_rows = s.H; cp.tw_out = 0;
-                if (md.inv_embed) { copy_embed_fields(cp, *md.inv_embed, true); cp.tiles_per_block = c->cols_tiles_embed ? c->cols_tiles_embed : (pl.log_n2 >= 9 ? 2 : 16); }
+                if (md.inv_embed) { copy_embed_fields(cp, *md.inv_embed, true); cp.tiles_per_block = c->cols_tiles_embed ? c->cols_tiles_embed : (pl.log_n2 >= 9 ? 2 : 16); cp.x_lim = lim_inv; }
                 else if (c->dc_bias != 0.0f) {
                     rc = get_dc_table(c, s.H, s.PH, s.center, 0, (double)c->dc_bias, &cp.dc_ah); if (rc) return rc;
                     rc = get_dc_table(c, s.W, s.PWi, s.center, 1, 1.0, &cp.dc_aw); if (rc) return rc;
@@ -289,7 +295,7 @@
                 HIPCHK(c, launch_cols(spec, md.inv_via_spec ? spec : tmp, tw_h, cp, pl.log_n2, -1, 3 * n, st));
             } else {
                 cp.G = N1; cp.in_a = N1; cp.in_b = 1; cp.out_a = 1; cp.out_b = N2; cp.in_rows = s.PH; cp.out_rows = s.PH; cp.tw_out = 1;
-                if (md.inv_embed) { copy_embed_fields(cp, *md.inv_embed, true); cp.tiles_per_block = c->cols_tiles_embed ? c->cols_tiles_embed : (pl.log_n2 >= 9 ? 2 : 16); }
+                if (md.inv_embed) { copy_embed_fields(cp, *md.inv_embed, true); cp.tiles_per_block = c->cols_tiles_embed ? c->cols_tiles_embed : (pl.log_n2 >= 9 ? 2 : 16); cp.x_lim = lim_inv; }
                 else if (c->dc_bias != 0.0f) {
                     rc = get_dc_table(c, s.H, s.PH, s.center, 0, (double)c->dc_bias, &cp.dc_ah); if (rc) return rc;
                     rc = get_dc_table(c, s.W, s.PWi, s.center, 1, 1.0, &cp.dc_aw); if (rc) return rc;
@@ -300,11 +306,13 @@
         case COLS_INV_B:
             if (pl.direct || pl.fused_fwd) return TFFT_OK;
             cp.G = N2; cp.in_a = N2; cp.in_b = 1; cp.out_a = N2; cp.out_b = 1; cp.in_rows = s.PH; cp.out_rows = s.H; cp.tw_out = 0;
+            cp.x_lim = lim_inv;
             HIPCHK(c, launch_cols(md.inv_via_spec ? spec : tmp, md.inv_via_spec ? spec : tmp, tw_h, cp, pl.log_n1, -1, 3 * n, st));
             return TFFT_OK;
         case ROWS_INV: {
             RowParams rp{s.W, s.H, s.PWi, s.PH, s.center, (float)(1.0 / ((double)M * (double)s.PH)), c->slot_stride, c->dc_bias, nullptr};
             if (md.inv_cover) { rp.cover = md.inv_cover; rp.bias = 0.f; }
+            rp.x_lim = lim_inv;
             if (md.inv_via_spec && !md.inv_embed) return TFFT_E_INVALID;
             if (pl.fused_fwd) HIPCHK(c, launch_colrow_inv(md.inv_via_spec ? spec : tmp, rgb_out, tw_w, rp, n, st));
             else HIPCHK(c, launch_rows_inv(md.inv_via_spec ? spec : tmp, rgb_out, tw_w, rp, n, st));
@@ -546,6 +554,7 @@
     if (const char* e = getenv("TFFT_STATS_SKEW")) c->stats_skew = atoi(e);
     if (const char* e = getenv("TFFT_STREAMS")) c->n_streams = atoi(e);
     if (const char* e = getenv("TFFT_TILE_READ")) c->tile_read = atoi(e);
+    if (const char* e = getenv("TFFT_PRUNE_COLS")) c->prune_cols = atoi(e);
     if (const char* e = getenv("TFFT_DC_BIAS")) c->dc_bias = (float)atof(e);
     if (const char* e = getenv("TFFT_MEDIAN_FALLBACK")) c->median_force_fallback = atoi(e);
     if (const char* e = getenv("TFFT_STATS_FUSED")) c->stats_fused = atoi(e);
@@ -584,6 +593,7 @@
     if (!rc) rc = dev_alloc(c, (void**)&c->err, sizeof(int));
     if (!rc) rc = dev_alloc(c, (void**)&c->trash, 8192);
     if (!rc) rc = dev_alloc(c, (void**)&c->last_row, 2 * sizeof(int));
+    if (!rc) rc = dev_alloc(c, (void**)&c->col_lim, 2 * sizeof(int));
     if (!rc && hipMemset(c->err, 0, sizeof(int)) != hipSuccess) rc = TFFT_E_HIP;
     if (!rc && hipMemset(c->sel, 0, ns * 3 * sizeof(SelectState)) != hipSuccess) rc = TFFT_E_HIP;
     if (!rc && hipDeviceSynchronize() != hipSuccess) rc = TFFT_E_HIP;
@@ -599,7 +609,7 @@
     invalidate_graphs(c);
     (void)hipFree(c->img_pool); (void)hipFree(c->spec_pool); (void)hipFree(c->tmp_pool); (void)hipFree(c->cand_pool);
     (void)hipFree(c->col0_pool);
-    (void)hipFree(c->sel); (void)hipFree(c->med); (void)hipFree(c->partial); (void)hipFree(c->amb); (void)hipFree(c->usable); (void)hipFree(c->err); (void)hipFree(c->ex_cand); (void)hipFree(c->ex_val); (void)hipFree(c->ex_below); (void)hipFree(c->ex_n); for (auto& kv : c->ex_table) (void)hipFree(kv.second); (void)hipFree(c->trash); (void)hipFree(c->bit_index); (void)hipFree(c->last_row); (void)hipFree(c->ph_jit);
+    (void)hipFree(c->sel); (void)hipFree(c->med); (void)hipFree(c->partial); (void)hipFree(c->amb); (void)hipFree(c->usable); (void)hipFree(c->err); (void)hipFree(c->ex_cand); (void)hipFree(c->ex_val); (void)hipFree(c->ex_below); (void)hipFree(c->ex_n); for (auto& kv : c->ex_table) (void)hipFree(kv.second); (void)hipFree(c->trash); (void)hipFree(c->bit_index); (void)hipFree(c->last_row); (void)hipFree(c->col_lim); (void)hipFree(c->ph_jit);
     (void)hipFree(c->fit_d); (void)hipFree(c->fit_mu); (void)hipFree(c->fit_part); (void)hipFree(c->fit_cnt); (void)hipFree(c->fit_iters); (void)hipFree(c->fit_wrong);
     (void)hipFree(c->bx_win); (void)hipFree(c->bx_cand); (void)hipFree(c->bx_below); (void)hipFree(c->bx_n); (void)hipFree(c->bx_idx); (void)hipFree(c->bx_grp);
     (void)hipFree(c->bx_part); (void)hipFree(c->bx_val); (void)hipFree(c->an_buf);
@@ -1303,13 +1313,15 @@
     return TFFT_OK;
 }
 
+static const int* col_limit(const tfft_ctx* c, int which) { return c->prune_cols ? c->col_lim + which : nullptr; }
+
 static int build_buckets(tfft_ctx* c, int which, const tfft_bin* bins, uint64_t n_bits, const Slot& s, int G, hipStream_t st) {
     auto& tb = c->tb[which];
     const bool registered = bins == c->reg_bins && n_bits == c->reg_n;
     if (!(registered && tb.built_for == bins && tb.built_n == n_bits && tb.built_ph == s.PH && tb.built_pw == s.PWi && tb.built_g == G &&
           tb.built_index == c->bit_index)) {
         if (tb.built_for) c->graphs_stale = true;
-        HIPCHK(c, launch_bucket_bins(bins, c->bit_index, n_bits, s.PH, s.PWi, G, tb.cnt, tb.off, tb.ent, c->err, c->tile_read == 2, st));
+        HIPCHK(c, launch_bucket_bins(bins, c->bit_index, n_bits, s.PH, s.PWi, G, tb.cnt, tb.off, tb.ent, c->err, c->col_lim + which, c->tile_read == 2, st));
         tb.built_for = registered ? bins : nullptr; tb.built_n = n_bits; tb.built_ph = s.PH; tb.built_pw = s.PWi; tb.built_g = G; tb.built_index = c->bit_index;
         tb.built_bad = false;
         tb.jp_for = 0;
@@ -1441,7 +1453,7 @@
     auto& tb = c->tb[which];
     if (tb.built_for) c->graphs_stale = true;
     tb.built_for = nullptr; tb.jp_for = 0; tb.row_for = nullptr;
-    HIPCHK(c, launch_bucket_walks(bins, n_bits, g, s.PH, s.PWi, G, tb.cnt, tb.off, tb.ent, c->err, st));
+    HIPCHK(c, launch_bucket_walks(bins, n_bits, g, s.PH, s.PWi, G, tb.cnt, tb.off, tb.ent, c->err, c->col_lim + which, st));
     if (!jit) return TFFT_OK;
     const uint64_t need = (uint64_t)g * n_bits;
     if (need > tb.jp_cap || !tb.jp) {
@@ -1501,6 +1513,7 @@
         auto& tb = c->tb[which];
         em.rd_bins = tb.ent; em.rd_off = tb.off; em.trash = c->trash; em.em_fl = tb.fl + (size_t)s0 * n_bits; em.em_pb = tb.pb + (size_t)s0 * n_bits;
         em.em_n = walks ? 0 : n_bits; em.em_cos = ep.cos_a; em.em_sin = ep.sin_a; em.rd_walks = walks ? 1 : 0;
+        em.x_lim = col_limit(c, which);
         if (!walks) rc = gather_jitter(c, which, n_bits, nb, st);
         if (rc) return rc;
         em.em_jp = jit ? tb.jp : nullptr;
@@ -1616,7 +1629,7 @@
         if (rc) return rc;
         ColParams rd{};
         rd.rd_bins = tb.ent; rd.rd_off = tb.off; rd.rd_bits = bits_out; rd.rd_n = n_bits; rd.trash = c->trash;
-        rd.em_jp = jit ? tb.jp : nullptr; rd.rd_walks = walks ? 1 : 0;
+        rd.em_jp = jit ? tb.jp : nullptr; rd.rd_walks = walks ? 1 : 0; rd.x_lim = col_limit(c, which);
         StageMode md;
         md.fwd_read = &rd;
         rc = enqueue_forward(c, s0, g, rgb_in, st, md);
@@ -2136,6 +2149,7 @@
     const unsigned nblk = (unsigned)std::min<uint64_t>(kFitMaxBlocks, (n_bins + 1023) / 1024);
     ColParams ed{};
     ed.rd_bins = tb.ent; ed.rd_off = tb.off; ed.trash = c->trash; ed.em_fl = c->fit_d; ed.em_pb = tb.pb; ed.em_n = 0; ed.rd_walks = 1; ed.em_dsrc = 1;
+    ed.x_lim = col_limit(c, 0);
     std::vector<unsigned> cnt((size_t)2 * g);
     for (int i = 0; i < g; i++) iters[i] = -1;
     for (int t = 0;; t++) {
@@ -2471,14 +2485,14 @@
             const int G = pl.direct ? 1 : (1 << pl.log_n1), ntiles = (s.PWi / 2 + 15) / 16;
             int rc = ensure_buckets(c, 0, n_bits, 3 * ntiles * G);
             if (rc) return rc;
-            HIPCHK(c, launch_bucket_bins((const tfft_bin*)bins_dev, c->bit_index, n_bits, s.PH, s.PWi, G, c->tb[0].cnt, c->tb[0].off, c->tb[0].ent, c->err, c->tile_read == 2, c->stream));
-            rd.rd_bins = c->tb[0].ent; rd.rd_off = c->tb[0].off; rd.rd_bits = (uint8_t*)bits_out_dev; rd.rd_n = n_bits; rd.trash = c->trash;
+            HIPCHK(c, launch_bucket_bins((const tfft_bin*)bins_dev, c->bit_index, n_bits, s.PH, s.PWi, G, c->tb[0].cnt, c->tb[0].off, c->tb[0].ent, c->err, c->col_lim, c->tile_read == 2, c->stream));
+            rd.rd_bins = c->tb[0].ent; rd.rd_off = c->tb[0].off; rd.rd_bits = (uint8_t*)bits_out_dev; rd.rd_n = n_bits; rd.trash = c->trash; rd.x_lim = col_limit(c, 0);
         } else {
             HIPCHK(c, launch_bins_last_row((const tfft_bin*)bins_dev, n_bits, s.PH, s.PWi, c->last_row, c->stream));
         }
     }
     ColParams em{};
-    if ((stage == COLS_INV_A || stage == final_fwd || stage == EMBED || (stage == MEDIANS && tile)) && delta && bits_dev) {
+    if ((stage == COLS_INV_A || stage == ROWS_INV || stage == final_fwd || stage == EMBED || (stage == MEDIANS && tile)) && delta && bits_dev) {
         if (!index_ok(c, n_bits)) return TFFT_E_STATE;
         const int G = pl.direct ? 1 : (1 << pl.log_n1), ntiles = (s.PWi / 2 + 15) / 16;
         int rc = ensure_buckets(c, 0, n_bits, 3 * ntiles * G, true);
@@ -2487,7 +2501,7 @@
         if (rc) return rc;
         const EmbedParams ep0 = embed_params(c, s, n_bits, alpha, 0, nullptr, false);
         em.rd_bins = c->tb[0].ent; em.rd_off = c->tb[0].off; em.trash = c->trash; em.em_fl = c->tb[0].fl; em.em_pb = c->tb[0].pb; em.em_n = n_bits;
-        em.em_cos = ep0.cos_a; em.em_sin = ep0.sin_a;
+        em.em_cos = ep0.cos_a; em.em_sin = ep0.sin_a; em.x_lim = col_limit(c, 0);
         if (m2) { em.em_m2 = 1; em.st_col0 = c->col0_pool; }
     }
     if (tile) {
@@ -2524,6 +2538,7 @@
                 break;
             case ROWS_INV:
                 { StageMode md; if (delta && rgb_dev) md.inv_cover = (const uint8_t*)rgb_dev;
+                  if (em.rd_bins) md.inv_embed = &em;
                   rc = enqueue_fft_stage(c, 0, n_images, stage, nullptr, (uint8_t*)rgb_out_dev, c->stream, md); }
                 break;
             case COLS_FWD_READ:
diff --git a/steganosaurus_amd/csrc/tfft_kernels.h b/steganosaurus_amd/csrc/tfft_kernels.h
--- a/steganosaurus_amd/csrc/tfft_kernels.h
+++ b/steganosaurus_amd/csrc/tfft_kernels.h
@@ -16,6 +16,7 @@
     size_t img_stride;
     float bias;
     const uint8_t* cover;
+    const int* x_lim;
 };
 
 struct TileBin { uint16_t k; uint8_t c; uint8_t conj; uint32_t bit; };
@@ -58,6 +59,7 @@
     const float2* dc_ah;
     const float2* dc_aw;
     const int* last_row_dev;
+    const int* x_lim;
     int tw_out;
     int tiles_per_block;
     size_t plane_stride;
@@ -159,9 +161,9 @@
 hipError_t audit_fft2d_f64(double2* a, double2* scratch, double2* wtab, int n_planes, int PH, int PW, int inverse, hipStream_t s);
 hipError_t audit_load_rgb8_f64(const uint8_t* rgb_dev, int W, int H, int PW, int PH, int center, double2* out, hipStream_t s);
 hipError_t launch_bucket_bins(const tfft_bin* bins, const uint32_t* bit_index, uint64_t n, int PH, int PW, int G,
-                              unsigned* cnt, unsigned* off, TileBin* out, int* err, int force_global, hipStream_t s);
+                              unsigned* cnt, unsigned* off, TileBin* out, int* err, int* x_lim, int force_global, hipStream_t s);
 hipError_t launch_bucket_walks(const tfft_bin* bins, uint64_t n, int n_images, int PH, int PW, int G, unsigned* cnt, unsigned* off, TileBin* out,
-                               int* err, hipStream_t s);
+                               int* err, int* x_lim, hipStream_t s);
 hipError_t launch_gather_bits_walks(const TileBin* ent, const uint8_t* bits, const uint8_t* hdr, const uint8_t* pay, uint64_t plen, uint64_t n,
                                     uint64_t limit, int n_images, uint8_t* out, hipStream_t s);
 hipError_t launch_gather_jitter_walks(const TileBin* ent, const float* jitter, uint64_t n, int n_images, float2* out, hipStream_t s);
diff --git a/steganosaurus_amd/csrc/tfft_kernels.hip b/steganosaurus_amd/csrc/tfft_kernels.hip
--- a/steganosaurus_amd/csrc/tfft_kernels.hip
+++ b/steganosaurus_amd/csrc/tfft_kernels.hip
@@ -174,10 +174,11 @@
     }
 }
 
-template <int LOGN1, int LOGM>
+template <int LOGN1, int LOGM, bool LIM = false>
 __global__ void __launch_bounds__(1 << (LOGM - 4 + LOGN1)) k_rowcol_fwd(const uint8_t* __restrict__ rgb, float2* __restrict__ out,
                              const float2* __restrict__ tw, const float2* __restrict__ tw_h, RowParams P) {
     constexpr int M = 1 << LOGM, E = 16, T = M / E, N1 = 1 << LOGN1;
+    const int xlim = LIM ? *P.x_lim : M;
     using Sync = typename std::conditional<T == 64, WaveSync, BlockSync>::type;
     const int t = threadIdx.x, n1 = threadIdx.y;
     const int N2 = P.PH >> LOGN1;
@@ -283,6 +284,19 @@
             vb[r] = cadd(ah, cmul(wsh, odh));
         }
     }
+    if (LIM) {
+        if (xa < xlim) {
+            DftReg<N1, +1, 0, N1>::run(va);
+#pragma unroll
+            for (int k1 = 0; k1 < N1; k1++) dst[(size_t)k1 * N2 * M + xa] = cmul(va[bitrev(k1, LOGN1)], wc[k1]);
+        }
+        if (xb < xlim) {
+            DftReg<N1, +1, 0, N1>::run(vb);
+#pragma unroll
+            for (int k1 = 0; k1 < N1; k1++) dst[(size_t)k1 * N2 * M + xb] = cmul(vb[bitrev(k1, LOGN1)], wc[k1]);
+        }
+        return;
+    }
     DftReg<N1, +1, 0, N1>::run(va);
     DftReg<N1, +1, 0, N1>::run(vb);
 #pragma unroll
@@ -292,10 +306,11 @@
     }
 }
 
-template <int LOGM, int NL>
+template <int LOGM, int NL, bool LIM = false>
 __global__ void __launch_bounds__((1 << (LOGM - 4)) * NL) k_rowcol_fwd_live(const uint8_t* __restrict__ rgb, float2* __restrict__ out,
                              const float2* __restrict__ tw, const float2* __restrict__ tw_h, RowParams P, int n2_lo, int n2_cnt) {
     constexpr int M = 1 << LOGM, E = 16, T = M / E, N1 = 8, NTHR = T * NL;
+    const int xlim = LIM ? *P.x_lim : M;
     constexpr bool LTW = (LOGM <= 10);
     constexpr int NPAIR = ((M / 2) + NTHR - 1) / NTHR;
     using Sync = typename std::conditional<T == 64, WaveSync, BlockSync>::type;
@@ -404,6 +419,19 @@
                 va[r] = make_float2(0.f, 0.f); vb[r] = make_float2(0.f, 0.f);
             }
         }
+        if (LIM) {
+            if (xa < xlim) {
+                DftReg<N1, +1, 0, N1>::run(va);
+#pragma unroll
+                for (int k1 = 0; k1 < N1; k1++) dst[(size_t)k1 * N2 * M + xa] = cmul(va[bitrev(k1, 3)], wc[k1]);
+            }
+            if (xb < xlim) {
+                DftReg<N1, +1, 0, N1>::run(vb);
+#pragma unroll
+                for (int k1 = 0; k1 < N1; k1++) dst[(size_t)k1 * N2 * M + xb] = cmul(vb[bitrev(k1, 3)], wc[k1]);
+            }
+            continue;
+        }
         DftReg<N1, +1, 0, N1>::run(va);
         DftReg<N1, +1, 0, N1>::run(vb);
 #pragma unroll
@@ -426,10 +454,11 @@
     return (unsigned)r + ((v - r >= 0.5f) ? 1u : 0u);
 }
 
-template <int LOGN1, int LOGM>
+template <int LOGN1, int LOGM, bool LIM = false>
 __global__ void __launch_bounds__(1 << (LOGM - 4 + LOGN1)) k_colrow_inv(const float2* __restrict__ in, uint8_t* __restrict__ rgb,
                              const float2* __restrict__ tw, RowParams P) {
     constexpr int M = 1 << LOGM, E = 16, T = M / E, N1 = 1 << LOGN1;
+    const int xlim = LIM ? *P.x_lim : M;
     using Sync = typename std::conditional<T == 64, WaveSync, BlockSync>::type;
     const int t = threadIdx.x, n1 = threadIdx.y;
     const int N2 = P.PH >> LOGN1;
@@ -476,8 +505,21 @@
         }
     };
     float2 va[N1], vb[N1];
-#pragma unroll
-    for (int k1 = 0; k1 < N1; k1++) { va[k1] = src[(size_t)k1 * N2 * M + xa]; vb[k1] = src[(size_t)k1 * N2 * M + xb]; }
+    if (LIM) {
+#pragma unroll
+        for (int k1 = 0; k1 < N1; k1++) { va[k1] = make_float2(0.f, 0.f); vb[k1] = make_float2(0.f, 0.f); }
+        if (xa < xlim) {
+#pragma unroll
+            for (int k1 = 0; k1 < N1; k1++) va[k1] = src[(size_t)k1 * N2 * M + xa];
+        }
+        if (xb < xlim) {
+#pragma unroll
+            for (int k1 = 0; k1 < N1; k1++) vb[k1] = src[(size_t)k1 * N2 * M + xb];
+        }
+    } else {
+#pragma unroll
+        for (int k1 = 0; k1 < N1; k1++) { va[k1] = src[(size_t)k1 * N2 * M + xa]; vb[k1] = src[(size_t)k1 * N2 * M + xb]; }
+    }
     if (T == 64 && y < P.H && cov && (P.W & 1) == 0) load_cover();
     DftReg<N1, -1, 0, N1>::run(va);
     DftReg<N1, -1, 0, N1>::run(vb);
@@ -575,7 +617,7 @@
     }
 }
 
-template <int LOGM, int PPB>
+template <int LOGM, int PPB, bool LIM = false>
 __global__ void __launch_bounds__((1 << LOGM) / rows_elems(LOGM) * PPB) TFFT_WAVES_PER_EU(LOGM >= TFFT_ROWS_LAZY_LOG ? 4 : 1)
 k_rows_inv(const float2* __restrict__ in, uint8_t* __restrict__ rgb, const float2* __restrict__ tw,
                            RowParams P) {
@@ -591,12 +633,13 @@
     using Sync = typename std::conditional<T == 64, WaveSync, BlockSync>::type;
 
     const float2* src = in + (size_t)img * P.img_stride + ((size_t)(plane0 + pb) * P.PH + y) * M;
+    const int xlim = LIM ? *P.x_lim : M;
     constexpr int NSPLIT = (M / 2) / T + 1;
     float2 xk[NSPLIT], xm[NSPLIT], wk[NSPLIT];
 #pragma unroll
     for (int j = 0; j < NSPLIT; j++) {
-        const int k = imin(t + j * T, M / 2);
-        xk[j] = src[k]; xm[j] = src[(M - k) & (M - 1)]; wk[j] = tw[k];
+        const int k = imin(t + j * T, M / 2), k2 = (M - k) & (M - 1);
+        xk[j] = src[(!LIM || k < xlim) ? k : 0]; xm[j] = src[(!LIM || k2 < xlim) ? k2 : 0]; wk[j] = tw[k];
     }
     constexpr bool LAZY = LOGM >= TFFT_ROWS_LAZY_LOG;
     float2 W[LAZY ? 1 : tw_regs<M, E>()];
@@ -606,6 +649,8 @@
         const int k = t + j * T;
         if (k <= M / 2) {
             const int k2 = (M - k) & (M - 1);
+            if (LIM && k >= xlim) xk[j] = make_float2(0.f, 0.f);
+            if (LIM && k2 >= xlim) xm[j] = make_float2(0.f, 0.f);
             float2 zk, zk2;
             rsplit_inv(xk[j], xm[j], wk[j], zk, zk2);
             if (k == 0) zk = make_float2(0.5f * (xk[j].x + xk[j].y), 0.5f * (xk[j].x - xk[j].y));
@@ -744,7 +789,12 @@
     const int toff = ts > 1 ? P.tile_off : 0;
     const int tile0 = blockIdx.x * P.tiles_per_block;
     const int ntiles = ((P.M + C - 1) / C - toff + ts - 1) / ts;
-    const int tile1 = (tile0 + P.tiles_per_block < ntiles) ? tile0 + P.tiles_per_block : ntiles;
+    int tile1 = (tile0 + P.tiles_per_block < ntiles) ? tile0 + P.tiles_per_block : ntiles;
+    constexpr bool LIM = MODE == COLS_READ || embed_mode(MODE) || (MODE == COLS_PLAIN && (SIGN < 0 || TW));
+    if (LIM && P.x_lim) {
+        tile1 = imin(tile1, *P.x_lim >> 4);
+        if (tile0 >= tile1) return;
+    }
     const int rows_in_max = P.in_a * (L - 1) + P.in_b * (P.G - 1);
     const bool in_full = (rows_in_max < P.in_rows) && (P.M % C == 0) && (P.G % (int)blockDim.z == 0);
     const unsigned voff_in = (unsigned)((P.in_a * t + P.in_b * g) * P.M + c) * 8u;
@@ -1391,9 +1441,10 @@
     return width > 0 && width <= BUCKET_LCAP;
 }
 __global__ void k_bucket_count(const tfft_bin* __restrict__ bins, uint64_t n, int PH, int PW, int G, unsigned* __restrict__ cnt,
-                               int* __restrict__ err, int force_global) {
+                               int* __restrict__ err, int* __restrict__ x_lim, int force_global) {
     unsigned* lc = reinterpret_cast<unsigned*>(tfft_smem);
     unsigned* mm = lc + BUCKET_LCAP;
+    if (blockIdx.x == 0 && threadIdx.x == 0) *x_lim = 0;
     const uint64_t per = (n + gridDim.x - 1) / gridDim.x, lo = (uint64_t)blockIdx.x * per, hi = (lo + per < n) ? lo + per : n;
     unsigned bmin, width;
     const bool local = bucket_span(bins, lo, hi, PH, PW, G, mm, bmin, width, err) && !force_global;
@@ -1410,13 +1461,17 @@
         for (unsigned i = threadIdx.x; i < width; i += blockDim.x) if (lc[i]) atomicAdd(&cnt[bmin + i], lc[i]);
     }
 }
-__global__ void k_bucket_scan_a(unsigned* __restrict__ cnt, unsigned* __restrict__ off, unsigned* __restrict__ totals, int nb) {
+__global__ void k_bucket_scan_a(unsigned* __restrict__ cnt, unsigned* __restrict__ off, unsigned* __restrict__ totals, int nb, int ntiles,
+                                int nb_tiled, int* __restrict__ x_lim) {
     unsigned* sh = reinterpret_cast<unsigned*>(tfft_smem);
+    int* lim = reinterpret_cast<int*>(sh + 1024);
     const int t = threadIdx.x, i = blockIdx.x * 1024 + t;
     const unsigned v = (i < nb) ? cnt[i] : 0u;
     if (i < nb) cnt[i] = 0;
     sh[t] = v;
-    __syncthreads();
+    if (t == 0) *lim = 0;
+    __syncthreads();
+    if (v && i < nb_tiled) atomicMax(lim, 16 * (i % ntiles + 1));
     for (int d = 1; d < 1024; d <<= 1) {
         const unsigned a = (t >= d) ? sh[t - d] : 0u;
         __syncthreads();
@@ -1425,6 +1480,7 @@
     }
     if (i < nb) off[i] = sh[t] - v;
     if (t == 1023) totals[blockIdx.x] = sh[t];
+    if (t == 0 && *lim) atomicMax(x_lim, *lim);
 }
 __global__ void k_bucket_scan_b(unsigned* __restrict__ totals, int nblk, unsigned* __restrict__ off, int nb) {
     unsigned* sh = reinterpret_cast<unsigned*>(tfft_smem);
@@ -1477,8 +1533,9 @@
 }
 
 __global__ void k_bucket_count_walks(const tfft_bin* __restrict__ bins, uint64_t n, int chunks, int PH, int PW, int G, unsigned nb,
-                                     unsigned* __restrict__ cnt, int* __restrict__ err) {
+                                     unsigned* __restrict__ cnt, int* __restrict__ err, int* __restrict__ x_lim) {
     unsigned* lc = reinterpret_cast<unsigned*>(tfft_smem);
+    if (blockIdx.x == 0 && threadIdx.x == 0) *x_lim = 0;
     const int img = blockIdx.x / chunks, ch = blockIdx.x - img * chunks, nimg = gridDim.x / chunks;
     const uint64_t per = (n + chunks - 1) / chunks, lo = (uint64_t)ch * per, hi = (lo + per < n) ? lo + per : n;
     const bool local = nb + 1 <= BUCKET_LCAP;
@@ -2432,7 +2489,7 @@
         }
         hipLaunchKernelGGL(k, grid, block, lds, s, (const uint8_t*)in, (float2*)out, tw, P);
     } else {
-        auto k = k_rows_inv<LOGM, PPB>;
+        auto k = P.x_lim ? k_rows_inv<LOGM, PPB, true> : k_rows_inv<LOGM, PPB, false>;
         if (lds > 48 * 1024) {
             hipError_t e = hipFuncSetAttribute((const void*)k, hipFuncAttributeMaxDynamicSharedMemorySize, (int)lds);
             if (e != hipSuccess) return e;
@@ -2455,7 +2512,7 @@
                                       int n_images, hipStream_t s) {
     constexpr int LOGN1 = 3, M = 1 << LOGM;
     const size_t lds = ((size_t)(1 << LOGN1) * LayRows::padded(M) + M + (1 << LOGN1)) * sizeof(float2);
-    auto k = k_rowcol_fwd<LOGN1, LOGM>;
+    auto k = P.x_lim ? k_rowcol_fwd<LOGN1, LOGM, true> : k_rowcol_fwd<LOGN1, LOGM, false>;
     hipError_t e = hipFuncSetAttribute((const void*)k, hipFuncAttributeMaxDynamicSharedMemorySize, (int)lds);
     if (e != hipSuccess) return e;
     hipLaunchKernelGGL(k, dim3((P.PH >> LOGN1) * 3, n_images), dim3(M / 16, 1 << LOGN1), lds, s, rgb, out, tw_pw, tw_ph, P);
@@ -2471,7 +2528,7 @@
 static hipError_t launch_colrow_inv_t(const float2* in, uint8_t* rgb, const float2* tw_pw, const RowParams& P, int n_images, hipStream_t s) {
     constexpr int LOGN1 = 3, M = 1 << LOGM;
     const size_t lds = ((size_t)(1 << LOGN1) * LayRows::padded(M) + M) * sizeof(float2);
-    auto k = k_colrow_inv<LOGN1, LOGM>;
+    auto k = P.x_lim ? k_colrow_inv<LOGN1, LOGM, true> : k_colrow_inv<LOGN1, LOGM, false>;
     hipError_t e = hipFuncSetAttribute((const void*)k, hipFuncAttributeMaxDynamicSharedMemorySize, (int)lds);
     if (e != hipSuccess) return e;
     hipLaunchKernelGGL(k, dim3((P.PH >> LOGN1) * 3, n_images), dim3(M / 16, 1 << LOGN1), lds, s, in, rgb, tw_pw, P);
@@ -2487,7 +2544,7 @@
                                     int n2_lo, int n2_cnt, hipStream_t s) {
     constexpr int M = 1 << LOGM;
     const size_t lds = ((size_t)NL * LayRows::padded(M) + (LOGM <= 10 ? M : 0) + 8) * sizeof(float2);
-    auto k = k_rowcol_fwd_live<LOGM, NL>;
+    auto k = P.x_lim ? k_rowcol_fwd_live<LOGM, NL, true> : k_rowcol_fwd_live<LOGM, NL, false>;
     hipError_t e = hipFuncSetAttribute((const void*)k, hipFuncAttributeMaxDynamicSharedMemorySize, (int)lds);
     if (e != hipSuccess) return e;
     hipLaunchKernelGGL(k, dim3(n2_cnt * 3, n_images), dim3(M / 16, NL), lds, s, in, out, tw_pw, tw_ph, P, n2_lo, n2_cnt);
@@ -2642,7 +2699,7 @@
 }
 
 hipError_t launch_bucket_bins(const tfft_bin* bins, const uint32_t* bit_index, uint64_t n, int PH, int PW, int G,
-                              unsigned* cnt, unsigned* off, TileBin* out, int* err, int force_global, hipStream_t s) {
+                              unsigned* cnt, unsigned* off, TileBin* out, int* err, int* x_lim, int force_global, hipStream_t s) {
     const int M = PW >> 1, ntiles = (M + 15) >> 4, nb = 3 * ntiles * G;
     hipError_t e = hipMemsetAsync(cnt, 0, (size_t)nb * sizeof(unsigned), s);
     if (e != hipSuccess) return e;
@@ -2650,18 +2707,18 @@
     if (blocks < 1) blocks = 1;
     if (blocks > 4096) blocks = 4096;
     const size_t lds = (BUCKET_LCAP + 2) * sizeof(unsigned);
-    hipLaunchKernelGGL(k_bucket_count, dim3(blocks), dim3(256), lds, s, bins, n, PH, PW, G, cnt, err, force_global);
+    hipLaunchKernelGGL(k_bucket_count, dim3(blocks), dim3(256), lds, s, bins, n, PH, PW, G, cnt, err, x_lim, force_global);
     const int nblk = (nb + 1023) / 1024;
     if (nblk > 1024) return hipErrorInvalidValue;
     unsigned* totals = off + nb + 1;
-    hipLaunchKernelGGL(k_bucket_scan_a, dim3(nblk), dim3(1024), 1024 * sizeof(unsigned), s, cnt, off, totals, nb);
+    hipLaunchKernelGGL(k_bucket_scan_a, dim3(nblk), dim3(1024), 1025 * sizeof(unsigned), s, cnt, off, totals, nb, ntiles, nb, x_lim);
     hipLaunchKernelGGL(k_bucket_scan_b, dim3(1), dim3(1024), 1024 * sizeof(unsigned), s, totals, nblk, off, nb);
     hipLaunchKernelGGL(k_bucket_scan_c, dim3(nblk), dim3(1024), 0, s, off, totals, nb);
     hipLaunchKernelGGL(k_bucket_fill, dim3(blocks), dim3(256), lds, s, bins, bit_index, n, PH, PW, G, cnt, off, out, force_global);
     return hipGetLastError();
 }
 hipError_t launch_bucket_walks(const tfft_bin* bins, uint64_t n, int n_images, int PH, int PW, int G, unsigned* cnt, unsigned* off, TileBin* out,
-                               int* err, hipStream_t s) {
+                               int* err, int* x_lim, hipStream_t s) {
     if (n == 0 || n_images <= 0) return hipErrorInvalidValue;
     const int M = PW >> 1, ntiles = (M + 15) >> 4;
     const unsigned nb = 3u * (unsigned)ntiles * (unsigned)G, nbi = nb + 1;
@@ -2673,10 +2730,10 @@
     if (chunks < 1) chunks = 1;
     if ((uint64_t)chunks * (uint64_t)n_images > 65535ull) chunks = 65535 / n_images > 0 ? 65535 / n_images : 1;
     const size_t lds = nbi <= BUCKET_LCAP ? (size_t)nbi * sizeof(unsigned) : 16;
-    hipLaunchKernelGGL(k_bucket_count_walks, dim3((unsigned)(chunks * n_images)), dim3(256), lds, s, bins, n, chunks, PH, PW, G, nb, cnt, err);
+    hipLaunchKernelGGL(k_bucket_count_walks, dim3((unsigned)(chunks * n_images)), dim3(256), lds, s, bins, n, chunks, PH, PW, G, nb, cnt, err, x_lim);
     const int nblk = (int)((nbt + 1023) / 1024);
     unsigned* totals = off + nbt + 1;
-    hipLaunchKernelGGL(k_bucket_scan_a, dim3(nblk), dim3(1024), 1024 * sizeof(unsigned), s, cnt, off, totals, (int)nbt);
+    hipLaunchKernelGGL(k_bucket_scan_a, dim3(nblk), dim3(1024), 1025 * sizeof(unsigned), s, cnt, off, totals, (int)nbt, ntiles, (int)(nbt - 1), x_lim);
     hipLaunchKernelGGL(k_bucket_scan_b, dim3(1), dim3(1024), 1024 * sizeof(unsigned), s, totals, nblk, off, (int)nbt);
     hipLaunchKernelGGL(k_bucket_scan_c, dim3(nblk), dim3(1024), 0, s, off, totals, (int)nbt);
     hipLaunchKernelGGL(k_bucket_fill_walks, dim3((unsigned)(chunks * n_images)), dim3(256), lds, s, bins, n, chunks, PH, PW, G, nb, cnt, off, out);
```
